# winddori2002/DEX-TTS

Hardware: AMD Instinct MI355X
Metric: mel-frames/s at n_timesteps=50, 80-ch mel (sampler only); RTF (higher is better)
Workload: dtype bf16; 1 GPU; gedex_b1: gedex_lj B=1/GPU T=512 n_timesteps=50 (BASELINE.json configs[1]); global_batch=1, frames=512, hipgraph=False, parallelism=1 GPU

## Files before the change

dex_tts_amd/csrc/conv3x3_bf16.hip:

```cpp
#include "kernels.h"
#include <cstdlib>
#include <cstdio>
#include "lp_util.h"
#include "kernels_lp.h"
#include "conv_gn.h"

namespace dex {
namespace DEX_LP_NS {

typedef float f32x16 __attribute__((ext_vector_type(16)));
typedef unsigned short u16;
typedef unsigned u32x4 __attribute__((ext_vector_type(4)));

__device__ __forceinline__ float cv_mish(float x) {
    const float e = __expf(fminf(x, 20.f));
    const float n = e * (e + 2.f);
    return x * (n * __builtin_amdgcn_rcpf(n + 2.f));
}

template <int NT, int COUT>
__device__ __forceinline__ void cv_epilogue(const Conv3P& p, f32x16 (&acc)[NT], int b, int ho, int w0, int nbase, int lane, int tid,
                                            long long* gnred) {
    const int i = lane & 31, hh = lane >> 5;
    constexpr int cpg = COUT / 8;
    if (p.gn_stats) { if (tid < 16) gnred[tid] = 0; __syncthreads(); }
    const bool full = ho < p.H && w0 + 32 <= p.W;
    const long ybase = (long)b * p.H * p.W * COUT + ((long)ho * p.W + w0 + 4 * hh) * COUT + nbase + i;
    float* yl = p.Y + ybase;
    u16* yh = reinterpret_cast<u16*>(p.Y) + ybase;
    const bool yb = p.y_bf16 != 0;
#pragma unroll
    for (int t = 0; t < NT; ++t) {
        const int n = nbase + t * 32 + i;
        const float bias = p.bias[n];
        float gs = 0.f, gss = 0.f;
        if (full && yb) {
            const bool odd = (lane & 1) != 0;
            u16* yp = yh + (odd ? 16 * COUT - 1 : 0) + t * 32;
#pragma unroll
            for (int r = 0; r < 16; ++r) { const float v = acc[t][r] + bias; gs += v; gss = fmaf(v, v, gss); }
#pragma unroll
            for (int j = 0; j < 8; ++j) {
                const float lo_r = acc[t][j] + bias, hi_r = acc[t][8 + j] + bias;
                const float recv = lane_xor1(odd ? lo_r : hi_r);
                const float mine = odd ? hi_r : lo_r;
                const unsigned pk = odd ? pack2_lp(recv, mine) : pack2_lp(mine, recv);
                *reinterpret_cast<unsigned*>(yp + ((j & 3) + 8 * (j >> 2)) * COUT) = pk;
            }
        } else if (full) {
            const bool odd = (lane & 1) != 0;
            float* yp = yl + (odd ? 16 * COUT - 1 : 0) + t * 32;
#pragma unroll
            for (int r = 0; r < 16; ++r) { const float v = acc[t][r] + bias; gs += v; gss = fmaf(v, v, gss); }
#pragma unroll
            for (int j = 0; j < 8; ++j) {
                const float lo_r = acc[t][j] + bias, hi_r = acc[t][8 + j] + bias;
                const float recv = lane_xor1(odd ? lo_r : hi_r);
                const float mine = odd ? hi_r : lo_r;
                *reinterpret_cast<float2*>(yp + ((j & 3) + 8 * (j >> 2)) * COUT) = odd ? make_float2(recv, mine) : make_float2(mine, recv);
            }
        } else {
#pragma unroll
            for (int r = 0; r < 16; ++r) {
                const int wo = w0 + (r & 3) + 8 * (r >> 2) + 4 * hh;
                const bool ok = ho < p.H && wo < p.W;
                const float v = acc[t][r] + bias;
                const float vs = ok ? v : 0.f;
                gs += vs; gss = fmaf(vs, vs, gss);
                if (ok) {
                    if (yb) yh[((r & 3) + 8 * (r >> 2)) * COUT + t * 32] = lp_bits(v);
                    else yl[((r & 3) + 8 * (r >> 2)) * COUT + t * 32] = v;
                }
            }
        }
        if (p.gn_stats) {
            for (int o = 1; o < cpg; o <<= 1) { gs += __shfl_xor(gs, o); gss += __shfl_xor(gss, o); }
            gs += __shfl_xor(gs, 32); gss += __shfl_xor(gss, 32);
            if (hh == 0 && (i & (cpg - 1)) == 0) {
                const double inv_n = 1.0 / ((double)p.H * p.W * cpg);
                gn_add(&gnred[(n / cpg) * 2], gn_fix(gs, inv_n)); gn_add(&gnred[(n / cpg) * 2 + 1], gn_fix(gss, inv_n));
            }
        }
    }
    if (p.gn_stats) {
        __syncthreads();
        if (tid < 16) {
            const long long v = gnred[tid];
            if (v != 0) {
                const int slot = (blockIdx.x + blockIdx.y * gridDim.x) % GN_SLOTS;
                gn_add(p.gn_stats + (((long)b * 8 + (tid >> 1)) * GN_SLOTS + slot) * 2 + (tid & 1), v);
            }
        }
    }
}

template <int NT, int COUT>
__device__ __forceinline__ void cv_res_store(const Conv3P& p, const f32x16 (&accr)[NT], int b, int ho, int w0, int nb, int lane) {
    const int i = lane & 31, hh = lane >> 5;
    float* yl = p.res_y + ((long)b * p.H * p.W + (long)ho * p.W + w0 + 4 * hh) * COUT + nb + i;
    const bool rfull = ho < p.H && w0 + 32 <= p.W;
    const bool odd = (lane & 1) != 0;
#pragma unroll
    for (int t = 0; t < NT; ++t) {
        const float bias = p.res_b[nb + t * 32 + i];
        if (rfull) {
            float* yp = yl + (odd ? 16 * COUT - 1 : 0) + t * 32;
#pragma unroll
            for (int j = 0; j < 8; ++j) {
                const float lo_r = accr[t][j] + bias, hi_r = accr[t][8 + j] + bias;
                const float recv = lane_xor1(odd ? lo_r : hi_r);
                const float mine = odd ? hi_r : lo_r;
                *reinterpret_cast<float2*>(yp + ((j & 3) + 8 * (j >> 2)) * COUT) = odd ? make_float2(recv, mine) : make_float2(mine, recv);
            }
        } else {
#pragma unroll
            for (int r = 0; r < 16; ++r) {
                const int wo = w0 + (r & 3) + 8 * (r >> 2) + 4 * hh;
                if (ho < p.H && wo < p.W) yl[((r & 3) + 8 * (r >> 2)) * COUT + t * 32] = accr[t][r] + bias;
            }
        }
    }
}

template <int CC, int COUT, int NSL, int TH, bool PRO2 = false, bool RES = false, bool XB = false, int NW = 4, bool RW = false>
__global__ __launch_bounds__(64 * NW) void conv3x3_lp_kernel(const Conv3P p) {
    constexpr int PW = 34, PH = TH + 2;
    constexpr int LDP = CC + 8;
    constexpr int WN = NW / TH;
    constexpr int NTHR = 64 * NW;
    constexpr int NT = NSL / 32 / WN;
    constexpr int NSLICE = COUT / NSL;
    constexpr int ITEMS = PH * PW * (CC / 8);
    constexpr int NI = (ITEMS + NTHR - 1) / NTHR;
    constexpr int WITEMS = NSL * CC / 8;
    constexpr int WPT = (WITEMS + NTHR - 1) / NTHR;
    constexpr bool WFULL = WITEMS % NTHR == 0;
    constexpr int RING = CC == 128 ? (PRO2 ? 1 : 2) : 3;
    constexpr int NPASS = RW ? 1
                        : TH == 5 ? (CC == 128 ? (PRO2 ? 6 : 3) : (PRO2 ? 3 : XB ? 1 : 2))
                                  : CC == 128 ? (TH == 8 ? (PRO2 ? 8 : 4) : (PRO2 ? 5 : 2)) : (PRO2 ? 3 : 1);
    constexpr int NIP = (NI + NPASS - 1) / NPASS;
    constexpr int RWI = 9 * WITEMS;
    constexpr int RWPT = (RWI + NTHR - 1) / NTHR;
    constexpr int RWB = (RWPT + NPASS - 1) / NPASS;
#ifdef DEX_LP_WSPLIT
    constexpr int NTAP = 18;
#else
    constexpr int NTAP = 9;
#endif
    static_assert(NT >= 1 && WPT >= 1 && NW % TH == 0 && NTHR % (CC / 8) == 0, "tile");
    static_assert(!RW || NTAP == 9, "the resident schedule holds nine taps");
    extern __shared__ __attribute__((aligned(16))) u16 smem[];
    u16* patch = smem;
    u16* wbuf = smem + PH * PW * LDP;
    u16* rbuf = wbuf + (RW ? 9 : 2) * NSL * LDP;
    __shared__ long long gnred[16];
    constexpr int COEF_N = (TH == 8) ? 128 : 256;
    __shared__ __attribute__((aligned(16))) float coef[3][COEF_N];

    const int tid = threadIdx.x, lane = tid & 63, wave = tid >> 6;
    const int i = lane & 31, hh = lane >> 5;
    const int wrow = wave % TH, wcol = wave / TH;
#ifdef DEX_TIMING
    long long tk[8] = {0, 0, 0, 0, 0, 0, 0, 0};
    const long long tk0 = __builtin_readcyclecounter();
    long long tlast = tk0;
#define CSTAMP(k) do { const long long now_ = __builtin_readcyclecounter(); tk[k] += now_ - tlast; tlast = now_; } while (0)
#else
#define CSTAMP(k) do {} while (0)
#endif
    const int xs = p.skip_dead ? (int)((blockIdx.x + blockIdx.y + blockIdx.z) % gridDim.x) : (int)blockIdx.x;
    const int w0 = xs * 32, h0 = blockIdx.y * TH;
    const int b = blockIdx.z / NSLICE, slice = blockIdx.z % NSLICE;
    const int step = p.step + b * p.row_bstride;
    const float* X = p.X + (long)b * p.H * p.W * p.ldx + p.x_coff;
    const u16* Xh = reinterpret_cast<const u16*>(p.X) + (long)b * p.H * p.W * p.ldx + p.x_coff;
    const float* mrow = p.mask + (long)b * p.mask_bstride;
    const int K = 9 * p.Cin;
    const u16* Wg = reinterpret_cast<const u16*>(p.Wbf) + (long)slice * NSL * K;
    const bool pro = p.pro_stats != nullptr;
    if constexpr (!PRO2) {
        if (p.skip_dead) {
            const int wi = w0 - 1 + (lane < 34 ? lane : 33);
            const float mv = (unsigned)wi < (unsigned)p.W ? mrow[wi * p.mask_ws] : 0.f;
            if (__builtin_amdgcn_ballot_w64(mv != 0.f) == 0) {
                f32x16 zacc[NT];
#pragma unroll
                for (int t = 0; t < NT; ++t)
#pragma unroll
                    for (int r = 0; r < 16; ++r) zacc[t][r] = 0.f;
                if constexpr (RES) cv_res_store<NT, COUT>(p, zacc, b, h0 + wrow, w0, slice * NSL + wcol * NT * 32, lane);
                cv_epilogue<NT, COUT>(p, zacc, b, h0 + wrow, w0, slice * NSL + wcol * NT * 32, lane, tid, gnred);
                return;
            }
        }
    }

    f32x16 acc[NT];
#pragma unroll
    for (int t = 0; t < NT; ++t)
#pragma unroll
        for (int r = 0; r < 16; ++r) acc[t][r] = 0.f;

    f32x16 accr[RES ? NT : 1];
    if constexpr (RES) {
#pragma unroll
        for (int t = 0; t < NT; ++t)
#pragma unroll
            for (int r = 0; r < 16; ++r) accr[t][r] = 0.f;
    }
    int wofs[WPT], wlds[WPT];
    bool wok[WPT];
#pragma unroll
    for (int j = 0; j < WPT; ++j) {
        const int it = tid + NTHR * j;
        const int n = it / (CC / 8), c8 = (it % (CC / 8)) * 8;
        wofs[j] = n * K + c8;
        wlds[j] = n * LDP + c8;
        wok[j] = WFULL || it < WITEMS;
    }
    const int pc8 = (tid % (CC / 8)) * 8;

    CvGnLoads gnl{};
    if (pro) gnl = cv_gn_issue(p, b, tid, step);
    const int nchunk = RW ? 1 : p.Cin / CC;
    for (int ch = 0; ch < nchunk; ++ch) {
        const int cbase = ch * CC;
        u32x4 w0r[WPT], wr[RING][WPT], rwr[RES ? WPT : 1];
#ifdef DEX_LP_WSPLIT
        u32x4 rwl[RES ? WPT : 1];
#define WS_TAPOFS(t) ((long)((t) % 9) * p.Cin + ((t) >= 9 ? p.w_lo_off : 0L))
#else
#define WS_TAPOFS(t) ((long)(t) * p.Cin)
#endif
        float4 sc0, sc1, sh0, sh1, t0, t1;
#pragma unroll
        for (int ps = 0; ps < NPASS; ++ps) {
            float4 pf0[NIP], pf1[XB ? 1 : NIP], rf0[PRO2 ? NIP : 1], rf1[PRO2 ? NIP : 1];
            float pmk[NIP];
            bool pin[NIP];
#pragma unroll
            for (int q = 0; q < NIP; ++q) {
                const int it = min(tid + NTHR * (ps * NIP + q), ITEMS - 1);
                const int px = it / (CC / 8);
                const int pw = px % PW, ph = px / PW;
                const int hi = h0 + ph - 1, wi = w0 + pw - 1;
                const bool inb = (unsigned)hi < (unsigned)p.H && (unsigned)wi < (unsigned)p.W;
                const int hc = inb ? hi : 0, wc = inb ? wi : 0;
                if constexpr (XB) {
                    pf0[q] = *reinterpret_cast<const float4*>(Xh + ((long)hc * p.W + wc) * p.ldx + cbase + pc8);
                } else {
                    const float* src = X + ((long)hc * p.W + wc) * p.ldx + cbase + pc8;
                    pf0[q] = *reinterpret_cast<const float4*>(src);
                    pf1[q] = *reinterpret_cast<const float4*>(src + 4);
                }
                if constexpr (PRO2) {
                    const float* rs = p.pro_res + ((long)b * p.H * p.W + (long)hc * p.W + wc) * p.Cin + cbase + pc8;
                    rf0[q] = *reinterpret_cast<const float4*>(rs);
                    rf1[q] = *reinterpret_cast<const float4*>(rs + 4);
                }
                const float mk = mrow[wc * p.mask_ws];
                pmk[q] = inb ? mk : 0.f;
                pin[q] = inb;
            }
            u32x4 rwv[RW ? RWB : 1];
            if constexpr (RW) {
#pragma unroll
                for (int j = 0; j < RWB; ++j) {
                    const int it = tid + NTHR * (ps * RWB + j);
                    if (ps * RWB + j < RWPT && (RWI % NTHR == 0 || it < RWI)) {
                        const int r = it % WITEMS;
                        rwv[j] = *reinterpret_cast<const u32x4*>(Wg + (r / (CC / 8)) * K + (it / WITEMS) * p.Cin + (r % (CC / 8)) * 8);
                    }
                }
            }
            if (ps == 0) {
                if constexpr (RES) {
                    const u16* Rg = reinterpret_cast<const u16*>(p.res_w) + (long)slice * NSL * p.Cin;
#pragma unroll
                    for (int j = 0; j < WPT; ++j) {
                        const int it = tid + NTHR * j;
                        if (!wok[j]) continue;
                        rwr[j] = *reinterpret_cast<const u32x4*>(Rg + (long)(it / (CC / 8)) * p.Cin + cbase + (it % (CC / 8)) * 8);
#ifdef DEX_LP_WSPLIT
                        rwl[j] = *reinterpret_cast<const u32x4*>(Rg + p.res_lo_off + (long)(it / (CC / 8)) * p.Cin + cbase + (it % (CC / 8)) * 8);
#endif
                    }
                }
                if constexpr (!RW) {
#pragma unroll
                    for (int j = 0; j < WPT; ++j) if (wok[j]) w0r[j] = *reinterpret_cast<const u32x4*>(Wg + wofs[j] + cbase);
#pragma unroll
                    for (int s = 0; s < RING; ++s)
// ... 67 lines not shown
        }
        if constexpr (!RW) {
#pragma unroll
            for (int j = 0; j < WPT; ++j) if (wok[j]) *reinterpret_cast<u32x4*>(wbuf + wlds[j]) = w0r[j];
        }
        if constexpr (RES) {
#pragma unroll
            for (int j = 0; j < WPT; ++j) if (wok[j]) *reinterpret_cast<u32x4*>(rbuf + wlds[j]) = rwr[j];
        }
        CSTAMP(2);
        if constexpr (RW) {
            lds_barrier();
            constexpr int KS = CC / 16;
            const u16* ap = patch + (wrow * PW + i) * LDP + hh * 8;
            const u16* bp = wbuf + (wcol * NT * 32 + i) * LDP + hh * 8;
            const u16* rp = rbuf + (wcol * NT * 32 + i) * LDP + hh * 8;
            lp8 af[2], bf[2][NT], rf[2][RES ? NT : 1];
            af[0] = *reinterpret_cast<const lp8*>(ap);
#pragma unroll
            for (int t = 0; t < NT; ++t) bf[0][t] = *reinterpret_cast<const lp8*>(bp + t * 32 * LDP);
#pragma unroll
            for (int s = 0; s < 9 * KS; ++s) {
                if (s + 1 < 9 * KS) {
                    const int tap = (s + 1) / KS, ks = (s + 1) % KS, kh = tap / 3, kw = tap - kh * 3;
                    af[(s + 1) & 1] = *reinterpret_cast<const lp8*>(ap + (kh * PW + kw) * LDP + ks * 16);
#pragma unroll
                    for (int t = 0; t < NT; ++t) bf[(s + 1) & 1][t] = *reinterpret_cast<const lp8*>(bp + (tap * NSL + t * 32) * LDP + ks * 16);
                    if constexpr (RES) {
                        if (tap == 4) {
#pragma unroll
                            for (int t = 0; t < NT; ++t) rf[(s + 1) & 1][t] = *reinterpret_cast<const lp8*>(rp + t * 32 * LDP + ks * 16);
                        }
                    }
                }
                __builtin_amdgcn_sched_barrier(0);
#pragma unroll
                for (int t = 0; t < NT; ++t) acc[t] = DEX_MFMA_LP(af[s & 1], bf[s & 1][t], acc[t], 0, 0, 0);
                if constexpr (RES) {
                    if (s / KS == 4) {
#pragma unroll
                        for (int t = 0; t < NT; ++t) accr[t] = DEX_MFMA_LP(af[s & 1], rf[s & 1][t], accr[t], 0, 0, 0);
                    }
                }
                __builtin_amdgcn_sched_barrier(0);
            }
        } else {
#pragma unroll
        for (int tt = 0; tt < NTAP; ++tt) {
            const int tap = tt % 9;
            lds_barrier();
            if (tt + 1 < NTAP) {
                u16* wn = wbuf + ((tt + 1) & 1) * NSL * LDP;
#pragma unroll
                for (int j = 0; j < WPT; ++j) if (wok[j]) *reinterpret_cast<u32x4*>(wn + wlds[j]) = wr[tt % RING][j];
                if (tt + 1 + RING < NTAP) {
#pragma unroll
                    for (int j = 0; j < WPT; ++j)
                        if (wok[j]) wr[tt % RING][j] = *reinterpret_cast<const u32x4*>(Wg + wofs[j] + WS_TAPOFS(tt + 1 + RING) + cbase);
                }
                __builtin_amdgcn_sched_barrier(0);
            }
#ifdef DEX_LP_WSPLIT
            if constexpr (RES) {
                if (tt == 5) {
#pragma unroll
                    for (int j = 0; j < WPT; ++j) if (wok[j]) *reinterpret_cast<u32x4*>(rbuf + wlds[j]) = rwl[j];
                }
            }
#endif
            const u16* wb = wbuf + (tt & 1) * NSL * LDP;
            const int kh = tap / 3, kw = tap - kh * 3;
            const u16* ap = patch + ((wrow + kh) * PW + i + kw) * LDP + hh * 8;
            const u16* bp = wb + (wcol * NT * 32 + i) * LDP + hh * 8;
#pragma unroll
            for (int ks = 0; ks < CC / 16; ++ks) {
                const lp8 af = *reinterpret_cast<const lp8*>(ap + ks * 16);
#pragma unroll
                for (int t = 0; t < NT; ++t) {
                    const lp8 bf = *reinterpret_cast<const lp8*>(bp + t * 32 * LDP + ks * 16);
                    acc[t] = DEX_MFMA_LP(af, bf, acc[t], 0, 0, 0);
                }
                if constexpr (RES) {
                    if (tap == 4) {
#pragma unroll
                        for (int t = 0; t < NT; ++t) {
                            const lp8 rf = *reinterpret_cast<const lp8*>(rbuf + (wcol * NT * 32 + t * 32 + i) * LDP + hh * 8 + ks * 16);
                            accr[t] = DEX_MFMA_LP(af, rf, accr[t], 0, 0, 0);
                        }
                    }
                }
            }
        }
        }
    }
    if constexpr (RES) cv_res_store<NT, COUT>(p, accr, b, h0 + wrow, w0, slice * NSL + wcol * NT * 32, lane);
    CSTAMP(3);
    cv_epilogue<NT, COUT>(p, acc, b, h0 + wrow, w0, slice * NSL + wcol * NT * 32, lane, tid, gnred);
#ifdef DEX_TIMING
    CSTAMP(4);
    if (p.dbg && tid == 0) {
        long long* d = p.dbg + ((long)(blockIdx.z * gridDim.y + blockIdx.y) * gridDim.x + blockIdx.x) * 8;
        for (int k = 0; k < 5; ++k) d[k] = tk[k];
        unsigned hw, xcc;
        asm volatile("s_getreg_b32 %0, hwreg(HW_REG_HW_ID)" : "=s"(hw));
        asm volatile("s_getreg_b32 %0, hwreg(HW_REG_XCC_ID)" : "=s"(xcc));
        d[5] = hw; d[6] = xcc & 15u;
        d[7] = __builtin_readcyclecounter() - tk0;
    }
#endif
}

template <int CC, int COUT, int NSL, int TH, bool PRO2 = false, bool RES = false, bool XB = false, int NW = 4, bool RW = false>
static void launch_c3(const Conv3P& p, hipStream_t st) {
    constexpr int LDP = CC + 8;
    const size_t lds = ((size_t)(TH + 2) * 34 * LDP + ((RW ? 9 : 2) + (RES ? 1 : 0)) * NSL * LDP) * sizeof(u16);
    static bool attr = false;
    if (!attr) {
        hipFuncSetAttribute(reinterpret_cast<const void*>(&conv3x3_lp_kernel<CC, COUT, NSL, TH, PRO2, RES, XB, NW, RW>), hipFuncAttributeMaxDynamicSharedMemorySize, (int)lds);
        attr = true;
    }
    dim3 grid((p.W + 31) / 32, (p.H + TH - 1) / TH, p.B * (COUT / NSL));
    if (RW && p.Cin != CC) { fprintf(stderr, "libdexamd: resident conv3x3 form needs Cin == %d in one chunk (got %d)\n", CC, p.Cin); abort(); }
    Conv3P q = p;
    q.skip_dead = (p.B >= 4 && (long)grid.x * grid.y * grid.z >= 1024 && knob_or("DEX_CONV_SKIP_DEAD", 1) != 0) ? 1 : 0;
    static char sym[96];
    if (!sym[0]) snprintf(sym, sizeof sym, "conv3x3_lp_kernel<%d,%d,%d,%d,%d,%d,%d,%d%s>", CC, COUT, NSL, TH, (int)PRO2, (int)RES, (int)XB, NW, RW ? ",resident" : "");
    g_last_symbol = sym;
    hipLaunchKernelGGL((conv3x3_lp_kernel<CC, COUT, NSL, TH, PRO2, RES, XB, NW, RW>), grid, dim3(64 * NW), lds, st, q);
}

bool conv3x3_bf16_tail_supported(int C) {
#if defined(DEX_LP_WSPLIT) && !defined(DEX_WS_HAVE_CONV3)
    return false;
#endif
    return C == 64 || C == 128; }
bool conv3x3_bf16_xb_supported(int Cin, int Cout) {
#if defined(DEX_LP_WSPLIT) && !defined(DEX_WS_HAVE_CONV3)
    return false;
#endif
    return Cin == Cout && (Cin == 64 || Cin == 128); }
bool conv3x3_bf16_res_supported(int Cin, int Cout) {
#if defined(DEX_LP_WSPLIT) && !defined(DEX_WS_HAVE_CONV3_RES)
    return false;
#endif
    return (Cout == 128 && Cin == 64) || (Cout == 64 && (Cin == 128 || Cin == 256)); }
bool conv3x3_bf16_supported(int Cin, int Cout) {
#if defined(DEX_LP_WSPLIT) && !defined(DEX_WS_HAVE_CONV3)
    return false;
#endif
   
    return (Cin == 64 || Cin == 128 || Cin == 256) && (Cout == 64 || Cout == 128);
}

bool conv3x3_plain_lp_in_supported(int H, int W, int B, int Cin, int Cout) {
#if defined(DEX_LP_WSPLIT) && !defined(DEX_WS_HAVE_CONV3)
    return false;
#endif
   
    const int w8 = knob_or("DEX_CONV_W8", 1);
    const long tiles4 = (long)((W + 31) / 32) * ((H + 3) / 4) * B;
    return w8 && tiles4 >= 256 && Cin == 64 && Cout == 128;
}

bool conv3x3_cat_lp_in_supported(int H, int W, int B, int Cin, int Cout) {
#if defined(DEX_LP_WSPLIT) && !defined(DEX_WS_HAVE_CONV3_RES)
    return false;
#endif
   
    if (Cout != 64 || Cin < 128 || Cin % 128 != 0) return false;
    const int w8 = knob_or("DEX_CONV_W8", 1);
    const long small_max = knob_or("DEX_CONV_SMALL_MAX", 256);
    const long tiles4 = (long)((W + 31) / 32) * ((H + 3) / 4) * B;
    return w8 && tiles4 >= small_max;
}

static bool conv3x3_resident_on() { return knob_or("DEX_CONV_RESIDENT", 1) != 0; }

static bool launch_c3_round1(const Conv3P& p, bool small, hipStream_t st) {
    if (!knob_or("DEX_CONV_ROUND1", 1)) return false;
    const bool tail_ = p.pro_res != nullptr;
#ifdef DEX_LP_WSPLIT
    const bool c64 = p.Cin == 64 && p.Cout == 64 && !p.res_w && !tail_;
#else
    const bool c64 = p.Cin == 64 && p.Cout == 64 && !p.res_w;
#endif
    const bool r128 = p.Cin == 64 && p.Cout == 128 && p.res_w && !tail_ && !p.x_bf16;
    if (!c64 && !r128) return false;
    const long strips = (long)((p.W + 31) / 32) * p.B;
    const long cur = c64 ? strips * (small ? (p.H + 1) / 2 : (p.H + 3) / 4) : strips * (small ? (p.H + 1) / 2 * 2 : (p.H + 3) / 4);
    const long one = strips * ((p.H + 4) / 5) * (c64 ? 1 : 4);
    const long ncu = device_cus();
    if (cur <= ncu || one > ncu || one * 4 < ncu * 3) return false;
#ifndef DEX_LP_WSPLIT
    if (conv3x3_resident_on()) {
        if (c64 && !tail_) {
            p.x_bf16 ? launch_c3<64, 64, 64, 5, false, false, true, 10, true>(p, st) : launch_c3<64, 64, 64, 5, false, false, false, 10, true>(p, st);
            return true;
        }
        if (!c64) { launch_c3<64, 128, 32, 5, false, true, false, 5, true>(p, st); return true; }
    }
#endif
    if (c64) {
#ifndef DEX_LP_WSPLIT
        if (tail_) { p.x_bf16 ? launch_c3<64, 64, 64, 5, true, false, true, 10>(p, st) : launch_c3<64, 64, 64, 5, true, false, false, 10>(p, st); return true; }
#endif
        p.x_bf16 ? launch_c3<64, 64, 64, 5, false, false, true, 10>(p, st) : launch_c3<64, 64, 64, 5, false, false, false, 10>(p, st);
    } else {
        launch_c3<64, 128, 32, 5, false, true, false, 5>(p, st);
    }
    return true;
}

static bool launch_c3_small_resident(const Conv3P& p, bool small, hipStream_t st) {
#ifdef DEX_LP_WSPLIT
    return false;
#else
    if (!small || !conv3x3_resident_on() || p.Cin != 64 || p.Cout != 64 || p.res_w) return false;
    if ((long)((p.W + 31) / 32) * ((p.H + 1) / 2) * p.B > device_cus()) return false;
    const bool tail_ = p.pro_res != nullptr;
    if (tail_) { p.x_bf16 ? launch_c3<64, 64, 64, 2, true, false, true, 4, true>(p, st) : launch_c3<64, 64, 64, 2, true, false, false, 4, true>(p, st); }
    else { p.x_bf16 ? launch_c3<64, 64, 64, 2, false, false, true, 4, true>(p, st) : launch_c3<64, 64, 64, 2, false, false, false, 4, true>(p, st); }
    return true;
#endif
}

void launch_conv3x3_lp(const Conv3P& p, hipStream_t st) {
    if (const int tpw = conv3x3_stream_tiles(p)) { launch_conv3x3_stream(p, tpw, st); return; }
    if (conv3x3_regw_form(p)) { launch_conv3x3_regw(p, st); return; }
    const bool tail_ = p.pro_res != nullptr;
    const long tiles4 = (long)((p.W + 31) / 32) * ((p.H + 3) / 4) * p.B;
    const long small_max = knob_or("DEX_CONV_SMALL_MAX", 256);
    const bool small = tiles4 < small_max;
    const int w8 = knob_or("DEX_CONV_W8", 1);
    const int th8 = knob_or("DEX_CONV_TH8", 1);
    if (th8 && w8 && !small && !tail_ && p.Cin == 128 && p.Cout == 128 && !p.res_w && p.H % 8 == 0 && (long)((p.W + 31) / 32) * (p.H / 8) * p.B >= 512) {
        p.x_bf16 ? launch_c3<128, 128, 128, 8, false, false, true, 8>(p, st) : launch_c3<128, 128, 128, 8, false, false, false, 8>(p, st);
        return;
    }
    if (w8 && !small && p.Cin == 128 && p.Cout == 128 && !p.res_w) {
        if (p.x_bf16) { tail_ ? launch_c3<128, 128, 128, 4, true, false, true, 8>(p, st) : launch_c3<128, 128, 128, 4, false, false, true, 8>(p, st); }
        else { tail_ ? launch_c3<128, 128, 128, 4, true, false, false, 8>(p, st) : launch_c3<128, 128, 128, 4, false, false, false, 8>(p, st); }
        return;
    }
    if (w8 && !small && p.res_w && p.Cout == 128 && p.Cin == 64) {
        p.x_bf16 ? launch_c3<64, 128, 128, 4, false, true, true, 8>(p, st) : launch_c3<64, 128, 128, 4, false, true, false, 8>(p, st);
        return;
    }
    if (th8 && w8 && !small && p.res_w && p.Cout == 64 && p.Cin >= 128 && !p.pro_stats && p.H % 8 == 0 && (long)((p.W + 31) / 32) * (p.H / 8) * p.B >= 512) {
        p.x_bf16 ? launch_c3<128, 64, 64, 8, false, true, true, 8>(p, st) : launch_c3<128, 64, 64, 8, false, true, false, 8>(p, st);
        return;
    }
    if (w8 && !small && p.res_w && p.Cout == 64 && p.Cin >= 128) {
        p.x_bf16 ? launch_c3<128, 64, 64, 4, false, true, true, 8>(p, st) : launch_c3<128, 64, 64, 4, false, true, false, 8>(p, st);
        return;
    }
    if (launch_c3_round1(p, small, st)) return;
    if (launch_c3_small_resident(p, small, st)) return;
    if (p.x_bf16) {
        if (tail_) {
            if (p.Cin == 64) { small ? launch_c3<64, 64, 64, 2, true, false, true>(p, st) : launch_c3<64, 64, 64, 4, true, false, true>(p, st); }
            else { small ? launch_c3<128, 128, 64, 2, true, false, true>(p, st) : launch_c3<128, 128, 128, 4, true, false, true>(p, st); }
        } else {
            if (p.Cin == 64) { small ? launch_c3<64, 64, 64, 2, false, false, true>(p, st) : launch_c3<64, 64, 64, 4, false, false, true>(p, st); }
            else { small ? launch_c3<128, 128, 64, 2, false, false, true>(p, st) : launch_c3<128, 128, 128, 4, false, false, true>(p, st); }
        }
        return;
    }
    if (tail_) {
        if (p.Cin == 64 && p.Cout == 64) { small ? launch_c3<64, 64, 64, 2, true>(p, st) : launch_c3<64, 64, 64, 4, true>(p, st); }
        else { small ? launch_c3<128, 128, 64, 2, true>(p, st) : launch_c3<128, 128, 128, 4, true>(p, st); }
        return;
    }
    if (p.res_w) {
        if (p.Cout == 128 && p.Cin == 64) { small ? launch_c3<64, 128, 64, 2, false, true>(p, st) : launch_c3<64, 128, 128, 4, false, true>(p, st); return; }
        if (p.Cout == 64 && p.Cin >= 128) { small ? launch_c3<128, 64, 64, 2, false, true>(p, st) : launch_c3<128, 64, 64, 4, false, true>(p, st); return; }
    }
    if (p.Cout == 64) {
        if (p.Cin == 64) { small ? launch_c3<64, 64, 64, 2>(p, st) : launch_c3<64, 64, 64, 4>(p, st); }
        else { small ? launch_c3<128, 64, 64, 2>(p, st) : launch_c3<128, 64, 64, 4>(p, st); }
    } else {
        if (p.Cin == 64) { small ? launch_c3<64, 128, 64, 2>(p, st) : launch_c3<64, 128, 128, 4>(p, st); }
        else { small ? launch_c3<128, 128, 64, 2>(p, st) : launch_c3<128, 128, 128, 4>(p, st); }
    }
}

}
}
```

dex_tts_amd/csrc/dex_api.hip:

```cpp
#include <hip/hip_runtime.h>
#include <cstdlib>

#include <cmath>
#include <cstdarg>
#include <atomic>
#include <cstdio>
#include <mutex>
#include <cstring>
#include <map>
#include <unordered_map>
#include <string_view>
#include <string>
#include <vector>

#include "../../include/dex_amd.h"
#include "kernels.h"
#include "weight_store.h"

using namespace dex;

namespace dex {
namespace {
const char* const KNOB_NAMES[] = {
    "DEX_CONV_STREAM", "DEX_CONV_PP", "DEX_CONV_SKIP_DEAD", "DEX_H_BF16", "DEX_ATTN_SEPARATE", "DEX_ATTN_Q64", "DEX_ATTN_Q64_TAIL", "DEX_ATTN_Q64_HALF", "DEX_DIT_XCDS", "DEX_ATTN_GENERIC", "DEX_RES2", "DEX_LP_INTER", "DEX_DIT_CHAIN",
    "DEX_DIT_CLUSTER", "DEX_DIT_CLUSTER_LOCAL", "DEX_ATTN_X_LP", "DEX_RES_X_LP", "DEX_CAT_LP", "DEX_XCD_MAP", "DEX_DEBUG_DROP_HANDOFF", "DEX_PATCH_FUSED",
    "DEX_CONV_DOWN", "DEX_CONVT_UP", "DEX_DEBUG_PLAN",
    "DEX_ATTN_SHARED_W8", "DEX_CONVT_MT", "DEX_CONVT_WGS", "DEX_CONV_DOWN_WGS", "DEX_CONV_REGW", "DEX_CONV_REGW_RES", "DEX_CONV_SMALL_MAX", "DEX_CONV_TH8",
    "DEX_CONV_W8", "DEX_DWCONV_CAP", "DEX_FINAL_CAP", "DEX_FIRST_CAP", "DEX_FIRST_MFMA", "DEX_GEMM_NWALK", "DEX_NWALK_SPLIT", "DEX_NWALK_BM", "DEX_POS_COL", "DEX_POS_COL_MIN",
    "DEX_POS_CT", "DEX_REGW_MIN_TILES", "DEX_REGW_WGS", "DEX_ROWCHAIN64", "DEX_ROWCHAIN64A", "DEX_TIV_CAP", "DEX_TV_CHAIN", "DEX_TIV_FOLD", "DEX_LINATTN_NSUB", "DEX_TV_FOLD", "DEX_OUT2_MIN", "DEX_NWALK_DMA",
    "DEX_LINATTN_HEADWAVES", "DEX_LINATTN_OUT2_HW", "DEX_CONV_ROUND1", "DEX_CONV_RESIDENT", "DEX_KVCTX_ROWS", "DEX_OUT2_ROWS", "DEX_PE_TOK", "DEX_NWALK_SMALL"};
constexpr int N_KNOBS = (int)(sizeof(KNOB_NAMES) / sizeof(KNOB_NAMES[0]));
int knob_parse(const char* e) {
    if (!e) return KNOB_UNSET;
    char* end = nullptr;
    const long v = strtol(e, &end, 10);
    if (end == e) {
        static bool warned = false;
        if (!warned) { warned = true; fprintf(stderr, "libdexamd: ignoring a DEX_* knob whose value '%s' is not an integer\n", e); }
        return KNOB_UNSET;
    }
    return (int)v;
}
struct KnobSnapshot {
    int v[N_KNOBS];
    KnobSnapshot() { for (int i = 0; i < N_KNOBS; ++i) v[i] = knob_parse(getenv(KNOB_NAMES[i])); }
};
thread_local const KnobSnapshot* t_knobs = nullptr;
struct WsplitScope {
    bool prev;
    explicit WsplitScope(bool on) : prev(g_lp_wsplit) { g_lp_wsplit = on; }
    ~WsplitScope() { g_lp_wsplit = prev; }
};
struct KnobScope {
    const KnobSnapshot* prev;
    explicit KnobScope(const KnobSnapshot* k) : prev(t_knobs) { t_knobs = k; }
    ~KnobScope() { t_knobs = prev; }
};
}
static int knob_index(const char* name) {
    static const std::unordered_map<std::string_view, int> idx = [] {
        std::unordered_map<std::string_view, int> m;
        for (int i = 0; i < N_KNOBS; ++i) m.emplace(KNOB_NAMES[i], i);
        return m;
    }();
    const auto it = idx.find(std::string_view(name));
    return it == idx.end() ? -1 : it->second;
}
int knob(const char* name) {
    if (t_knobs) {
        const int i = knob_index(name);
        if (i >= 0) return t_knobs->v[i];
    }
    return knob_parse(getenv(name));
}
}
static_assert(PREC_FP32 == DEX_PREC_FP32 && PREC_BF16 == DEX_PREC_BF16 && PREC_FP16 == DEX_PREC_FP16 && PREC_FP16X2 == DEX_PREC_FP16X2, "kernels.h mirrors DexPrecision");

namespace {
void xcd_map_probe();

struct TD { float* p; int ld; int coff; int C; int lp = 0; };

struct ResW { PackedW w1, w2, wr; const float *b1, *g1, *be1, *b2, *g2, *be2, *br, *mlp_w, *mlp_b; int cin, cout; };
constexpr int ATT_KSPLIT_MAX = 4;
static int att_split_cap(long tokens) { return tokens <= 20480 ? 8 : ATT_KSPLIT_MAX; }
static bool attention_q64_regime(int N, int B) {
    if (N < 1024) return dit_sep64_small_n(N, B) && dit_rowchain64_form(N, B, 0);
    const int ks = attention_q64_ksplit(N, B, att_split_cap((long)B * N));
    const int nt32 = (N + 31) / 32, ng = (nt32 + 7) / 8;
    return 2L * B * ng * ks >= 128;
}
struct LinW { PackedW wqkv; const float *wqkv_raw, *wout_raw, *bias_eff, *g; LpView wkv[3], wq_frag[3]; int C; };
struct DitBlockW { PackedW wqkv, wproj, wfc1, wfc2; const float *bqkv, *bproj, *bfc1, *bfc2, *ada_w, *ada_b; };

struct Prof { std::string name; hipEvent_t a, b; double flops, bytes; };
struct ProfAgg { std::string name; int calls; double ms, flops, bytes; };

struct Arena {
    char* base = nullptr; size_t off = 0, cap = 0; bool dry = true;
    void* take(size_t bytes) {
        off = (off + 255) & ~size_t(255);
        void* p = dry ? nullptr : (void*)(base + off);
        if (!dry && trace) fprintf(stderr, "plan[%d] off %zu bytes %zu\n", trace++, off, bytes);
        off += bytes;
        return p;
    }
    int trace = 0;
    float* f(size_t n) { return (float*)take(n * sizeof(float)); }
};

}

struct DexCtx : WeightStore {
    DexCtx() : WeightStore("") {}
    DexConfig cfg{};
    int lpi() const { return precision == DEX_PREC_FP16X2 ? 2 : precision == DEX_PREC_FP16 ? 1 : 0; }
    int lp_kind() const { return precision == DEX_PREC_BF16 ? 1 : 2; }
    bool lp() const { return precision != DEX_PREC_FP32; }
    bool tuned = true;
    int precision = DEX_PREC_FP32;
    std::vector<std::vector<ResW>> down_res, up_res;
    std::vector<LinW> down_lin, up_lin;
    std::vector<PackedW> down_ds_w;
    std::vector<std::vector<PackedW>> up_us_w;
    std::vector<const float*> down_ds_b, up_us_b;
    const float *fc_w3 = nullptr, *fc_w1 = nullptr;
    PackedW fin_w, pe_pw, fl_w, tv_wk, tv_wv, tv_wl;
    PackedW pos_w;
    const float *fin_b = nullptr, *fin_g = nullptr, *fin_be = nullptr, *fconv_w = nullptr, *fconv_b = nullptr;
    const float *pe_dw = nullptr, *pe_db = nullptr, *pe_pb = nullptr, *pos_b = nullptr, *freq_pos = nullptr;
    std::vector<DitBlockW> blocks;
    const float *fl_b = nullptr, *fl_ada_w = nullptr, *fl_ada_b = nullptr;
    const float *tv_wq_raw = nullptr;
    float *mel_basis = nullptr, *mel_filt = nullptr; void* mel_ws = nullptr; size_t mel_ws_bytes = 0;
    const int* last_xerr = nullptr;
    int* st_host = nullptr; hipEvent_t st_ev = nullptr; bool st_pending = false;
    struct Tap { std::string name; const float* p; std::vector<int64_t> shape; };
    std::vector<Tap> taps;
    bool prof_on = false;
    std::vector<Prof> prof;
    std::vector<ProfAgg> prof_agg;
    struct GraphEntry { std::vector<uint64_t> key; hipGraphExec_t exec; uint64_t stamp; const int* xerr; };
    std::vector<GraphEntry> graphs;
    uint64_t graph_clock = 0;
    void drop_graphs() { for (auto& g : graphs) hipGraphExecDestroy(g.exec); graphs.clear(); }
    template <typename F> int replay(const std::vector<uint64_t>& key, hipStream_t st, F&& enqueue);
    void reset_records() {
        taps.clear();
        if (prof_on) { for (auto& pr : prof) { hipEventDestroy(pr.a); hipEventDestroy(pr.b); } prof.clear(); prof_agg.clear(); }
    }
};

template <typename F> int DexCtx::replay(const std::vector<uint64_t>& key, hipStream_t st, F&& enqueue) {
    GraphEntry* hit = nullptr;
    for (auto& g : graphs) if (g.key == key) { hit = &g; break; }
    if (!hit) {
        constexpr size_t MAX_GRAPHS = 8;
        if (graphs.size() >= MAX_GRAPHS) {
            size_t lru = 0;
            for (size_t i = 1; i < graphs.size(); ++i) if (graphs[i].stamp < graphs[lru].stamp) lru = i;
            hipGraphExecDestroy(graphs[lru].exec);
            graphs.erase(graphs.begin() + lru);
        }
        hipGraph_t graph = nullptr;
        DEX_HIPCHK(this, hipStreamBeginCapture(st, hipStreamCaptureModeThreadLocal));
        const int rc = enqueue();
        hipError_t ec = hipStreamEndCapture(st, &graph);
        if (rc) { if (graph) hipGraphDestroy(graph); return rc; }
        if (ec != hipSuccess || !graph) return fail(DEX_ERR_HIP, "stream capture failed: %s", hipGetErrorString(ec));
        hipGraphExec_t exec = nullptr;
        ec = hipGraphInstantiate(&exec, graph, nullptr, nullptr, 0);
        hipGraphDestroy(graph);
        if (ec != hipSuccess) return fail(DEX_ERR_HIP, "hipGraphInstantiate failed: %s", hipGetErrorString(ec));
        graphs.push_back({key, exec, 0, last_xerr});
        hit = &graphs.back();
    }
    last_xerr = hit->xerr;
    hit->stamp = ++graph_clock;
    DEX_HIPCHK(this, hipGraphLaunch(hit->exec, st));
    DEX_HIPCHK(this, hipGetLastError());
    return DEX_OK;
}

// ... 663 lines not shown
        g.inmask = nullptr; g.inmask_ws = 1; g.outmask = nullptr; g.outmask_ws = 1; g.mask_bstride = P.d.T;
        g.act = 0; g.gate = nullptr; g.gate_nstride = 1; g.gate_step_stride = 0;
        g.res = nullptr; g.ldres = 0; g.res_bstride = 0; g.res_coff = 0;
        g.step = sp; g.row_bstride = rbs; g.unpatch_s = 0; g.unpatch_C = 0; g.B = P.d.B;
        return g;
    }
    void gemm(const char* name, const IGemmP& g) {
        const double M = (double)g.Ho * g.Wo * g.B;
        const double fl = 2.0 * M * g.N * g.groups * g.K;
        const double by = 4.0 * (M * g.Cin * g.groups + M * g.N * g.groups * g.ksplit + (double)g.K * g.N * g.groups);
        run(name, fl, by, [&] { launch_igemm(g, x->precision, st); });
    }
    struct Pro { const gnfix_t* stats; const float *gamma, *beta, *tadd; const float* res = nullptr; float* xout = nullptr; bool x_bf16 = false;
                 bool res2 = false; FirstConvP res2f{};
                 mutable bool xout_lp_ok = false;
                 mutable bool xout_lp = false; };
    static bool ln_fusable(int K) { return K == 64 || K == 128 || K == 256 || K == 512; }
    bool h_bf16() const { return x->lp() && !knob_off("DEX_H_BF16"); }
    bool fast_conv(int cin, int cout) const { return x->lp() && conv3x3_bf16_supported(cin, cout); }
    void conv3x3(const char* name, const TD& X, int H, int W, int mask_ws, bool inmask, const PackedW& Wt, const float* bias, int Cout, float* out,
                 gnfix_t* gn = nullptr, const Pro* pro = nullptr, const ResW* shortcut = nullptr, float* shortcut_out = nullptr,
                 bool xb = false, bool yb = false) {
        const int t = x->lpi();
        if (fast_conv(X.C, Cout) && Wt.nk[t].p) {
            Conv3P c{};
            c.x_bf16 = (xb || X.lp) ? 1 : 0; c.y_bf16 = yb ? 1 : 0;
            c.X = X.p; c.ldx = X.ld; c.x_coff = X.coff; c.H = H; c.W = W; c.Cin = X.C; c.Cout = Cout;
            c.Wbf = Wt.nk[t].p; c.w_lo_off = Wt.nk[t].lo_off; c.bias = bias; c.Y = out; c.mask = mask; c.mask_ws = mask_ws; c.mask_bstride = P.d.T;
            if (pro) { c.pro_stats = pro->stats; c.pro_gamma = pro->gamma; c.pro_beta = pro->beta; c.pro_tadd = pro->tadd; c.pro_res = pro->res; c.pro_xout = pro->xout;
                if (pro->res2) {
                    const FirstConvP& f = pro->res2f;
                    c.pro_res = nullptr; c.res2_w = f.W1; c.res2_b = f.b1; c.res2_mu = f.mu; c.res2_x = f.x; c.res2_spk = f.spk;
                    c.res2_scal = f.scal; c.res2_scal_stride = f.scal_stride; c.res2_planes = f.planes;
                } }
            c.step = sp; c.row_bstride = rbs; c.gn_stats = gn; c.B = P.d.B;
            c.Wfrag = Wt.frag[t].p;
            const bool want_xout_lp = pro && pro->xout && pro->xout_lp_ok;
            if (shortcut) {
                c.res_w = shortcut->wr.nk[t].p; c.res_lo_off = shortcut->wr.nk[t].lo_off; c.res_b = shortcut->br; c.res_y = shortcut_out;
                c.res_wfrag = shortcut->wr.frag[t].p;
            }
            if (want_xout_lp && (c.pro_res || c.res2_w) && conv3x3_strip_form(c)) { c.xout_lp = 1; pro->xout_lp = true; }
            const double M = (double)H * W * P.d.B;
            const double bytes = M * (((xb || X.lp) ? 2.0 : 4.0) * X.C + (yb ? 2.0 : 4.0) * Cout + (pro && (pro->res || pro->res2) ? (pro->res2 ? 4.0 * X.C : 8.0 * X.C) - (c.xout_lp ? 2.0 * X.C : 0.0) : 0.0) + (shortcut ? 4.0 * Cout : 0.0))
                                 + 2.0 * 9 * X.C * Cout;
            run(name, 2.0 * M * Cout * (9 * X.C + (shortcut ? X.C : 0)), bytes, [&] { launch_conv3x3_lp(c, x->precision, st); });
            return;
        }
        IGemmP g = base_gemm(X.p, X.ld, X.coff, H, W, X.C, Wt, Cout, bias, out, Cout, 0);
        g.KH = 3; g.KW = 3; g.off_h = -1; g.off_w = -1; g.K = 9 * X.C;
        if (inmask) { g.inmask = mask; g.inmask_ws = mask_ws; }
        g.gn_stats = gn; g.gn_groups = 8; g.gn_cpg = Cout / 8;
        gemm(name, g);
    }
    void gn_stats(const float* h, int C, long npix, gnfix_t* stats) {
        GnStatsP s{h, C, npix * C, (int)npix, C, 8, stats, P.d.B};
        run("gn_stats", 3.0 * npix * C * P.d.B, 4.0 * npix * C * P.d.B, [&] { launch_gn_stats(s, st); });
    }
    void gn_apply(const float* h, int C, long npix, int W, int mask_ws, const gnfix_t* stats, const float* gamma, const float* beta,
                  const float* tadd, const float* res, int ldres, long resb, bool res_under_mask, float* out) {
        GnApplyP a{};
        a.X = h; a.ldx = C; a.xb = npix * C; a.Y = out; a.ldy = C; a.yb = npix * C; a.y_coff = 0;
        a.npix = (int)npix; a.W = W; a.C = C; a.groups = 8; a.stats = stats; a.gamma = gamma; a.beta = beta;
        a.mask = mask; a.mask_ws = mask_ws; a.mask_bstride = P.d.T;
        a.tadd = tadd; a.tadd_step_stride = C; a.step = sp; a.row_bstride = rbs;
        a.res = res; a.ldres = ldres; a.resb = resb; a.res_under_mask = res_under_mask ? 1 : 0; a.B = P.d.B;
        run("gn_apply_mish", 12.0 * npix * C * P.d.B, (res ? 12.0 : 8.0) * npix * C * P.d.B, [&] { launch_gn_apply(a, st); });
    }

    void resblock(const ResW& w, const StageBuf& s, const TD& X, const float* tadd, float* out, bool first_layer, LinKvCtxP* tail = nullptr,
                  const Pro* head = nullptr, Pro* ctail = nullptr) {
        const long npix = s.npix;
        const float* resptr; int ldres; long resb; bool under = false;
        gnfix_t* st1 = nullptr;
        const bool conv2_fast = fast_conv(w.cout, w.cout) && conv3x3_bf16_xb_supported(w.cout, w.cout);
        const bool conv1_fast = first_layer || (head ? true : fast_conv(X.C, w.cout));
        const bool h1b = h_bf16() && conv2_fast && conv1_fast;
        const bool h2b = h_bf16() && conv2_fast && (ctail || tail);
        if (first_layer) {
            FirstConvP f{};
            f.h1_bf16 = h1b ? x->lp_kind() : 0;
            f.mu = mu; f.x = xcur; f.spk = P.spk_plane; f.mask = mask; f.B = P.d.B; f.H = s.H; f.T = s.W; f.planes = w.cin; f.C = w.cout;
            f.W3 = w.w1.f32; f.b3 = w.b1; f.W1 = w.wr.f32; f.b1 = w.br; f.scal = P.scal; f.scal_stride = SCAL_STRIDE; f.step = sp; f.row_bstride = rbs;
            f.h1 = s.h1; f.res = s.rbuf;
            { if (ctail && h2b && w.cout == 64 && conv3x3_res2_form(s.H, s.W, P.d.B) && !knob_off("DEX_RES2")) { f.res = nullptr; ctail->res2 = true; ctail->res2f = f; } }
            st1 = next_stats(); f.gn_stats = st1;
            run("first_conv", 2.0 * npix * P.d.B * w.cout * (w.cin * 10), npix * P.d.B * ((h1b ? 2.0 : 4.0) * w.cout + (f.res ? 4.0 * w.cout : 0.0) + 4.0 * w.cin), [&] { launch_first_conv(f, st); });
            resptr = s.rbuf; ldres = w.cout; resb = npix * w.cout;
        } else {
            st1 = next_stats();
            bool fused_res = false;
            if (head) {
                TD H2{s.h2, X.C, 0, X.C};
                head->xout_lp_ok = tail != nullptr && !w.wr && lp_inter_cur && head->xout == X.p && X.coff == 0 && X.ld == X.C && !knob_off("DEX_RES_X_LP");
                conv3x3("conv3x3", H2, s.H, s.W, s.mask_ws, true, w.w1, w.b1, w.cout, s.h1, st1, head, nullptr, nullptr, head->x_bf16, h1b);
            } else {
                fused_res = w.wr && fast_conv(X.C, w.cout) && conv3x3_bf16_res_supported(X.C, w.cout);
                conv3x3("conv3x3", X, s.H, s.W, s.mask_ws, true, w.w1, w.b1, w.cout, s.h1, st1, nullptr, fused_res ? &w : nullptr, s.rbuf, false, h1b);
            }
            if (fused_res) {
                resptr = s.rbuf; ldres = w.cout; resb = npix * w.cout;
            } else if (w.wr) {
                IGemmP g = base_gemm(X.p, X.ld, X.coff, s.H, s.W, X.C, w.wr, w.cout, w.br, s.rbuf, w.cout, 0);
                g.inmask = mask; g.inmask_ws = s.mask_ws;
                gemm("conv1x1_res", g);
                resptr = s.rbuf; ldres = w.cout; resb = npix * w.cout;
            } else {
                resptr = X.p + X.coff; ldres = X.ld; resb = npix * X.ld; under = true;
            }
        }
        if (!st1) { st1 = next_stats(); gn_stats(s.h1, w.cout, npix, st1); }
        gnfix_t* st2 = next_stats();
        if (fast_conv(w.cout, w.cout)) {
            Pro pro{st1, w.g1, w.be1, tadd};
            TD H1{s.h1, w.cout, 0, w.cout};
            conv3x3("conv3x3", H1, s.H, s.W, s.mask_ws, true, w.w2, w.b2, w.cout, s.h2, st2, &pro, nullptr, nullptr, h1b, h2b);
        } else {
            gn_apply(s.h1, w.cout, npix, s.W, s.mask_ws, st1, w.g1, w.be1, tadd, nullptr, 0, 0, false, s.a1);
            TD A1{s.a1, w.cout, 0, w.cout};
            conv3x3("conv3x3", A1, s.H, s.W, s.mask_ws, false, w.w2, w.b2, w.cout, s.h2, st2);
        }
        if (ctail) {
            ctail->stats = st2; ctail->gamma = w.g2; ctail->beta = w.be2; ctail->tadd = nullptr; ctail->res = resptr; ctail->xout = out;
            ctail->x_bf16 = h2b;
            return;
        }
        if (tail) {
            tail->H2 = s.h2; tail->gn_stats = st2; tail->gamma = w.g2; tail->beta = w.be2;
            tail->res = resptr; tail->ldres = ldres; tail->resb = resb; tail->res_under_mask = under ? 1 : 0;
            tail->res_lp = (head && head->xout_lp && resptr == X.p) ? 1 : 0;
            tail->mask = mask; tail->mask_ws = s.mask_ws; tail->mask_bstride = P.d.T; tail->W = s.W; tail->Xout = out;
            tail->h2_bf16 = h2b ? 1 : 0;
            return;
        }
        gn_apply(s.h2, w.cout, npix, s.W, s.mask_ws, st2, w.g2, w.be2, nullptr, resptr, ldres, resb, under, out);
    }

    bool lp_inter_cur = false;
    bool cat_lp = false;
    IGemmP final_gemm(int mask_ws, float* out, int ldo, int ocoff) {
        const DexConfig& c = x->cfg;
        const int hid = c.dit_hidden, mid = mid_dim(c);
        const bool fuse_lnf = x->lp() && ln_fusable(hid);
        const int s2c = c.dit_stride * c.dit_stride * mid;
        IGemmP fl = base_gemm(fuse_lnf ? P.tok : P.xn, hid, 0, P.Hf, P.Wt, hid, x->fl_w, s2c, x->fl_b, out, ldo, ocoff);
        if (fuse_lnf) { fl.ln_shift = P.fin_mod; fl.ln_scale = P.fin_mod + hid; fl.ln_step_stride = 2L * hid; }
        fl.Wfrag = x->fl_w.frag[x->lpi()].p;
        fl.unpatch_s = c.dit_stride; fl.unpatch_C = mid; fl.OHf = P.Hm; fl.OWf = P.Wm;
        fl.c_bstride = (long)P.Hm * P.Wm * ldo;
        fl.outmask = mask; fl.outmask_ws = mask_ws;
        return fl;
    }
    bool linattn_fused(int C) const { return x->lp() && (C == 64 || C == 128) && linattn_fused_supported(C); }
    void linattn(const LinW& w, const StageBuf& s, const TD& X, float* out, int ldo, int ocoff, const LinKvCtxP* tail = nullptr, bool out_lp = false,
                 void* out2_lp = nullptr, int ldo2 = 0, int ocoff2 = 0) {
        const long npix = s.npix; const int B = P.d.B;
        if (linattn_fused(X.C)) {
            int nsub = 1;
            while (nsub < 4 && (npix + 128 * nsub - 1) / (128 * nsub) * B > 192) nsub *= 2;
            {
                const int ncu = device_cus();
                const long slots = (long)(X.C == 64 ? 2 : 1) * ncu;
                if ((npix + 127) / 128 * B >= 2 * slots) {
                    long best = -1;
                    for (int n = 1; n <= 8; ++n) {
                        const long wgs = (npix + 128L * n - 1) / (128L * n) * B;
                        const long cost = (wgs + slots - 1) / slots * n;
                        if (best < 0 || cost <= best) { best = cost; nsub = n; }
                    }
                }
                const int forced = knob_or("DEX_LINATTN_NSUB", 0);
                if (forced > 0) nsub = forced;
            }
            const int nblk = (int)((npix + 128L * nsub - 1) / (128L * nsub));
            LinKvCtxP k{};
            if (tail) k = *tail;
            k.X = X.p; k.ldx = X.ld; k.x_coff = X.coff; k.xb = npix * X.ld; k.npix = (int)npix; k.C = X.C; k.Wkv = w.wkv[x->lpi()].p;
            k.wkv_lo_off = w.wkv[x->lpi()].lo_off;
            k.nsub = nsub; k.nblk = nblk; k.part_m = s.pm; k.part_s = s.ps; k.part_c = s.pc; k.B = B;
            k.headwaves = knob_or("DEX_LINATTN_HEADWAVES", (long)nblk * B <= device_cus() ? 1 : 0) != 0 ? 1 : 0;
            k.rows = knob_or("DEX_KVCTX_ROWS", 1) != 0 ? 1 : 0;
            const bool xlp = k.H2 && k.Xout && lp_inter_cur && linattn_out2_lp_out_supported((int)npix, B) && !knob_off("DEX_ATTN_X_LP");
            k.xout_lp = xlp ? 1 : 0;
            run("linattn_kvctx", 2.0 * npix * B * (256.0 * X.C + 128 * 32), (tail ? (tail->h2_bf16 ? 10.0 : 12.0) - (xlp ? 2.0 : 0.0) : 4.0) * npix * X.C * B, [&] { launch_linattn_kvctx(k, x->precision, st); });
            LinMergeP mg{s.pm, s.ps, s.pc, nblk, w.wout_raw, w.g, X.C, s.mbf, B};
            run("linattn_merge", 2.0 * 128 * 32 * X.C * B, 4.0 * nblk * 4 * 1088 * B, [&] { launch_linattn_merge(mg, x->precision, st); });
            LinOut2P o{X.p, X.ld, X.coff, npix * X.ld, (int)npix, X.C, w.wq_frag[x->lpi()].p, s.mbf, w.bias_eff, out, ldo, ocoff, npix * ldo, B, out_lp ? 1 : 0,
                       out2_lp, ldo2, ocoff2, npix * ldo2, xlp ? 1 : 0};
            o.wq_lo_off = w.wq_frag[x->lpi()].lo_off;
            o.hw = knob_or("DEX_LINATTN_OUT2_HW", linattn_out2_lp_out_supported((int)npix, B) ? 0 : 1) != 0 ? 1 : 0;
            o.rows = knob_or("DEX_OUT2_ROWS", 1) != 0 ? 1 : 0;
            run("linattn_out", 4.0 * npix * B * 128.0 * X.C, ((out_lp ? 6.0 : 8.0) - (xlp ? 2.0 : 0.0) + (out2_lp ? 2.0 : 0.0)) * npix * X.C * B, [&] { launch_linattn_out2(o, x->precision, st); });
            return;
        }
        IGemmP g = base_gemm(X.p, X.ld, X.coff, s.H, s.W, X.C, w.wqkv, 384, nullptr, s.qkv, 384, 0);
        gemm("linattn_qkv", g);
        LinAttnCtxP cp{s.qkv, 384, npix * 384, (int)npix, 4, LA_CHUNK, s.nchunks, s.pm, s.ps, s.pc, B};
        run("linattn_ctx", 2.0 * npix * 128 * 32 * B, 4.0 * npix * 384 * B, [&] { launch_linattn_ctx(cp, st); });
        LinAttnCombineP cb{s.pm, s.ps, s.pc, s.nchunks, 4, w.wout_raw, w.g, w.C, s.weff, B};
        run("linattn_combine", 2.0 * 128 * 32 * w.C * B, 4.0 * s.nchunks * 4 * 1100 * B, [&] { launch_linattn_combine(cb, st); });
        IGemmP o = base_gemm(s.qkv, 384, 0, s.H, s.W, 128, s.weff, w.C, w.bias_eff, out, ldo, ocoff);
        o.w_bstride = 128L * w.C;
        o.res = X.p; o.ldres = X.ld; o.res_coff = X.coff; o.res_bstride = npix * X.ld;
        gemm("linattn_out", o);
    }

    void dit(const TD& X, bool mask_input, int mask_ws, float* out, int ldo, int ocoff, const float* in_aff = nullptr) {
        const DexConfig& c = x->cfg;
        const int B = P.d.B, hid = c.dit_hidden, mid = mid_dim(c), N = P.N, mh = mlp_hidden(c);
        DwConvP dw{};
        dw.X = X.p + X.coff; dw.ldx = X.ld; dw.xb = (long)P.Hm * P.Wm * X.ld; dw.Hi = P.Hm; dw.Wi = P.Wm; dw.C = mid;
        dw.k = c.dit_patch; dw.s = c.dit_stride; dw.pad = c.dit_patch / 2; dw.Wd = x->pe_dw; dw.bd = x->pe_db;
        dw.mask = mask_input ? mask : nullptr; dw.mask_ws = mask_ws; dw.mask_bstride = P.d.T;
        dw.Y = P.pe0; dw.Hf = P.Hf; dw.Wt = P.Wt; dw.B = B; dw.aff = in_aff;
        if (patch_fused()) {
            run("patch_embed", 2.0 * B * N * mid * (c.dit_patch * c.dit_patch + hid), 4.0 * B * (P.Hm * P.Wm * mid + N * hid),
                [&] { launch_patch_embed_fused(dw, x->pe_pw.nk[x->lpi()].p, x->pe_pb, P.emb, hid, x->precision, st); });
        } else {
            run("patch_dwconv_silu", 2.0 * B * N * mid * c.dit_patch * c.dit_patch, 4.0 * B * (P.Hm * P.Wm + N) * mid, [&] { launch_dwconv_silu(dw, st); });
            IGemmP pe = base_gemm(P.pe0, mid, 0, P.Hf, P.Wt, mid, x->pe_pw, hid, x->pe_pb, P.emb, hid, 0);
            gemm("patch_pointwise", pe);
        }
        const int G = c.dit_conv_pos_groups, kp = c.dit_conv_pos, cg = hid / G;
        int nsplit = POS_SPLIT, pcg = 0, pcgp = 0;
        if (x->lp() && x->pos_w.frag[x->lpi()].p) {
            PosConvP pcd{P.emb, x->pos_w.frag[x->lpi()].p, P.pos_part, P.Hf, P.Wt, hid, G, B};
            run("pos_conv", 2.0 * B * N * (double)kp * kp * cg * hid, 8.0 * B * N * hid + 2.0 * kp * kp * cg * hid, [&] { launch_pos_conv_direct(pcd, x->precision, st); });
            nsplit = 1;
        } else {
            const int cgp = (cg % 32) ? 64 : cg;
            const float* src = P.emb;
            if (cgp != cg) {
                run("pos_group_pad", 0, 8.0 * B * N * hid, [&] { launch_group_pad(P.emb, P.emb_pad, (long)B * N, G, cg, cgp, st); });
                src = P.emb_pad;
            }
            IGemmP pc = base_gemm(src, G * cgp, 0, P.Hf, P.Wt, cgp, x->pos_w, cgp, nullptr, P.pos_part, G * cgp, 0);
            pc.KH = kp; pc.KW = kp; pc.off_h = -(kp / 2); pc.off_w = -(kp / 2); pc.K = kp * kp * cgp;
            pc.groups = G; pc.w_gstride = (long)kp * kp * cgp * cgp; pc.ksplit = POS_SPLIT; pc.c_sstride = (long)B * N * G * cgp;
            gemm("pos_conv", pc);
            pcg = cgp != cg ? cg : 0; pcgp = cgp;
        }
        PosFinishP pf{P.pos_part, nsplit, (long)B * N * (pcg ? G * pcgp : hid), x->pos_b, P.emb, x->freq_pos, P.tok, P.Hf, P.Wt, hid, B, pcg, pcgp};
        run("pos_finish", 20.0 * B * N * hid, 4.0 * B * N * hid * (nsplit + 2), [&] { launch_pos_finish(pf, st); });
        if (debug) hipMemcpyAsync(P.dbg_tok, P.tok, (size_t)B * N * hid * 4, hipMemcpyDeviceToDevice, st);
        tap("tok_in", P.dbg_tok, (long)B * N, hid, hid);
        const float scale = 1.0f / sqrtf((float)(hid / c.dit_heads));
        const bool chain = x->lp() && dit_rowchain_supported(hid, mh) && c.dit_heads == 2 &&
                           !knob_off("DEX_DIT_CHAIN");
        for (int k = 0; k < c.dit_depth; ++k) {
            const DitBlockW& w = x->blocks[k];
            const float* ada = P.ada[k];
            const bool fuse_ln = x->lp() && ln_fusable(hid);
            DitChainP ch{};
            if (chain) {
                ch.ksplit = 0; ch.heads = c.dit_heads; ch.rows_per_batch = N; ch.X = P.tok; ch.ada = ada; ch.step = sp; ch.row_bstride = rbs; ch.M = B * N; ch.B = B;
                ch.Qh = (k & 1) ? P.qh : P.qh2; ch.Kh = (k & 1) ? P.kh : P.kh2; ch.Vt = (k & 1) ? P.vt : P.vt2;
                ch.Qin = (k & 1) ? P.qh2 : P.qh; ch.Kin = (k & 1) ? P.kh2 : P.kh; ch.Vin = (k & 1) ? P.vt2 : P.vt;
                ch.Npad = P.Npad;
                ch.qscale = scale * 1.4426950408889634f;
                if (P.xflag) {
                    ch.xslab = P.xslab; ch.xflag = P.xflag; ch.epoch = (unsigned)(sp * (c.dit_depth + 1) + k + 1);
                    ch.xerr = reinterpret_cast<int*>(P.xflag + (P.xflag_bytes - sizeof(int)) / sizeof(unsigned));
                    x->last_xerr = ch.xerr;
                    ch.xdrop = knob_or("DEX_DEBUG_DROP_HANDOFF", 0);
                    ch.xlocal = (P.xlocal && ch.epoch < (1u << 24)) ? 1 : 0;
                    ch.xcds = dit_rowchain_cluster_xcds(N, B);
                }
            }
            if (chain && k == 0) {
                ch.qkv_only = 1; ch.Wq = w.wqkv.frag[x->lpi()].p; ch.bq = w.bqkv;
                ch.Qh = P.qh; ch.Kh = P.kh; ch.Vt = P.vt;
                ch.next_shift = ada; ch.next_scale = ada + hid; ch.next_step_stride = 6L * hid;
                run("dit_qkv", 2.0 * B * N * 3.0 * hid * hid, 4.0 * B * N * hid + 2.0 * B * N * 3 * hid, [&] { launch_dit_rowchain(ch, x->precision, st); });
                ch.qkv_only = 0; ch.Wq = nullptr; ch.bq = nullptr; ch.next_shift = ch.next_scale = nullptr;
                ch.Qh = P.qh2; ch.Kh = P.kh2; ch.Vt = P.vt2;
            }
            if (!chain) {
                IGemmP q = base_gemm(fuse_ln ? P.tok : P.xn, hid, 0, 1, N, hid, w.wqkv, 3 * hid, w.bqkv, P.qkv, 3 * hid, 0);
                if (fuse_ln) { q.ln_shift = ada + 0 * hid; q.ln_scale = ada + 1 * hid; q.ln_step_stride = 6L * hid; }
                else {
                    LnModP l1{P.tok, P.xn, N, hid, ada + 0 * hid, ada + 1 * hid, 6L * hid, sp, B, rbs};
                    run("ln_modulate", 8.0 * B * N * hid, 8.0 * B * N * hid, [&] { launch_ln_mod(l1, st); });
                }
                gemm("dit_qkv", q);
            }
            if (chain) {
                const int sep_env = knob("DEX_ATTN_SEPARATE");
                const bool batch_regime = attention_direct_batch_regime(N, B);
                const int q64_env = knob("DEX_ATTN_Q64");
                const bool q64_ok = q64_env != KNOB_UNSET ? q64_env != 0 : attention_q64_regime(N, B);
                const bool separate = sep_env != KNOB_UNSET ? sep_env != 0 : ((batch_regime && N >= 1024) || q64_ok);
                const bool q64 = separate && q64_ok;
                int ks = 1, tail_row0 = 0, tail_ks = 0;
                bool o_lp = false;
                if (separate) {
                    const long blocks = (long)((N + 31) / 32) * 2 * B;
                    const int ntiles = (N + 31) / 32;
                    ks = q64 ? attention_q64_ksplit(N, B, att_split_cap((long)B * N))
                       : batch_regime ? attention_direct_ksplit(N, B)
                                      : (int)std::max<long>(1, std::min<long>(std::min<long>(768 / blocks, (ntiles + 7) / 8), ATT_KSPLIT_MAX));
                    AttnDirectP ad{ch.Qin, ch.Kin, ch.Vin, N, P.Npad, B, P.ao, (long)B * N * hid, ks > 1 ? P.att_ml : nullptr, ks, nullptr};
                    o_lp = (batch_regime || q64) && ks == 1 && lp_inter_cur && dit_rowchain64_form(N, B, 0);
                    ad.o_lp = o_lp ? 1 : 0;
                    if (q64 && ks == 1 && dit_rowchain64_form(N, B, 0) && knob_or("DEX_ATTN_Q64_TAIL", 0) != 0) {
                        int pks = 1, tg = 0, tk = 1;
                        attention_q64_plan(N, B, att_split_cap((long)B * N), &pks, &tg, &tk);
                        if (pks == 1 && tk > 1) { ad.tail_g = tg; ad.tail_ks = tk; ad.ml = P.att_ml; tail_row0 = tg * 256; tail_ks = tk; }
                    }
                    run("dit_attention", 4.0 * B * (double)N * N * hid, 2.0 * 3 * B * N * hid + (o_lp ? 2.0 : 4.0) * B * N * hid * ks,
                        [&] { if (q64) launch_attention_q64(ad, x->precision, st); else launch_attention_direct(ad, x->precision, st); });
                }
                ch.attn_inline = separate ? 0 : 1; ch.o_lp = o_lp ? 1 : 0; ch.tail_row0 = tail_row0; ch.tail_ks = tail_ks;
                const bool last = k + 1 == c.dit_depth;
                ch.O = P.ao; ch.ksplit = ks; ch.o_sstride = (long)B * N * hid; ch.ml = P.att_ml;
                ch.Wp = w.wproj.frag[x->lpi()].p; ch.W1 = w.wfc1.frag[x->lpi()].p; ch.W2 = w.wfc2.frag[x->lpi()].p;
                ch.bp = w.bproj; ch.b1 = w.bfc1; ch.b2 = w.bfc2;
                if (!last) {
                    const DitBlockW& wn = x->blocks[k + 1];
                    ch.Wq = wn.wqkv.frag[x->lpi()].p; ch.bq = wn.bqkv;
                    ch.next_shift = P.ada[k + 1]; ch.next_scale = P.ada[k + 1] + hid; ch.next_step_stride = 6L * hid;
                }
                const double M = (double)B * N;
                const double wel = (double)hid * hid + 2.0 * hid * mh + (last ? 0.0 : 3.0 * hid * hid);
                run(separate ? "dit_rowchain" : "dit_block", 2.0 * M * wel + (separate ? 0.0 : 4.0 * B * (double)N * N * hid),
                    4.0 * M * hid * (last ? 3 : 6) + 2.0 * wel, [&] { launch_dit_rowchain(ch, x->precision, st); });
                if (debug) {
                    float* dst = P.dbg_tok + (size_t)(k + 1) * B * N * hid;
                    hipMemcpyAsync(dst, P.tok, (size_t)B * N * hid * 4, hipMemcpyDeviceToDevice, st);
                    char nm[32]; snprintf(nm, sizeof nm, "tok_blk%d", k);
                    tap(nm, dst, (long)B * N, hid, hid);
                }
                continue;
            }
            AttnP a{};
            a.Q = P.qkv; a.ldq = 3 * hid; a.qb = (long)N * 3 * hid;
            a.K = P.qkv + hid; a.ldk = 3 * hid; a.kb = a.qb; a.V = P.qkv + 2 * hid; a.ldv = 3 * hid; a.vb = a.qb;
            a.O = P.ao; a.ldo = hid; a.ob = (long)N * hid; a.Nq = N; a.Nk = N; a.kv_len = nullptr; a.kv_len_add = 0;
            a.heads = c.dit_heads; a.scale = scale; a.B = B; a.head_dim = hid / c.dit_heads;
            a.force_generic = (knob_or("DEX_ATTN_GENERIC", 0) && x->precision == DEX_PREC_FP32) ? 1 : 0;
            run("dit_attention", 4.0 * B * (double)N * N * hid, 4.0 * 4 * B * N * hid, [&] { launch_attention(a, x->precision, st); });
            IGemmP pr = base_gemm(P.ao, hid, 0, 1, N, hid, w.wproj, hid, w.bproj, P.tok, hid, 0);
            pr.gate = ada + 2 * hid; pr.gate_nstride = 1; pr.gate_step_stride = 6L * hid;
            pr.res = P.tok; pr.ldres = hid; pr.res_bstride = (long)N * hid;
            gemm("dit_proj", pr);
            IGemmP f1 = base_gemm(fuse_ln ? P.tok : P.xn, hid, 0, 1, N, hid, w.wfc1, mh, w.bfc1, P.hmlp, mh, 0);
            if (fuse_ln) { f1.ln_shift = ada + 3 * hid; f1.ln_scale = ada + 4 * hid; f1.ln_step_stride = 6L * hid; }
            else {
                LnModP l2{P.tok, P.xn, N, hid, ada + 3 * hid, ada + 4 * hid, 6L * hid, sp, B, rbs};
                run("ln_modulate", 8.0 * B * N * hid, 8.0 * B * N * hid, [&] { launch_ln_mod(l2, st); });
            }
            f1.act = 1;
            gemm("dit_fc1_gelu", f1);
            IGemmP f2 = base_gemm(P.hmlp, mh, 0, 1, N, mh, w.wfc2, hid, w.bfc2, P.tok, hid, 0);
            f2.gate = ada + 5 * hid; f2.gate_nstride = 1; f2.gate_step_stride = 6L * hid;
            f2.res = P.tok; f2.ldres = hid; f2.res_bstride = (long)N * hid;
            gemm("dit_fc2", f2);
            if (debug) {
                float* dst = P.dbg_tok + (size_t)(k + 1) * B * N * hid;
                hipMemcpyAsync(dst, P.tok, (size_t)B * N * hid * 4, hipMemcpyDeviceToDevice, st);
                char nm[32]; snprintf(nm, sizeof nm, "tok_blk%d", k);
                tap(nm, dst, (long)B * N, hid, hid);
            }
        }
        const bool fuse_lnf = x->lp() && ln_fusable(hid);
        if (!fuse_lnf) {
            LnModP lf{P.tok, P.xn, N, hid, P.fin_mod, P.fin_mod + hid, 2L * hid, sp, B, rbs};
            run("ln_modulate", 8.0 * B * N * hid, 8.0 * B * N * hid, [&] { launch_ln_mod(lf, st); });
        }
        IGemmP fl = final_gemm(mask_ws, out, ldo, ocoff);
        if (cat_lp) { fl.C = reinterpret_cast<float*>(P.cat16); fl.c_lp = x->lp_kind(); }
        gemm("dit_final_unpatchify", fl);
    }

    bool patch_fused() const {
        const DexConfig& c = x->cfg;
        return x->lp() && !debug && !knob_off("DEX_PATCH_FUSED") &&
               patch_embed_fused_supported(c.dit_patch, mid_dim(c), c.dit_hidden, (long)P.d.B * P.N);
    }
    bool tiv_fold() const { return !debug && P.tiv_aff && knob_or("DEX_TIV_FOLD", 1) != 0; }
    bool tv_chain_on() const {
        return x->lp() && x->tv_wl.nk[x->lpi()].p && P.tv_kp && tv_chain_form(P.Hm * P.Wm, mid_dim(x->cfg), P.d.B);
    }
    bool tv_fold_on() const { return tv_chain_on() && x->lpi() != 2 && P.tv_G && knob_or("DEX_TV_FOLD", 1) != 0; }
    void dex_adaptors(const TD& X, int mask_ws) {
        const DexConfig& c = x->cfg;
        const int B = P.d.B, mid = mid_dim(c);
        const long npix = (long)P.Hm * P.Wm;
        InStatsP is{X.p + X.coff, X.ld, npix * X.ld, (int)npix, mid, P.tv_stats, B, mask, mask_ws, (long)P.d.T, P.Wm};
        run("in2d_stats", 3.0 * npix * mid * B, 4.0 * npix * mid * B, [&] { launch_in_stats(is, st); });
        const long stats_floats = (long)B * mid * IN_SLOTS * 2 * (long)(sizeof(gnfix_t) / sizeof(float));
        if (tv_fold_on()) {
            TvFold2P f2{P.tv_stats, (int)npix, 1e-5f, P.tv_G, (long)(P.d.Ts + 1) * mid, P.tv_g0, P.tv_v0p, sp, P.d.Ts + 1, P.tv_nkpad, mid,
                        1.0f / sqrtf((float)mid), P.tv_kp, P.tv_vtp, P.tv_xmean, reinterpret_cast<float*>(P.tiv_stats), stats_floats, x->lp_kind(), B, rbs};
            run("tv_fold_keys", 2.0 * B * (P.d.Ts + 1) * mid, 6.0 * B * (P.d.Ts + 1) * mid, [&] { launch_tv_fold2(f2, st); });
            TvChainP tc{X.p, X.ld, X.coff, npix * X.ld, (int)npix, P.Wm, mask, mask_ws, (long)P.d.T,
                        nullptr, 0L, nullptr, nullptr, 0L,
                        P.tv_kp, P.tv_vtp, P.tv_nkpad, P.d.Ts + 1, args->sty_lengths_dev, 1, 1.0f,
                        P.tv_out, P.tiv_stats, B, P.tv_xmean, reinterpret_cast<float*>(P.tv_stats), stats_floats};
            run("tv_chain", 4.0 * B * (double)npix * (P.d.Ts + 1) * mid, 8.0 * B * npix * mid, [&] { launch_tv_chain(tc, x->precision, st); });
            tap("tv", P.tv_out, B * npix, mid, mid);
            tiv(npix);
            return;
        }
        const bool qbf = x->lp();
        InFoldP fo{P.tv_stats, (int)npix, 1e-5f, x->tv_wq_raw, mid, P.tv_weff, P.tv_beff, B, qbf ? P.tv_wbf : nullptr, x->lp_kind()};
        fo.split = x->lpi() == 2 ? 1 : 0;
        run("tv_fold_in2d", 2.0 * mid * mid * B, 8.0 * mid * mid * B, [&] { launch_in_fold(fo, st); });
        IGemmP q = base_gemm(X.p, X.ld, X.coff, P.Hm, P.Wm, mid, P.tv_weff, mid, P.tv_beff, P.tv_q, mid, 0);
        q.w_bstride = (long)mid * mid; q.bias_bstride = mid; q.inmask = mask; q.inmask_ws = mask_ws;
        if (qbf) { q.Wbf = P.tv_wbf; q.w_lo_off = fo.split ? (long)B * mid * mid : 0; }
        const bool chain = tv_chain_on();
        if (!chain) gemm("tv_q", q);
        TvRow0P r0{P.tv_k0, P.tv_v0, sp, P.tv_K, P.tv_V, (long)(P.d.Ts + 1) * mid, mid, B, reinterpret_cast<float*>(P.tv_stats),
                   (long)B * mid * IN_SLOTS * 2 * 2 * (long)(sizeof(gnfix_t) / sizeof(float))};
        r0.row_bstride = rbs;
        if (chain) { r0.Kp = P.tv_kp; r0.VTp = P.tv_vtp; r0.NkPad = P.tv_nkpad; r0.lp_kind = x->lp_kind(); }
        run("tv_time_token", 0, 8.0 * mid * B, [&] { launch_tv_row0(r0, st); });
        if (chain) {
            const LpView& wl = x->tv_wl.nk[x->lpi()];
            TvChainP tc{X.p, X.ld, X.coff, npix * X.ld, (int)npix, P.Wm, mask, mask_ws, (long)P.d.T,
                        P.tv_wbf, fo.split ? (long)B * mid * mid : 0L, P.tv_beff, wl.p, wl.lo_off,
                        P.tv_kp, P.tv_vtp, P.tv_nkpad, P.d.Ts + 1, args->sty_lengths_dev, 1, 1.0f / sqrtf((float)mid),
                        P.tv_out, P.tiv_stats, B};
            run("tv_chain", 4.0 * B * (double)npix * mid * mid + 4.0 * B * (double)npix * (P.d.Ts + 1) * mid, 8.0 * B * npix * mid,
                [&] { launch_tv_chain(tc, x->precision, st); });
            tap("tv", P.tv_out, B * npix, mid, mid);
            tiv(npix);
            return;
        }
        AttnP a{};
        a.Q = P.tv_q; a.ldq = mid; a.qb = npix * mid; a.K = P.tv_K; a.ldk = mid; a.kb = (long)(P.d.Ts + 1) * mid;
        a.V = P.tv_V; a.ldv = mid; a.vb = a.kb; a.O = P.tv_ao; a.ldo = mid; a.ob = npix * mid;
        a.Nq = (int)npix; a.Nk = P.d.Ts + 1; a.kv_len = args->sty_lengths_dev; a.kv_len_add = 1; a.heads = 1;
        a.scale = 1.0f / sqrtf((float)mid); a.B = B; a.head_dim = mid;
        const bool ao_lp = lp_inter_cur && mid == 128 && x->tv_wl.nk[x->lpi()].p && attention_lp_shared_form((int)npix, 1, B, 1);
        a.o_lp = ao_lp ? 1 : 0;
        run("tv_attention", 4.0 * B * (double)npix * (P.d.Ts + 1) * mid, (ao_lp ? 2.0 : 4.0) * B * npix * mid + 4.0 * B * (npix + 2 * (P.d.Ts + 1)) * mid, [&] { launch_attention(a, x->precision, st); });
        IGemmP o = base_gemm(P.tv_ao, mid, 0, P.Hm, P.Wm, mid, x->tv_wl, mid, nullptr, P.tv_out, mid, 0);
        if (ao_lp) o.a_lp = x->lp_kind();
        o.res = X.p; o.ldres = X.ld; o.res_coff = X.coff; o.res_bstride = npix * X.ld;
        o.outmask = mask; o.outmask_ws = mask_ws;
        o.gn_stats = P.tiv_stats; o.gn_groups = mid; o.gn_cpg = 1; o.stats_final = 1;
        gemm("tv_out", o);
        tap("tv", P.tv_out, B * npix, mid, mid);
        tiv(npix);
    }
    void tiv(long npix) {
        const int B = P.d.B, mid = mid_dim(x->cfg);
        TivApplyP ta{P.tv_out, mid, npix * mid, P.tiv_out, mid, npix * mid, (int)npix, mid, P.tiv_stats, 1e-5f, P.sap_s, P.sap_m, sp, B, rbs};
        if (tiv_fold()) { run("tiv_coefficients", 0, 16.0 * mid * B, [&] { launch_tiv_coef(ta, P.tiv_aff, st); }); return; }
        run("tiv_adain", 2.0 * npix * mid * B, 8.0 * npix * mid * B, [&] { launch_tiv_apply(ta, st); });
        tap("tiv", P.tiv_out, B * npix, mid, mid);
    }

    void step(float* denoised, float* xnext) {
        const DexConfig& c = x->cfg;
        const int B = P.d.B, ns = c.n_stages;
        gn_idx = 0;
        if (debug) {
            tap("mlp", P.temb + (long)sp * c.dim, rbs ? B : 1, c.dim, c.dim);
            tap("vit.t_embedder", P.c_emb + (long)sp * c.dit_hidden, rbs ? B : 1, c.dit_hidden, c.dit_hidden);
        }
        if (!stats_other) zero_fill(stats_base, P.stats_bytes, st);
        TD cur{nullptr, 0, 0, 0};
        const bool lp_inter = x->lp() && !debug && ns >= 2 && !knob_off("DEX_LP_INTER") && fast_conv(c.dim, c.dim);
        lp_inter_cur = lp_inter;
        cat_lp = false;
        if (lp_inter && ns == 2 && P.cat16) {
            const StageBuf& sm_ = P.down[ns - 1];
            const ResW& uw = x->up_res[0][0];
            const bool tail_ok = linattn_fused(sm_.C) && linattn_out2_lp_out_supported((int)sm_.npix, B);
            const bool conv_ok = uw.wr && fast_conv(2 * sm_.C, uw.cout) && conv3x3_bf16_res_supported(2 * sm_.C, uw.cout) &&
                                 conv3x3_cat_lp_in_supported(P.up[0].H, P.up[0].W, B, 2 * sm_.C, uw.cout);
            IGemmP fl = final_gemm(sm_.mask_ws, P.cat[0], 2 * sm_.C, 0);
            fl.c_lp = x->lp_kind();
            cat_lp = !knob_off("DEX_CAT_LP") && tail_ok && conv_ok && fl.Wbf && igemm_nwalk_form(fl);
        }
        const int lpk = x->lp_kind();
        for (int i = 0; i < ns; ++i) {
            const StageBuf& s = P.down[i];
            Pro t0{};
            const bool defer0 = x->lp() && conv3x3_bf16_tail_supported(s.C) && fast_conv(s.C, s.C) &&
                                (i == 0 || x->down_res[i][0].wr);
            resblock(x->down_res[i][0], s, cur, P.tadd_down[2 * i], s.r0out, i == 0, nullptr, nullptr, defer0 ? &t0 : nullptr);
            TD r0{s.r0out, s.C, 0, s.C};
            LinKvCtxP tail{};
            const bool defer = linattn_fused(s.C);
            resblock(x->down_res[i][1], s, r0, P.tadd_down[2 * i + 1], s.r1out, false, defer ? &tail : nullptr, defer0 ? &t0 : nullptr);
            TD r1{s.r1out, s.C, 0, s.C};
            if (debug && !x->lp()) {
                char n0[24], n1[24]; snprintf(n0, sizeof n0, "downs.%d.0", i); snprintf(n1, sizeof n1, "downs.%d.1", i);
                tap(n0, s.r0out, B * s.npix, s.C, s.C); tap(n1, s.r1out, B * s.npix, s.C, s.C);
            }
            const bool t1_lp = lp_inter && i == 0 && i < ns - 1 && linattn_fused(s.C) && linattn_out2_lp_out_supported((int)s.npix, B);
            const bool skip16 = cat_lp && i == ns - 1;
            linattn(x->down_lin[i], s, r1, s.attn_out, s.attn_ld, s.attn_coff, defer ? &tail : nullptr, t1_lp,
                    skip16 ? P.cat16 : nullptr, s.attn_ld, s.attn_coff);
            char nm[16]; snprintf(nm, sizeof nm, "down%d", i);
            tap(nm, s.attn_out + s.attn_coff, B * s.npix, s.C, s.attn_ld);
            if (i < ns - 1) {
                TD a{s.attn_out, s.attn_ld, s.attn_coff, s.C};
                IGemmP g = base_gemm(a.p, a.ld, a.coff, s.H, s.W, s.C, x->down_ds_w[i], s.C, x->down_ds_b[i], s.ds_out, s.C, 0);
                g.KH = 3; g.KW = 3; g.sh = 2; g.sw = 2; g.off_h = -1; g.off_w = -1; g.K = 9 * s.C;
                g.Ho = s.H / 2; g.Wo = s.W / 2; g.OHf = g.Ho; g.OWf = g.Wo; g.c_bstride = (long)g.Ho * g.Wo * s.C;
                g.inmask = mask; g.inmask_ws = s.mask_ws;
                const ResW& nw = x->down_res[i + 1][0];
                const bool t2_lp = lp_inter && nw.wr && fast_conv(s.C, nw.cout) && conv3x3_bf16_res_supported(s.C, nw.cout) &&
                                   conv3x3_plain_lp_in_supported(g.Ho, g.Wo, B, s.C, nw.cout);
                g.a_lp = t1_lp ? lpk : 0; g.c_lp = t2_lp ? lpk : 0;
                const bool strip_off = knob_off("DEX_CONV_DOWN");
                if (x->lp() && !strip_off && x->down_ds_w[i].frag[x->lpi()].p && conv_down_supported(s.C, s.H, s.W, a.ld, s.C, a.coff)) {
                    ConvDownP d{};
                    d.X = a.p; d.a_lp = g.a_lp; d.ldx = a.ld; d.xb = (long)s.H * s.W * a.ld; d.x_coff = a.coff; d.H = s.H; d.W = s.W;
                    d.Wfrag = x->down_ds_w[i].frag[x->lpi()].p; d.bias = x->down_ds_b[i];
                    d.Y = s.ds_out; d.c_lp = g.c_lp; d.ldy = s.C; d.y_coff = 0;
                    d.inmask = mask; d.inmask_ws = s.mask_ws; d.mask_bstride = P.d.T; d.B = B;
                    const double M = 0.25 * s.H * s.W * B;
                    run("downsample", 2.0 * M * s.C * 9 * s.C, 4.0 * M * s.C * (g.a_lp ? 2.0 : 4.0) + M * s.C * (g.c_lp ? 2.0 : 4.0), [&] { launch_conv_down(d, x->precision, st); });
                } else
                gemm("downsample", g);
                cur = TD{s.ds_out, s.C, 0, s.C, t2_lp ? lpk : 0};
                if (debug && !x->lp()) { char nd[24]; snprintf(nd, sizeof nd, "downs.%d.3", i); tap(nd, s.ds_out, (long)B * g.Ho * g.Wo, s.C, s.C); }
            }
        }
        const StageBuf& sm = P.down[ns - 1];
        TD mid_in{sm.attn_out, sm.attn_ld, sm.attn_coff, sm.C};
        float* dit_dst = P.cat[0];
        const int dit_ld = 2 * sm.C;
        if (c.variant == DEX_VARIANT_DEX) {
            dex_adaptors(mid_in, sm.mask_ws);
            TD t{tiv_fold() ? P.tv_out : P.tiv_out, sm.C, 0, sm.C};
            dit(t, false, sm.mask_ws, dit_dst, dit_ld, 0, tiv_fold() ? P.tiv_aff : nullptr);
        } else {
            dit(mid_in, true, sm.mask_ws, dit_dst, dit_ld, 0);
        }
        tap("dit_out", dit_dst, B * sm.npix, sm.C, dit_ld);
        bool up_out_lp = false;
        for (int j = 0; j < ns - 1; ++j) {
            const StageBuf& s = P.up[j];
            const int i = ns - 1 - j;
            TD X{P.cat[j], 2 * stage_dim(c, i), 0, 2 * stage_dim(c, i)};
            if (cat_lp && j == 0) X = TD{reinterpret_cast<float*>(P.cat16), 2 * stage_dim(c, i), 0, 2 * stage_dim(c, i), lpk};
            Pro t0{};
            const bool defer0 = x->lp() && conv3x3_bf16_tail_supported(s.C) && fast_conv(s.C, s.C) &&
                                x->up_res[j][0].wr;
            resblock(x->up_res[j][0], s, X, P.tadd_up[2 * j], s.r0out, false, nullptr, nullptr, defer0 ? &t0 : nullptr);
            TD r0{s.r0out, s.C, 0, s.C};
            LinKvCtxP tail{};
            const bool defer = linattn_fused(s.C);
            resblock(x->up_res[j][1], s, r0, P.tadd_up[2 * j + 1], s.r1out, false, defer ? &tail : nullptr, defer0 ? &t0 : nullptr);
            TD r1{s.r1out, s.C, 0, s.C};
            if (debug && !x->lp()) {
                char n0[24], n1[24]; snprintf(n0, sizeof n0, "ups.%d.0", j); snprintf(n1, sizeof n1, "ups.%d.1", j);
                tap(n0, s.r0out, B * s.npix, s.C, s.C); tap(n1, s.r1out, B * s.npix, s.C, s.C);
            }
            const bool t5_lp = lp_inter && linattn_fused(s.C) && linattn_out2_lp_out_supported((int)s.npix, B);
            linattn(x->up_lin[j], s, r1, s.attn_out, s.C, 0, defer ? &tail : nullptr, t5_lp);
            char nm[16]; snprintf(nm, sizeof nm, "up%d", j);
            tap(nm, s.attn_out, B * s.npix, s.C, s.C);
            float* dst; int ldd;
            if (j < ns - 2) { dst = P.cat[j + 1]; ldd = 2 * stage_dim(c, i - 1); } else { dst = P.up_out; ldd = s.C; }
            {
                IGemmP g = base_gemm(s.attn_out, s.C, 0, s.H, s.W, s.C, x->up_us_w[j][0], s.C, x->up_us_b[j], dst, ldd, 0);
                g.KH = 2; g.KW = 2; g.step_h = -1; g.step_w = -1; g.K = 4 * s.C; g.parity = 1;
                g.OHf = 2 * s.H; g.OWf = 2 * s.W; g.osh = 2; g.osw = 2;
                g.c_bstride = 4L * s.H * s.W * ldd;
                g.inmask = mask; g.inmask_ws = s.mask_ws;
                g.a_lp = t5_lp ? lpk : 0;
                up_out_lp = lp_inter && j == ns - 2 && conv3x3_res2_form(80, P.d.T, B);
                g.c_lp = up_out_lp ? lpk : 0;
                const bool strip_off = knob_off("DEX_CONVT_UP");
                if (x->lp() && x->up_us_w[j][0].frag[x->lpi()].p && !strip_off && convt_up_supported(s.C, s.H, s.W, s.C, ldd)) {
                    ConvTUpP u{};
                    u.X = s.attn_out; u.a_lp = g.a_lp; u.ldx = s.C; u.xb = (long)s.H * s.W * s.C; u.x_coff = 0; u.H = s.H; u.W = s.W;
                    for (int par = 0; par < 4; ++par) u.Wfrag[par] = x->up_us_w[j][par].frag[x->lpi()].p;
                    u.bias = x->up_us_b[j];
                    u.Y = dst; u.c_lp = g.c_lp; u.ldy = ldd; u.y_coff = 0;
                    u.inmask = mask; u.inmask_ws = s.mask_ws; u.mask_bstride = P.d.T; u.B = B;
                    const double M = 4.0 * s.H * s.W * B;
                    run("upsample_convT", 2.0 * M * s.C * 4 * s.C, M * s.C * (g.c_lp ? 2.0 : 4.0) + 0.25 * M * s.C * (g.a_lp ? 2.0 : 4.0),
                        [&] { launch_convt_up(u, x->precision, st); });
                } else gemm("upsample_convT", g);
            }
        }
        tap("up_out", P.up_out, (long)B * 80 * P.d.T, c.dim, c.dim);
        TD U{P.up_out, c.dim, 0, c.dim, up_out_lp ? lpk : 0};
        gnfix_t* stf = next_stats();
        const bool hfb = h_bf16() && fast_conv(c.dim, c.dim);
        conv3x3("conv3x3", U, 80, P.d.T, 1, true, x->fin_w, x->fin_b, c.dim, P.hF, stf, nullptr, nullptr, nullptr, false, hfb);
        FinalGP f{};
        f.x_bf16 = hfb ? x->lp_kind() : 0;
        f.X = P.hF; f.xb = 80L * P.d.T * c.dim; f.npix = 80 * P.d.T; f.W = P.d.T; f.C = c.dim; f.groups = 8; f.stats = stf;
        f.gamma = x->fin_g; f.beta = x->fin_be; f.mask = mask; f.mask_bstride = P.d.T; f.wfc = x->fconv_w; f.bfc = x->fconv_b;
        f.xcur = xcur; f.denoised = denoised; f.xnext = xnext; f.scal = P.scal; f.scal_stride = SCAL_STRIDE; f.step = sp; f.row_bstride = rbs; f.B = B;
        f.zero_ptr = reinterpret_cast<float*>(stats_other); f.zero_n = P.stats_bytes / (long)sizeof(float);
        f.poison = P.xflag ? reinterpret_cast<const int*>(P.xflag + (P.xflag_bytes - sizeof(int)) / sizeof(unsigned)) : nullptr;
        f.mode = up.mode; f.htab = up.htab; f.dbuf = P.dbuf; f.xhat = P.xbuf;
        f.gtab = up.gtab; f.xstate = up.xstate; f.xin_next = up.xin_next;
        FinalMP fm{};
        static_cast<FinalP&>(fm) = f;
        fm.mtab = up.mtab; fm.dprev_in = up.dprev_in; fm.dprev_out = up.dprev_out;
        run("final_conv_euler", 14.0 * 80 * P.d.T * c.dim * B, 80.0 * P.d.T * ((hfb ? 2.0 : 4.0) * c.dim + 12.0) * B,
            [&] { if (up.mtab) launch_final_multistep(fm, st); else if (up.gtab) launch_final_general(f, st); else launch_final(f, st); });
    }

    void prepare(const float* sigmas_dev, int n, bool levels = false) {
        const DexConfig& c = x->cfg;
        const int dim = c.dim, hid = c.dit_hidden, B = P.d.B, mid = mid_dim(c);
        auto R = [&](const std::string& k) { return x->raw.at(k).p; };
        auto lin = [&](const float* X, int ldx, int rows, int K, const std::string& w, bool bias, int N, float* Y, int ai, int ao) {
            SmallLinP s{X, ldx, rows, K, R(w + ".weight"), bias ? R(w + ".bias") : nullptr, N, Y, N, ai, ao};
            run("cond_mlp", 2.0 * rows * K * N, 4.0 * K * N, [&] { launch_small_linear(s, st); });
        };
        if (P.tv_stats) zero_fill(P.tv_stats, (size_t)B * mid_dim(c) * IN_SLOTS * 2 * 2 * sizeof(gnfix_t), st);
        if (P.xflag) zero_fill(P.xflag, P.xflag_bytes, st);
        zero_fill(P.vt, P.vt_bytes, st);
        zero_fill(P.vt2, P.vt_bytes, st);
        CondPrepP cp{sigmas_dev, n, c.pe_scale, dim, P.scal, SCAL_STRIDE, P.t_unet, P.t_dit, levels ? 1 : 0};
        run("cond_prep", 0, 0, [&] { launch_cond_prep(cp, st); });
        lin(P.t_unet, dim, n, dim, "mlp.0", true, 4 * dim, P.tmp_u, 0, 1);
        lin(P.tmp_u, 4 * dim, n, 4 * dim, "mlp.2", true, dim, P.temb, 0, 0);
        for (int i = 0; i < c.n_stages; ++i)
            for (int r = 0; r < 2; ++r)
                lin(P.temb, dim, n, dim, "downs." + std::to_string(i) + "." + std::to_string(r) + ".mlp.1", true, stage_dim(c, i), P.tadd_down[2 * i + r], 1, 0);
        for (int j = 0; j < c.n_stages - 1; ++j)
            for (int r = 0; r < 2; ++r)
                lin(P.temb, dim, n, dim, "ups." + std::to_string(j) + "." + std::to_string(r) + ".mlp.1", true, stage_dim(c, c.n_stages - 2 - j), P.tadd_up[2 * j + r], 1, 0);
        lin(P.t_dit, 256, n, 256, "vit.t_embedder.mlp.0", true, hid, P.c_tmp, 0, 2);
        lin(P.c_tmp, hid, n, hid, "vit.t_embedder.mlp.2", true, hid, P.c_emb, 0, 0);
        for (int k = 0; k < c.dit_depth; ++k)
            lin(P.c_emb, hid, n, hid, "vit.blocks." + std::to_string(k) + ".adaLN_modulation.1", true, 6 * hid, P.ada[k], 2, 0);
        lin(P.c_emb, hid, n, hid, "vit.final_layer.adaLN_modulation.1", true, 2 * hid, P.fin_mod, 2, 0);
        if (c.n_spks > 1) {
            lin(args->spk_dev, c.spk_emb_dim, B, c.spk_emb_dim, "spk_mlp.0", true, 4 * c.spk_emb_dim, P.spk_tmp, 0, 1);
            lin(P.spk_tmp, 4 * c.spk_emb_dim, B, 4 * c.spk_emb_dim, "spk_mlp.2", true, c.n_feats, P.spk_plane, 0, 0);
        }
        if (c.variant == DEX_VARIANT_DEX) {
            lin(P.t_unet, dim, n, dim, "mlp_adap.0", true, dim, P.adap_tmp, 0, 1);
            lin(P.adap_tmp, dim, n, dim, "mlp_adap.2", true, 2 * dim, P.t_adap, 0, 0);
            lin(P.t_unet, dim, n, dim, "mlp_adap_sty.0", true, dim, P.adap_tmp, 0, 1);
            lin(P.adap_tmp, dim, n, dim, "mlp_adap_sty.2", true, 2 * dim, P.t_sty, 0, 0);
            lin(P.t_sty, mid, n, mid, "tv_adaptor.w_k", false, mid, P.tv_k0, 0, 0);
            lin(P.t_sty, mid, n, mid, "tv_adaptor.w_v", false, mid, P.tv_v0, 0, 0);
            const int L = args->n_ref;
            for (int j = 0; j < L; ++j)
                run("ref_stats", 0, 4.0 * B * mid * args->Tr, [&] {
                    launch_row_stats(args->ref_skips_dev[j], B, mid, args->Tr, 1e-5f, P.ref_mean + (long)j * mid, P.ref_std + (long)j * mid, (long)L * mid, st);
                });
            SapP sm{P.t_adap, 2 * dim, 0, n, P.ref_mean, L, mid, R("tiv_adaptor.mean_sap.W.weight"), R("tiv_adaptor.mean_sap.W.bias"), P.sap_m, B};
            SapP ss{P.t_adap, 2 * dim, 0, n, P.ref_std, L, mid, R("tiv_adaptor.std_sap.W.weight"), R("tiv_adaptor.std_sap.W.bias"), P.sap_s, B};
            run("sap_pool", 0, 0, [&] { launch_sap(sm, st); launch_sap(ss, st); });
            run("sty_transpose", 0, 8.0 * B * mid * args->Ts, [&] { launch_transpose_cl(args->sty_dev, P.tv_keys, B, mid, args->Ts, 0, (long)args->Ts * mid, st); });
            for (int which = 0; which < 2; ++which) {
                float* dst = which ? P.tv_V : P.tv_K;
                IGemmP g = base_gemm(P.tv_keys, mid, 0, 1, args->Ts, mid, which ? x->tv_wv : x->tv_wk, mid, nullptr, dst + mid, mid, 0);
                g.c_bstride = (long)(args->Ts + 1) * mid;
                gemm("tv_kv", g);
            }
            if (tv_chain_on()) {
                TvKvPrepP kp{P.tv_K, P.tv_V, (long)(args->Ts + 1) * mid, args->Ts + 1, P.tv_nkpad, P.tv_kp, P.tv_vtp, B};
                run("tv_kv_operands", 0, 12.0 * B * (args->Ts + 1) * mid, [&] { launch_tv_kv_prep(kp, x->precision, st); });
            }
            if (tv_fold_on()) {
                const long kvb = (long)(args->Ts + 1) * mid;
                for (int which = 0; which < 2; ++which) {
                    IGemmP g = base_gemm((which ? P.tv_V : P.tv_K) + mid, mid, 0, 1, args->Ts, mid, which ? x->tv_wl.f32 : x->tv_wq_raw, mid, nullptr,
                                         (which ? P.tv_Vp : P.tv_G) + mid, mid, 0);
                    g.a_bstride = kvb; g.c_bstride = kvb;
                    gemm("tv_fold_kv", g);
                    IGemmP t = base_gemm(which ? P.tv_v0 : P.tv_k0, mid, 0, 1, n, mid, which ? x->tv_wl.f32 : x->tv_wq_raw, mid, nullptr, which ? P.tv_v0p : P.tv_g0, mid, 0);
                    t.B = 1;
                    gemm("tv_fold_time_rows", t);
                }
                TvKvPrepP kp{P.tv_G, P.tv_Vp, kvb, args->Ts + 1, P.tv_nkpad, P.tv_kp, P.tv_vtp, B};
                run("tv_fold_operands", 0, 6.0 * B * (args->Ts + 1) * mid, [&] { launch_tv_vfrag_prep(kp, x->precision, st); });
            }
        }
    }
};

int validate(DexCtx* x, const DexSampleArgs* a, bool need_z) {
    if (!x || !a) return DEX_ERR_ARG;
    if (!x->finalized) return x->fail(DEX_ERR_STATE, "dex_ctx_finalize has not been called");
    if (a->B < 1 || a->T < 4 || (a->T % 4) != 0) return x->fail(DEX_ERR_ARG, "T (%d) must be a positive multiple of 4 (fix_len_compatibility), B >= 1", a->T);
    if ((a->T >> (x->cfg.n_stages - 1)) * (1 << (x->cfg.n_stages - 1)) != a->T) return x->fail(DEX_ERR_ARG, "T must be divisible by 2^(n_stages-1)");
    if (need_z && a->n_steps < 2) return x->fail(DEX_ERR_ARG, "n_steps must be >= 2 (edm.py:157 divides by num_steps - 1)");
    const bool tables = need_z && a->tables;
    if (!a->mu_dev || !a->mask_dev || (!a->sigmas_dev && !tables) || !a->out_dev || !a->workspace_dev) return x->fail(DEX_ERR_ARG, "null device pointer");
    if (need_z && !a->z_dev) return x->fail(DEX_ERR_ARG, "z_dev is null");
    if (need_z && !tables && a->S_churn < 0.f) return x->fail(DEX_ERR_ARG, "S_churn must be >= 0");
    if (need_z && !tables && a->S_churn > 0.f && !a->noise_dev) return x->fail(DEX_ERR_ARG, "S_churn > 0 needs noise_dev ([n_steps][B,80,T] draws of randn_like, edm.py:196)");
    if (tables) {
        const DexSamplerTables* tb = a->tables;
        if (!tb->sigma_dev || !tb->coef_dev || !tb->step_dev) return x->fail(DEX_ERR_ARG, "DexSamplerTables: null table pointer");
        if (tb->n_rows != dex_num_evals(a->n_steps, a->solver))
            return x->fail(DEX_ERR_ARG, "DexSamplerTables: n_rows (%d) must be dex_num_evals(n_steps, solver) = %d", tb->n_rows, dex_num_evals(a->n_steps, a->solver));
        if (tb->flags & ~(uint32_t)(DEX_TABLES_SCALED | DEX_TABLES_CHURN)) return x->fail(DEX_ERR_ARG, "DexSamplerTables: unknown flags 0x%x", tb->flags);
    }
    if (x->cfg.n_spks > 1 && !a->spk_dev) return x->fail(DEX_ERR_ARG, "spk_dev required when n_spks > 1");
    if (x->cfg.variant == DEX_VARIANT_DEX) {
        if (!a->ref_skips_dev || !a->sty_dev || !a->sty_lengths_dev || a->Tr < 2 || a->Ts < 1 || a->n_ref < 1 || a->n_ref > 7)
            return x->fail(DEX_ERR_ARG, "DEX needs ref_skips_dev (1..7 tensors, Tr >= 2), sty_dev, sty_lengths_dev, Ts >= 1");
        for (int j = 0; j < a->n_ref; ++j) if (!a->ref_skips_dev[j]) return x->fail(DEX_ERR_ARG, "ref_skips_dev[%d] is null", j);
    }
    if (((uintptr_t)a->workspace_dev & 255) != 0) return x->fail(DEX_ERR_ARG, "workspace must be 256-byte aligned");
    return DEX_OK;
}

__global__ void set_sigma_pair(const float* src, float* dst) { dst[0] = src[0]; dst[1] = 0.f; }

struct Eval {
    const float* xin;
    float* xout;
    Update up;
    int noise_step = -1;
};

struct SamplerKind {
    const DexSamplerTables* tb;
    bool heun, multistep, churn, scaled;
    int n, E;
    explicit SamplerKind(const DexSampleArgs* a)
// ... 373 lines not shown
```

dex_tts_amd/csrc/kernels.h:

```cpp
#pragma once
#include <hip/hip_runtime.h>
#include <stdint.h>

namespace dex {

constexpr int KNOB_UNSET = -2147483647 - 1;
int knob(const char* name);
inline int knob_or(const char* name, int dflt) { const int v = knob(name); return v == KNOB_UNSET ? dflt : v; }
inline bool knob_off(const char* name) { return knob(name) == 0; }
inline bool knob_set(const char* name) { return knob(name) != KNOB_UNSET; }
inline int device_cus() {
    static const int n = [] { int dev = 0, v = 0; (void)hipGetDevice(&dev); (void)hipDeviceGetAttribute(&v, hipDeviceAttributeMultiprocessorCount, dev); return v > 0 ? v : 256; }();
    return n;
}

constexpr int GN_SLOTS = 32;
typedef long long gnfix_t;

extern thread_local const char* g_last_symbol;

constexpr int PREC_FP32 = 0, PREC_BF16 = 1, PREC_FP16 = 2, PREC_FP16X2 = 3;
inline bool prec_wsplit(int precision) { return precision == PREC_FP16X2; }
extern thread_local bool g_lp_wsplit;
inline bool prec_is_lp(int precision) { return precision != PREC_FP32; }

struct IGemmP {
    const float* A; int lda; long a_bstride; int a_coff;
    int Hi, Wi, Cin;
    int KH, KW, sh, sw, off_h, off_w, step_h, step_w;
    int Ho, Wo;
    const float* W; long w_bstride; long w_gstride;
    const void* Wbf;
    const void* Wfrag = nullptr;
    long w_lo_off = 0;
    int N, K, ksplit, groups;
    const float* bias; long bias_bstride;
    float* C; int ldc; long c_bstride; long c_sstride; int c_coff;
    int OHf, OWf, osh, osw, oh0, ow0;
    const float* inmask; int inmask_ws;
    const float* outmask; int outmask_ws;
    long mask_bstride;
    int act;
    float act_in_slope;
    const float* gate; int gate_nstride; long gate_step_stride;
    const float* res; int ldres; long res_bstride; int res_coff;
    int step;
    int row_bstride = 0;
    int unpatch_s, unpatch_C;
    int parity;
    gnfix_t* gn_stats; int gn_groups, gn_cpg;
    int stats_final;
    const float* ln_shift; const float* ln_scale; long ln_step_stride;
    int B;
    int a_lp, c_lp;
};
void launch_igemm(const IGemmP& p, int precision, hipStream_t st);

struct ConvTUpP { const void* X; int a_lp; int ldx; long xb; int x_coff; int H, W;
                  const void* Wfrag[4]; const float* bias;
                  void* Y; int c_lp; int ldy; int y_coff;
                  const float* inmask; int inmask_ws; long mask_bstride; int B;
                  int nseg, rows_per_wg; };
bool convt_up_supported(int C, int H, int W, int ldx, int ldy);
struct ConvDownP { const void* X; int a_lp; int ldx; long xb; int x_coff; int H, W;
                   const void* Wfrag; const float* bias;
                   void* Y; int c_lp; int ldy; int y_coff;
                   const float* inmask; int inmask_ws; long mask_bstride; int B;
                   int nseg, rows_per_wg; };
bool conv_down_supported(int C, int H, int W, int ldx, int ldy, int x_coff);
void launch_conv_down(const ConvDownP& p, int precision, hipStream_t st);
void launch_convt_up(const ConvTUpP& p, int precision, hipStream_t st);

struct Conv3P {
    const float* X; int ldx; int x_coff; int H, W, Cin, Cout;
    const void* Wbf; const float* bias; float* Y;
    const void* Wfrag;
    const float* mask; int mask_ws; long mask_bstride;
    const gnfix_t* pro_stats; const float* pro_gamma; const float* pro_beta; const float* pro_tadd;
    const float* pro_res; float* pro_xout;
    int xout_lp;
    const float *res2_w, *res2_b, *res2_mu, *res2_x, *res2_spk, *res2_scal; int res2_scal_stride, res2_planes;
    const void* res_w; const float* res_b; float* res_y;
    const void* res_wfrag;
    int step; gnfix_t* gn_stats; int B;
    long long* dbg;
    int x_bf16, y_bf16;
    long w_lo_off = 0, res_lo_off = 0;
    int row_bstride = 0;
    int skip_dead = 0;
};
bool conv3x3_bf16_supported(int Cin, int Cout);
bool conv3x3_bf16_tail_supported(int C);
bool conv3x3_bf16_res_supported(int Cin, int Cout);
bool conv3x3_bf16_xb_supported(int Cin, int Cout);
bool conv3x3_plain_lp_in_supported(int H, int W, int B, int Cin, int Cout);
bool igemm_nwalk_form(const IGemmP& p);
bool conv3x3_cat_lp_in_supported(int H, int W, int B, int Cin, int Cout);
bool conv3x3_strip_form(const Conv3P& p);
bool conv3x3_res2_form(int H, int W, int B);
void launch_conv3x3_lp(const Conv3P& p, int precision, hipStream_t st);

struct FirstConvP {
    const float* mu; const float* x; const float* spk;
    const float* mask; int B, H, T, planes, C;
    const float* W3; const float* b3;
    const float* W1; const float* b1;
    const float* scal; int scal_stride; int step;
    float* h1; float* res;
    int h1_bf16;
    gnfix_t* gn_stats;
    int row_bstride = 0;
};
void launch_first_conv(const FirstConvP& p, hipStream_t st);

struct GnStatsP { const float* X; int ld; long bstride; int npix; int C; int groups; gnfix_t* stats; int B; };
void launch_gn_stats(const GnStatsP& p, hipStream_t st);

struct GnApplyP {
    const float* X; int ldx; long xb;
    float* Y; int ldy; long yb; int y_coff;
    int npix, W, C, groups; const gnfix_t* stats; const float* gamma; const float* beta;
    const float* mask; int mask_ws; long mask_bstride;
    const float* tadd; long tadd_step_stride; int step;
    const float* res; int ldres; long resb; int res_under_mask;
    int B;
    int row_bstride = 0;
};
void launch_gn_apply(const GnApplyP& p, hipStream_t st);

struct FinalP {
    const float* X; long xb; int npix, W, C, groups; const gnfix_t* stats; const float* gamma; const float* beta;
    const float* mask; long mask_bstride;
    const float* wfc; const float* bfc;
    const float* xcur;
    float* denoised;
    float* xnext;
    const float* scal; int scal_stride; int step;
    float* zero_ptr; long zero_n;
    int B;
    int mode; const float* htab; float* dbuf; const float* xhat;
    int x_bf16;
    const int* poison;
    int row_bstride = 0;
};
void launch_final(const FinalP& p, hipStream_t st);
struct FinalGP : FinalP {
    const float* gtab; const float* xstate; float* xin_next;
};
void launch_final_general(const FinalGP& p, hipStream_t st);
struct FinalMP : FinalP {
    const float* mtab; const float* dprev_in; float* dprev_out;
};
void launch_final_multistep(const FinalMP& p, hipStream_t st);
void launch_ablation_churn(float* x, const float* noise, const float* rk, float* xin, const float* s, long n, hipStream_t st);
void launch_ablation_init(const float* z, float* x, const float* c0, float* xin, const float* s, long n, hipStream_t st);
void launch_churn_tables(const float* sigmas, int n, float S_churn, float S_min, float S_max, float S_noise,
                         float* t_hat, float* h, float* ncoef, hipStream_t st);
void launch_add_noise(float* x, const float* noise, const float* ncoef_i, long n, hipStream_t st);
void launch_heun_expand(const float* t_hat, const float* h, int n, float* sig, float* hout, hipStream_t st);

struct LinAttnCtxP { const float* qkv; int ld; long bstride; int n; int heads; int chunk; int nchunks;
                     float* part_m; float* part_s; float* part_c; int B; };
void launch_linattn_ctx(const LinAttnCtxP& p, hipStream_t st);
struct LinAttnCombineP { const float* part_m; const float* part_s; const float* part_c; int nchunks; int heads;
                         const float* Wout;
                         const float* g;
                         int C; float* Weff;
                         int B; };
void launch_linattn_combine(const LinAttnCombineP& p, hipStream_t st);

struct LinKvCtxP { const float* X; int ldx; int x_coff; long xb; int npix; int C; const void* Wkv; int nsub; int nblk;
                   float* part_m; float* part_s; float* part_c; int B;
                   const float* H2; const gnfix_t* gn_stats; const float* gamma; const float* beta;
                   const float* res; int ldres; long resb; int res_under_mask;
                   const float* mask; int mask_ws; long mask_bstride; int W; float* Xout;
                   int h2_bf16;
                   int res_lp;
                   int xout_lp;     long wkv_lo_off = 0;
                   int headwaves = 0;
                   int rows = 0;
                   long long* dbg = nullptr;
};
void launch_linattn_kvctx(const LinKvCtxP& p, int precision, hipStream_t st);
struct LinMergeP { const float* part_m; const float* part_s; const float* part_c; int nblk;
                   const float* Wout; const float* g; int C; void* W2; int B; };
void launch_linattn_merge(const LinMergeP& p, int precision, hipStream_t st);
struct LinOut2P { const float* X; int ldx; int x_coff; long xb; int npix; int C; const void* Wq; const void* W2;
                  const float* bias; float* Y; int ldy; int y_coff; long yb; int B;
                  int y_lp;
                  void* Y2; int ldy2; int y2_coff; long y2b;
                  int x_lp;     long wq_lo_off = 0;
                  int hw = 0;
                  int rows = 0;
                  long long* dbg = nullptr;
                  };
void launch_linattn_out2(const LinOut2P& p, int precision, hipStream_t st);
bool linattn_out2_lp_out_supported(int npix, int B);
bool linattn_fused_supported(int C);

struct DwConvP { const float* X; int ldx; long xb; int Hi, Wi, C; int k, s, pad; const float* Wd; const float* bd;
                 const float* mask; int mask_ws; long mask_bstride;
                 float* Y; int Hf, Wt; int B;
                 const float* aff = nullptr; };
void launch_dwconv_silu(const DwConvP& p, hipStream_t st);
bool patch_embed_fused_supported(int k, int C, int hid, long ntok);
void launch_patch_embed_fused(const DwConvP& p, const void* Wb, const float* bias, float* emb, int hid, int precision, hipStream_t st);

struct PosConvP { const float* X; const void* Wf; float* Y; int Hf, Wt, hid, G, B;
                  int ncol; };
bool pos_conv_direct_supported(int hid, int groups, int kernel, int Hf);
void launch_pos_conv_direct(const PosConvP& p, int precision, hipStream_t st);
struct PosFinishP { const float* part; int nsplit; long split_stride; const float* bias; const float* emb;
                    const float* freq_pos; float* tok; int Hf, Wt, D; int B;
                    int cg, cg_pad; };
void launch_pos_finish(const PosFinishP& p, hipStream_t st);
void launch_group_pad(const float* src, float* dst, long rows, int G, int cg, int cg_pad, hipStream_t st);

struct LnModP { const float* X; float* Y; int rows_per_batch; int D; const float* shift; const float* scale;
                long step_stride; int step; int B; int row_bstride = 0; };
void launch_ln_mod(const LnModP& p, hipStream_t st);

struct DitChainP { const float* O; int ksplit; long o_sstride; const float* ml; int heads; int rows_per_batch;
                   float* X; const void *Wp, *W1, *W2, *Wq; const float *bp, *b1, *b2, *bq;
                   const float* ada;
                   const float *next_shift, *next_scale; long next_step_stride;
                   void *Qh, *Kh, *Vt; int Npad; float qscale;
                   const void *Qin, *Kin, *Vin;
                   int qkv_only;
                   int attn_inline;
                   int step; int M; int B; long long* dbg;
                   float* xslab; unsigned* xflag; unsigned epoch; int* xerr;
                   int o_lp;
                   int xcd_map;
                   int xlocal;
                   int xdrop;
                   int tail_row0 = 0, tail_ks = 0;
                   int row_bstride = 0;
                   int xcds = 8; };
constexpr int DIT_CLUSTER = 4;
constexpr size_t DIT_CLUSTER_SLAB_FLOATS = 2 * DIT_CLUSTER * (32 * 256 + 256);
constexpr size_t DIT_CLUSTER_FLAG_WORDS = 2 * DIT_CLUSTER;
bool dit_rowchain64_form(int rows_per_batch, int B, int attn_inline);
bool dit_rowchain_cluster_form(int rows_per_batch, int B);
bool dit_rowchain_cluster_local_fits(int rows_per_batch, int B);
int dit_rowchain_cluster_xcds(int rows_per_batch, int B);
bool dit_rowchain_supported(int hidden, int mlp_hidden);
struct AttnDirectP { const void *Qh, *Kh, *Vt; int N, Npad, B; float* O; long o_sstride; float* ml; int ksplit; long long* dbg;
                     int o_lp;
                     int xcd_map;
                     int tail_g = 0, tail_ks = 0;
                     int half_g = 0, half_n = 0; };
void launch_attention_direct(const AttnDirectP& p, int precision, hipStream_t st);
bool attention_direct_batch_regime(int N, int B);
int attention_direct_ksplit(int N, int B);
void launch_attention_q64(const AttnDirectP& p, int precision, hipStream_t st);
int attention_q64_ksplit(int N, int B, int max_split);
void attention_q64_plan(int N, int B, int max_split, int* ks, int* tail_g, int* tail_ks);
bool attention_q64_half_plan(int N, int B, int* half_g, int* half_n);
void launch_dit_rowchain(const DitChainP& p, int precision, hipStream_t st);
void launch_pack_lp_frag(const float* src, void* dst, int K, int N, int precision, hipStream_t st);
void launch_pack_lp_frag_nk(const float* src, void* dst, int K, int N, int precision, hipStream_t st);

struct AttnP { const float* Q; int ldq; long qb; const float* K; int ldk; long kb; const float* V; int ldv; long vb;
               float* O; int ldo; long ob; int Nq, Nk; const int* kv_len; int kv_len_add; int heads; float scale; int B;
               int ksplit; long o_sstride; float* ml;
               long long* dbg;
               int head_dim;
               int force_generic;
               int o_lp; };
inline bool dit_sep64_small_n(int N, int B) {
    if (N < 512 || N >= 1024) return false;
    const long t = (long)B * ((N + 63) / 64), r = (t + 255) / 256;
    return t >= 256 && t * 100 >= r * 256 * 65;
}
bool attention_lp_shared_form(int Nq, int heads, int B, int ksplit);
bool attention_head_dim_supported(int hd);
void launch_attention(const AttnP& p, int precision, hipStream_t st);

struct SmallLinP { const float* X; int ldx; int rows; int K; const float* W; const float* bias; int N;
                   float* Y; int ldy; int act_in; int act_out; };
void launch_small_linear(const SmallLinP& p, hipStream_t st);

struct CondPrepP { const float* sigmas; int n; float pe_scale; int dim; float* scal; int scal_stride;
                   float* t_unet; float* t_dit;
                   int no_next = 0; };
void launch_cond_prep(const CondPrepP& p, hipStream_t st);

void launch_scale_copy(const float* src, float* dst, long n, const float* scal_ptr, hipStream_t st);
void launch_step_reset(int* step, hipStream_t st);
void launch_step_inc(int* step, hipStream_t st);
void launch_iota(int* dst, int n, hipStream_t st);
void launch_permute4(const float* src, float* dst, int d0, int d1, int d2, int d3, int p0, int p1, int p2, int p3,
                     hipStream_t st);
void launch_f32_residual_lp(const float* src, float* dst, long n, int precision, hipStream_t st);
void launch_f32_to_lp(const float* src, void* dst, long n, int precision, hipStream_t st);
void launch_pack_lp_nk(const float* src, void* dst, int K, int N, int precision, hipStream_t st);
void launch_spk_plane(const float* spk_out, float* plane, int B, int F, hipStream_t st);

void launch_row_stats(const float* X, int B, int C, int len, float eps, float* mean, float* std, long out_bstride, hipStream_t st);
constexpr int IN_SLOTS = GN_SLOTS;
struct InStatsP { const float* X; int ld; long bstride; int npix; int C; gnfix_t* stats; int B;
                  const float* mask; int mask_ws; long mask_bstride; int W; };
void launch_in_stats(const InStatsP& p, hipStream_t st);
struct SapP { const float* t_tok; int t_ld; int t_coff; int nsteps; const float* stats; int L; int C;
              const float* w; const float* bias; float* out; int B; };
void launch_sap(const SapP& p, hipStream_t st);
struct InFoldP { const gnfix_t* stats; int npix; float eps; const float* Wq; int C; float* Weff; float* beff; int B;
                 void* Wbf; int lp; int split = 0; };
void launch_in_fold(const InFoldP& p, hipStream_t st);
struct TivApplyP { const float* X; int ld; long xb; float* Y; int ldy; long yb; int npix; int C; const gnfix_t* stats;
                   float eps; const float* s_tab; const float* m_tab; int step; int B;
                   int row_bstride = 0; };
void launch_tiv_apply(const TivApplyP& p, hipStream_t st);
void launch_tiv_coef(const TivApplyP& p, float* aff, hipStream_t st);
struct TvRow0P { const float* k0; const float* v0; int step; float* K; float* V; long kvb; int C; int B;
                 float* zero_ptr; long zero_n;
                 void* Kp = nullptr; void* VTp = nullptr; int NkPad = 0; int lp_kind = 0;
                 int row_bstride = 0; };
void launch_tv_row0(const TvRow0P& p, hipStream_t st);
struct TvKvPrepP { const float* K; const float* V; long kvb; int Nk; int NkPad; void* Kp; void* VTp; int B; };
struct TvChainP { const float* X; int ldx; int x_coff; long x_bstride; int npix; int Wm;
                  const float* mask; int mask_ws; long mask_bstride;
                  const void* Weff; long weff_lo_off; const float* beff;
                  const void* Wl; long wl_lo_off;
                  const void* Kp; const void* VTp; int NkPad; int Nk; const int* kv_len; int kv_len_add; float scale;
                  float* out; gnfix_t* stats; int B;
                  const float* xmean = nullptr; float* zero_ptr = nullptr; long zero_n = 0; };
struct TvFold2P { const gnfix_t* stats; int npix; float eps; const float* G; long gb; const float* g0; const float* v0p; int step;
                  int Nk; int NkPad; int C; float scale; void* Kp; void* VTp; float* xmean; float* zero_ptr; long zero_n; int lp_kind; int B;
                  int row_bstride = 0; };
void launch_tv_fold2(const TvFold2P& p, hipStream_t st);
bool tv_chain_form(int npix, int C, int B);
void launch_tv_kv_prep(const TvKvPrepP& p, int precision, hipStream_t st);
void launch_tv_vfrag_prep(const TvKvPrepP& p, int precision, hipStream_t st);
void launch_tv_chain(const TvChainP& p, int precision, hipStream_t st);
void launch_transpose_cl(const float* src, float* dst, int B, int C, int L, int row_off, long dst_bstride, hipStream_t st);

void launch_mel_to_cl(const float* mel, float* out, int B, int C, int T, int ldc, hipStream_t st, const int* len = nullptr);
void launch_voc_len_mask(const int* len, float* mask, int B, int T, int R, hipStream_t st);
void launch_voc_window_len(const int* len, int* wlen, int B, int T, int lo, int W, hipStream_t st);
void launch_mel_window_to_cl(const float* mel, float* out, int B, int C, int T, int lo, int W, int ldc, const int* wlen, hipStream_t st);
void launch_voc_window_crop(const float* src, long src_bstride, long off, float* dst, long dst_bstride, long n, int B, hipStream_t st);
struct ConvTFoldP { const float* Y; const float* bias; float* out; int L, Cout, k, u, pad, B; const int* len; int R; };
void launch_convt_fold(const ConvTFoldP& p, hipStream_t st);
void launch_avg3(const float* a, const float* b, const float* c, float* out, long n, hipStream_t st);
struct ConvPostP { const float* X; const float* W; const float* bias; float* wav; int L, C, B; float slope; const int* len; int R; };
struct AaSnakeP { const float* X; float* Y; int L, C, B; const float* a; const float* inv_b; const float* filt; const int* len; int R; };
void launch_aa_snake(const AaSnakeP& p, hipStream_t st);
void launch_snake_coeffs(const float* alpha, const float* beta, float* a, float* inv_b, int C, int logscale, hipStream_t st);
void launch_conv_post_tanh(const ConvPostP& p, hipStream_t st);
// ... 50 lines not shown
```

dex_tts_amd/csrc/kernels_lp.h:

```cpp
#include "kernels.h"
#include "lp_config.h"

namespace dex {
namespace DEX_LP_NS {

bool conv3x3_bf16_supported(int Cin, int Cout);
bool conv3x3_bf16_tail_supported(int C);
bool conv3x3_bf16_res_supported(int Cin, int Cout);
bool conv3x3_bf16_xb_supported(int Cin, int Cout);
void launch_conv3x3_lp(const Conv3P& p, hipStream_t st);
int conv3x3_stream_tiles(const Conv3P& p);
void launch_conv3x3_stream(const Conv3P& p, int tiles_per_wg, hipStream_t st);
bool conv3x3_regw_form(const Conv3P& p);
void launch_conv3x3_regw(const Conv3P& p, hipStream_t st);
bool linattn_out2_lp_out_supported(int npix, int B);
bool linattn_fused_supported(int C);
bool conv3x3_plain_lp_in_supported(int H, int W, int B, int Cin, int Cout);
bool conv3x3_res2_form(int H, int W, int B);
void launch_igemm_lp(const IGemmP& p, hipStream_t st);
bool attention_lp_shared_form(int Nq, int heads, int B, int ksplit);
bool igemm_nwalk_form(const IGemmP& p);
bool conv3x3_cat_lp_in_supported(int H, int W, int B, int Cin, int Cout);
bool convt_up_supported(int C, int H, int W, int ldx, int ldy);
void launch_convt_up(const ConvTUpP& p, hipStream_t st);
bool conv_down_supported(int C, int H, int W, int ldx, int ldy, int x_coff);
void launch_conv_down(const ConvDownP& p, hipStream_t st);
void launch_attention_lp(const AttnP& p, hipStream_t st);
void launch_attention_direct(const AttnDirectP& p, hipStream_t st);
bool tv_chain_form(int npix, int C, int B);
void launch_tv_kv_prep(const TvKvPrepP& p, hipStream_t st);
void launch_tv_vfrag_prep(const TvKvPrepP& p, hipStream_t st);
void launch_tv_chain(const TvChainP& p, hipStream_t st);
bool attention_direct_batch_regime(int N, int B);
int attention_direct_ksplit(int N, int B);
void launch_attention_q64(const AttnDirectP& p, hipStream_t st);
int attention_q64_ksplit(int N, int B, int max_split);
void attention_q64_plan(int N, int B, int max_split, int* ks, int* tail_g, int* tail_ks);
bool attention_q64_half_plan(int N, int B, int* half_g, int* half_n);
bool dit_rowchain_supported(int hidden, int mlp_hidden);
bool dit_rowchain64_form(int rows_per_batch, int B, int attn_inline);
bool dit_rowchain_cluster_form(int rows_per_batch, int B);
bool dit_rowchain_cluster_local_fits(int rows_per_batch, int B);
int dit_rowchain_cluster_xcds(int rows_per_batch, int B);
void launch_dit_rowchain(const DitChainP& p, hipStream_t st);
void launch_pack_lp_frag(const float* src, void* dst, int K, int N, hipStream_t st);
void launch_pack_lp_frag_nk(const float* src, void* dst, int K, int N, hipStream_t st);
void launch_linattn_kvctx(const LinKvCtxP& p, hipStream_t st);
void launch_linattn_merge(const LinMergeP& p, hipStream_t st);
void launch_linattn_out2(const LinOut2P& p, hipStream_t st);
bool patch_embed_fused_supported(int k, int C, int hid, long ntok);
void launch_patch_embed_fused(const DwConvP& p, const void* Wb, const float* bias, float* emb, int hid, hipStream_t st);
bool pos_conv_direct_supported(int hid, int groups, int kernel, int Hf);
void launch_pos_conv_direct(const PosConvP& p, hipStream_t st);

}
}
```

dex_tts_amd/csrc/linattn_fused.hip:

```cpp
#include "kernels.h"
#include "lp_util.h"
#include "kernels_lp.h"

namespace dex {
namespace DEX_LP_NS {

typedef float f32x16 __attribute__((ext_vector_type(16)));
typedef unsigned short u16;
union LFrag { uint4 u; lp8 v; };
constexpr float LOG2E_F = 1.4426950408889634f;


#ifdef DEX_TIMING
#define KSTAMP_DECL long long tk[8] = {0, 0, 0, 0, 0, 0, 0, 0}; const long long tk0 = __builtin_readcyclecounter(); long long tlast = tk0;
#define KSTAMP(k) do { const long long now_ = __builtin_readcyclecounter(); tk[k] += now_ - tlast; tlast = now_; } while (0)
#define KSTAMP_STORE(n)                                                                                               \
    if (p.dbg && threadIdx.x == 0) {                                                                                  \
        long long* d_ = p.dbg + ((long)blockIdx.y * gridDim.x + blockIdx.x) * 8;                                      \
        for (int k_ = 0; k_ < (n); ++k_) d_[k_] = tk[k_];                                                             \
        d_[7] = __builtin_readcyclecounter() - tk0;                                                                   \
    }
#else
#define KSTAMP_DECL
#define KSTAMP(k) do {} while (0)
// ... 815 lines not shown
        }
        KSTAMP(5);
    }
    KSTAMP_STORE(7)
}

template <int C, bool ROWS = false>
__global__ __launch_bounds__(256) void linattn_out2_hw_kernel(const LinOut2P p) {
    constexpr int KS1 = C / 16, CT = C / 32, KQ = KS1 / 4;
    constexpr int O8 = C / 8, XH = ROWS ? 33 : 32, LDY = C + 4;
    __shared__ uint4 xs[KS1][2 * XH], qs[8][64];
    __shared__ __attribute__((aligned(16))) float ys[ROWS ? 32 * LDY : 4];
    KSTAMP_DECL
    const int tid = threadIdx.x, lane = tid & 63;
    const int t = __builtin_amdgcn_readfirstlane(tid >> 6);
    const int i = lane & 31, hh = lane >> 5;
    const int fi = hh * XH + i;
    const int b = blockIdx.y;
    const int px0 = blockIdx.x * 32;
    if (px0 >= p.npix) return;
    const float* X = p.X + (long)b * p.xb + p.x_coff;
    const int px = min(px0 + i, p.npix - 1);
    const int rp0 = 8 * t + lane / O8, rch = 8 * (lane % O8);
    float4 xa[KQ], xc[KQ];
    if constexpr (ROWS) {
#pragma unroll
        for (int k = 0; k < KQ; ++k) {
            const float* xr = X + (long)min(px0 + rp0 + k * (64 / O8), p.npix - 1) * p.ldx + rch;
            xa[k] = *reinterpret_cast<const float4*>(xr);
            xc[k] = *reinterpret_cast<const float4*>(xr + 4);
        }
    } else {
        const float* xr = X + (long)px * p.ldx + hh * 8;
#pragma unroll
        for (int k = 0; k < KQ; ++k) {
            const int ks = t * KQ + k;
            xa[k] = *reinterpret_cast<const float4*>(xr + ks * 16);
            xc[k] = *reinterpret_cast<const float4*>(xr + ks * 16 + 4);
        }
    }
    const uint4* wq = reinterpret_cast<const uint4*>(p.Wq) + lane;
    uint4 wqf[KS1];
#ifdef DEX_LP_WSPLIT
    uint4 wql[KS1];
#endif
#pragma unroll
    for (int ks = 0; ks < KS1; ++ks) {
        wqf[ks] = wq[(t * KS1 + ks) * 64];
#ifdef DEX_LP_WSPLIT
        wql[ks] = wq[(t * KS1 + ks) * 64 + p.wq_lo_off / 8];
#endif
    }
    const bool g2 = t < CT;
    const int ct = g2 ? t : 0;
    const uint4* w2 = reinterpret_cast<const uint4*>(p.W2) + (long)b * CT * 8 * 64 + lane;
    uint4 w2f[8];
    float4 res[4], bia[4];
    if (g2) {
#pragma unroll
        for (int ks = 0; ks < 8; ++ks) w2f[ks] = w2[(ct * 8 + ks) * 64];
    }
    if constexpr (ROWS) {
        bia[0] = *reinterpret_cast<const float4*>(p.bias + rch);
        bia[1] = *reinterpret_cast<const float4*>(p.bias + rch + 4);
    } else if (g2) {
        if constexpr (C != 128) {
#pragma unroll
            for (int g4 = 0; g4 < 4; ++g4) res[g4] = *reinterpret_cast<const float4*>(X + (long)px * p.ldx + ct * 32 + 8 * g4 + 4 * hh);
        }
        const float4* bt = reinterpret_cast<const float4*>(p.bias + ct * 32);
        const unsigned hm = 0u - (unsigned)hh;
#pragma unroll
        for (int g4 = 0; g4 < 4; ++g4) {
            const float4 b0 = bt[2 * g4], b1 = bt[2 * g4 + 1];
            bia[g4] = make_float4(__uint_as_float((__float_as_uint(b1.x) & hm) | (__float_as_uint(b0.x) & ~hm)),
                                  __uint_as_float((__float_as_uint(b1.y) & hm) | (__float_as_uint(b0.y) & ~hm)),
                                  __uint_as_float((__float_as_uint(b1.z) & hm) | (__float_as_uint(b0.z) & ~hm)),
                                  __uint_as_float((__float_as_uint(b1.w) & hm) | (__float_as_uint(b0.w) & ~hm)));
        }
    }
    KSTAMP(0);
#pragma unroll
    for (int k = 0; k < KQ; ++k) {
        LFrag f;
        f.u.x = pack2_lp(xa[k].x, xa[k].y); f.u.y = pack2_lp(xa[k].z, xa[k].w);
        f.u.z = pack2_lp(xc[k].x, xc[k].y); f.u.w = pack2_lp(xc[k].z, xc[k].w);
        if constexpr (ROWS) xs[rch >> 4][((rch >> 3) & 1) * XH + rp0 + k * (64 / O8)] = f.u;
        else xs[t * KQ + k][fi] = f.u;
    }
    if constexpr (C == 128 && !ROWS) {
#pragma unroll
        for (int k = 0; k < 2; ++k) {
            const float4 snd = hh ? xa[k] : xc[k];
            float4 rcv;
            rcv.x = __shfl_xor(snd.x, 32); rcv.y = __shfl_xor(snd.y, 32); rcv.z = __shfl_xor(snd.z, 32); rcv.w = __shfl_xor(snd.w, 32);
            res[2 * k] = hh ? rcv : xa[k];
            res[2 * k + 1] = hh ? xc[k] : rcv;
        }
    }
    lds_barrier();
    KSTAMP(1);
    {
        f32x16 q;
#pragma unroll
        for (int r = 0; r < 16; ++r) q[r] = 0.f;
#pragma unroll
        for (int ks = 0; ks < KS1; ++ks) {
            LFrag af, xf; af.u = wqf[ks]; xf.u = xs[ks][fi];
            q = DEX_MFMA_LP(af.v, xf.v, q, 0, 0, 0);
#ifdef DEX_LP_WSPLIT
            LFrag al; al.u = wql[ks];
            q = DEX_MFMA_LP(al.v, xf.v, q, 0, 0, 0);
#endif
        }
#pragma unroll
        for (int k2 = 0; k2 < 2; ++k2) {
            LFrag f;
            f.u.x = pack2_lp(q[8 * k2 + 0], q[8 * k2 + 1]); f.u.y = pack2_lp(q[8 * k2 + 2], q[8 * k2 + 3]);
            f.u.z = pack2_lp(q[8 * k2 + 4], q[8 * k2 + 5]); f.u.w = pack2_lp(q[8 * k2 + 6], q[8 * k2 + 7]);
            qs[t * 2 + k2][lane] = f.u;
        }
    }
    KSTAMP(2);
    lds_barrier();
    KSTAMP(3);
    if constexpr (!ROWS) { if (!g2) return; }
    f32x16 y;
    if (g2) {
#pragma unroll
        for (int r = 0; r < 16; ++r) y[r] = 0.f;
#pragma unroll
        for (int ks = 0; ks < 8; ++ks) {
            LFrag af, qf; af.u = w2f[ks]; qf.u = qs[ks][lane];
            y = DEX_MFMA_LP(af.v, qf.v, y, 0, 0, 0);
        }
    }
    KSTAMP(4);
    float* Y = p.Y + (long)b * p.yb + p.y_coff;
    if constexpr (ROWS) {
        if (g2) {
#pragma unroll
            for (int g4 = 0; g4 < 4; ++g4)
                *reinterpret_cast<float4*>(ys + i * LDY + ct * 32 + 8 * g4 + 4 * hh) = make_float4(y[g4 * 4 + 0], y[g4 * 4 + 1], y[g4 * 4 + 2], y[g4 * 4 + 3]);
        }
        lds_barrier();
#pragma unroll
        for (int k = 0; k < KQ; ++k) {
            const int rp = rp0 + k * (64 / O8);
            const float4 ya = *reinterpret_cast<const float4*>(ys + rp * LDY + rch), yc = *reinterpret_cast<const float4*>(ys + rp * LDY + rch + 4);
            if (px0 + rp < p.npix) {
                float4 oa, oc;
                oa.x = ya.x + xa[k].x + bia[0].x; oa.y = ya.y + xa[k].y + bia[0].y; oa.z = ya.z + xa[k].z + bia[0].z; oa.w = ya.w + xa[k].w + bia[0].w;
                oc.x = yc.x + xc[k].x + bia[1].x; oc.y = yc.y + xc[k].y + bia[1].y; oc.z = yc.z + xc[k].z + bia[1].z; oc.w = yc.w + xc[k].w + bia[1].w;
                float* yr = Y + (long)(px0 + rp) * p.ldy + rch;
                *reinterpret_cast<float4*>(yr) = oa;
                *reinterpret_cast<float4*>(yr + 4) = oc;
            }
        }
    } else if (px0 + i < p.npix) {
#pragma unroll
        for (int g4 = 0; g4 < 4; ++g4) {
            const int co = ct * 32 + 8 * g4 + 4 * hh;
            float4 o;
            o.x = y[g4 * 4 + 0] + res[g4].x + bia[g4].x; o.y = y[g4 * 4 + 1] + res[g4].y + bia[g4].y;
            o.z = y[g4 * 4 + 2] + res[g4].z + bia[g4].z; o.w = y[g4 * 4 + 3] + res[g4].w + bia[g4].w;
            *reinterpret_cast<float4*>(Y + (long)(px0 + i) * p.ldy + co) = o;
        }
    }
    KSTAMP(5);
    KSTAMP_STORE(7)
}
template <int C>
__global__ __launch_bounds__(256) __attribute__((amdgpu_waves_per_eu(2, C == 64 ? 4 : 2))) void linattn_out2_kernel(const LinOut2P p) {
    constexpr int KS1 = C / 16, CT = C / 32;
    constexpr int LDX = C + 4;
    constexpr int NCH = 32 * C / 4 / 64;
    extern __shared__ __attribute__((aligned(16))) float smem_o2[];
    const int tid = threadIdx.x, lane = tid & 63, wave = tid >> 6;
    const int i = lane & 31, hh = lane >> 5;
    const int b = blockIdx.y;
    const int px0 = (blockIdx.x * 4 + wave) * 32;
    if (px0 >= p.npix) return;
    float* xs = smem_o2 + wave * 32 * LDX;
    const float* X = p.X + (long)b * p.xb + p.x_coff;
    float4 xin[NCH];
    const bool xlp = p.x_lp != 0;
    if (xlp) {
        const u16* Xh = reinterpret_cast<const u16*>(p.X) + (long)b * p.xb + p.x_coff;
#pragma unroll
        for (int k = 0; k < NCH / 2; ++k) {
            const int c = lane + 64 * k, px = c / (C / 8), ch = (c % (C / 8)) * 8;
            xin[k] = *reinterpret_cast<const float4*>(Xh + (long)min(px0 + px, p.npix - 1) * p.ldx + ch);
        }
    } else {
#pragma unroll
        for (int k = 0; k < NCH; ++k) {
            const int c = lane + 64 * k, px = c / (C / 4), ch = (c % (C / 4)) * 4;
            xin[k] = *reinterpret_cast<const float4*>(X + (long)min(px0 + px, p.npix - 1) * p.ldx + ch);
        }
    }
    const uint4* w2 = reinterpret_cast<const uint4*>(p.W2) + (long)b * CT * 8 * 64 + lane;
    uint4 w2f[CT][8];
#pragma unroll
    for (int ct = 0; ct < CT; ++ct)
#pragma unroll
        for (int ks = 0; ks < 8; ++ks) w2f[ct][ks] = w2[(ct * 8 + ks) * 64];
    if (xlp) {
#pragma unroll
        for (int k = 0; k < NCH / 2; ++k) {
            const int c = lane + 64 * k, px = c / (C / 8), ch = (c % (C / 8)) * 8;
            const unsigned u0 = __float_as_uint(xin[k].x), u1 = __float_as_uint(xin[k].y), u2 = __float_as_uint(xin[k].z), u3 = __float_as_uint(xin[k].w);
            *reinterpret_cast<float4*>(xs + px * LDX + ch) = make_float4(lp_lo(u0), lp_hi(u0), lp_lo(u1), lp_hi(u1));
            *reinterpret_cast<float4*>(xs + px * LDX + ch + 4) = make_float4(lp_lo(u2), lp_hi(u2), lp_lo(u3), lp_hi(u3));
        }
    } else {
#pragma unroll
        for (int k = 0; k < NCH; ++k) {
            const int c = lane + 64 * k, px = c / (C / 4), ch = (c % (C / 4)) * 4;
            *reinterpret_cast<float4*>(xs + px * LDX + ch) = xin[k];
        }
    }
    __builtin_amdgcn_wave_barrier();
    LFrag xf[KS1];
#pragma unroll
    for (int ks = 0; ks < KS1; ++ks) {
        const float4 xa = *reinterpret_cast<const float4*>(xs + i * LDX + ks * 16 + hh * 8);
        const float4 xc = *reinterpret_cast<const float4*>(xs + i * LDX + ks * 16 + hh * 8 + 4);
        xf[ks].u.x = pack2_lp(xa.x, xa.y); xf[ks].u.y = pack2_lp(xa.z, xa.w);
        xf[ks].u.z = pack2_lp(xc.x, xc.y); xf[ks].u.w = pack2_lp(xc.z, xc.w);
    }
    const uint4* wq = reinterpret_cast<const uint4*>(p.Wq) + lane;
    LFrag qf[8];
#pragma unroll
    for (int t = 0; t < 4; ++t) {
        f32x16 q;
#pragma unroll
        for (int r = 0; r < 16; ++r) q[r] = 0.f;
#pragma unroll
        for (int ks = 0; ks < KS1; ++ks) {
            LFrag af; af.u = wq[(t * KS1 + ks) * 64];
            q = DEX_MFMA_LP(af.v, xf[ks].v, q, 0, 0, 0);
#ifdef DEX_LP_WSPLIT
            LFrag al; al.u = wq[(t * KS1 + ks) * 64 + p.wq_lo_off / 8];
            q = DEX_MFMA_LP(al.v, xf[ks].v, q, 0, 0, 0);
#endif
        }
#pragma unroll
        for (int k2 = 0; k2 < 2; ++k2) {
            qf[t * 2 + k2].u.x = pack2_lp(q[8 * k2 + 0], q[8 * k2 + 1]); qf[t * 2 + k2].u.y = pack2_lp(q[8 * k2 + 2], q[8 * k2 + 3]);
            qf[t * 2 + k2].u.z = pack2_lp(q[8 * k2 + 4], q[8 * k2 + 5]); qf[t * 2 + k2].u.w = pack2_lp(q[8 * k2 + 6], q[8 * k2 + 7]);
        }
    }
#pragma unroll
    for (int ct = 0; ct < CT; ++ct) {
        f32x16 y;
#pragma unroll
        for (int r = 0; r < 16; ++r) y[r] = 0.f;
#pragma unroll
        for (int ks = 0; ks < 8; ++ks) {
            LFrag af; af.u = w2f[ct][ks];
            y = DEX_MFMA_LP(af.v, qf[ks].v, y, 0, 0, 0);
        }
#pragma unroll
        for (int g4 = 0; g4 < 4; ++g4) {
            const int co = ct * 32 + 8 * g4 + 4 * hh;
            float* slot = xs + i * LDX + co;
            const float4 res = *reinterpret_cast<const float4*>(slot);
            const float4 bia = *reinterpret_cast<const float4*>(p.bias + co);
            float4 o;
            o.x = y[g4 * 4 + 0] + res.x + bia.x; o.y = y[g4 * 4 + 1] + res.y + bia.y;
            o.z = y[g4 * 4 + 2] + res.z + bia.z; o.w = y[g4 * 4 + 3] + res.w + bia.w;
            *reinterpret_cast<float4*>(slot) = o;
        }
    }
    __builtin_amdgcn_wave_barrier();
    float* Y = p.Y + (long)b * p.yb + p.y_coff;
#pragma unroll
    for (int k = 0; k < NCH; ++k) {
        const int c = lane + 64 * k, px = c / (C / 4), ch = (c % (C / 4)) * 4;
        const float4 o = *reinterpret_cast<const float4*>(xs + px * LDX + ch);
        if (px0 + px < p.npix) {
            if (p.y_lp) {
                u16* yh = reinterpret_cast<u16*>(p.Y) + (long)b * p.yb + p.y_coff + (long)(px0 + px) * p.ldy + ch;
                *reinterpret_cast<uint2*>(yh) = make_uint2(pack2_lp(o.x, o.y), pack2_lp(o.z, o.w));
            } else *reinterpret_cast<float4*>(Y + (long)(px0 + px) * p.ldy + ch) = o;
            if (p.Y2) {
                u16* y2 = reinterpret_cast<u16*>(p.Y2) + (long)b * p.y2b + p.y2_coff + (long)(px0 + px) * p.ldy2 + ch;
                *reinterpret_cast<uint2*>(y2) = make_uint2(pack2_lp(o.x, o.y), pack2_lp(o.z, o.w));
            }
        }
    }
}
bool linattn_fused_supported(int C) {
#if defined(DEX_LP_WSPLIT) && !defined(DEX_WS_HAVE_LINATTN)
    return false;
#endif
    return C == 64 || C == 128;
}
static long out2_min_wgs() { return knob_or("DEX_OUT2_MIN", 256); }
bool linattn_out2_lp_out_supported(int npix, int B) { return (long)((npix + 127) / 128) * B >= out2_min_wgs(); }
void launch_linattn_out2(const LinOut2P& p, hipStream_t st) {
    dim3 grid((p.npix + 127) / 128, p.B);
    const size_t lds = (size_t)4 * 32 * (p.C + 4) * sizeof(float);
    static bool attr = false;
    if (!attr) {
        hipFuncSetAttribute(reinterpret_cast<const void*>(&linattn_out2_kernel<128>), hipFuncAttributeMaxDynamicSharedMemorySize, (int)((size_t)4 * 32 * 132 * sizeof(float)));
        attr = true;
    }
    const bool lp_io = p.x_lp || p.y_lp || p.Y2;
    if (p.hw && !lp_io) {
        g_last_symbol = "linattn_out2_hw_kernel";
        const dim3 g1((p.npix + 31) / 32, p.B);
        if (p.rows) {
            if (p.C == 64) hipLaunchKernelGGL((linattn_out2_hw_kernel<64, true>), g1, dim3(256), 0, st, p);
            else hipLaunchKernelGGL((linattn_out2_hw_kernel<128, true>), g1, dim3(256), 0, st, p);
            return;
        }
        if (p.C == 64) hipLaunchKernelGGL((linattn_out2_hw_kernel<64, false>), g1, dim3(256), 0, st, p);
        else hipLaunchKernelGGL((linattn_out2_hw_kernel<128, false>), g1, dim3(256), 0, st, p);
        return;
    }
    if ((long)grid.x * p.B < out2_min_wgs()) {
        if (p.C == 64) hipLaunchKernelGGL(linattn_out2_direct_kernel<64>, grid, dim3(256), 0, st, p);
        else hipLaunchKernelGGL(linattn_out2_direct_kernel<128>, grid, dim3(256), 0, st, p);
        return;
    }
    if (p.C == 64) hipLaunchKernelGGL(linattn_out2_kernel<64>, grid, dim3(256), lds, st, p);
    else hipLaunchKernelGGL(linattn_out2_kernel<128>, grid, dim3(256), lds, st, p);
}

}
}
```

dex_tts_amd/csrc/lp_dispatch.hip:

```cpp
#include "kernels.h"

#include "kernels_lp.h"
#undef DEX_LP_NS
#define DEX_LP_NS f16
#include "kernels_lp.h"
#undef DEX_LP_NS
#define DEX_LP_NS f16w
#include "kernels_lp.h"
#undef DEX_LP_NS

namespace dex {

thread_local const char* g_last_symbol = nullptr;
thread_local bool g_lp_wsplit = false;

bool conv3x3_bf16_supported(int Cin, int Cout) { return (g_lp_wsplit ? f16w::conv3x3_bf16_supported(Cin, Cout) : bf16::conv3x3_bf16_supported(Cin, Cout)); }
bool conv3x3_bf16_tail_supported(int C) { return (g_lp_wsplit ? f16w::conv3x3_bf16_tail_supported(C) : bf16::conv3x3_bf16_tail_supported(C)); }
bool conv3x3_bf16_res_supported(int Cin, int Cout) { return (g_lp_wsplit ? f16w::conv3x3_bf16_res_supported(Cin, Cout) : bf16::conv3x3_bf16_res_supported(Cin, Cout)); }
bool conv3x3_bf16_xb_supported(int Cin, int Cout) { return (g_lp_wsplit ? f16w::conv3x3_bf16_xb_supported(Cin, Cout) : bf16::conv3x3_bf16_xb_supported(Cin, Cout)); }
bool conv3x3_plain_lp_in_supported(int H, int W, int B, int Cin, int Cout) { return (g_lp_wsplit ? f16w::conv3x3_plain_lp_in_supported(H, W, B, Cin, Cout) : bf16::conv3x3_plain_lp_in_supported(H, W, B, Cin, Cout)); }
bool linattn_out2_lp_out_supported(int npix, int B) { return (g_lp_wsplit ? f16w::linattn_out2_lp_out_supported(npix, B) : bf16::linattn_out2_lp_out_supported(npix, B)); }
bool linattn_fused_supported(int C) { return (g_lp_wsplit ? f16w::linattn_fused_supported(C) : bf16::linattn_fused_supported(C)); }
bool conv3x3_res2_form(int H, int W, int B) { return (g_lp_wsplit ? f16w::conv3x3_res2_form(H, W, B) : bf16::conv3x3_res2_form(H, W, B)); }
bool attention_lp_shared_form(int Nq, int heads, int B, int ksplit) { return (g_lp_wsplit ? f16w::attention_lp_shared_form(Nq, heads, B, ksplit) : bf16::attention_lp_shared_form(Nq, heads, B, ksplit)); }
bool igemm_nwalk_form(const IGemmP& p) { return (g_lp_wsplit ? f16w::igemm_nwalk_form(p) : bf16::igemm_nwalk_form(p)); }
bool conv3x3_cat_lp_in_supported(int H, int W, int B, int Cin, int Cout) { return (g_lp_wsplit ? f16w::conv3x3_cat_lp_in_supported(H, W, B, Cin, Cout) : bf16::conv3x3_cat_lp_in_supported(H, W, B, Cin, Cout)); }
bool conv3x3_strip_form(const Conv3P& p) { return (g_lp_wsplit ? f16w::conv3x3_stream_tiles(p) : bf16::conv3x3_stream_tiles(p)) != 0 || (g_lp_wsplit ? f16w::conv3x3_regw_form(p) : bf16::conv3x3_regw_form(p)); }
bool pos_conv_direct_supported(int hid, int groups, int kernel, int Hf) { return (g_lp_wsplit ? f16w::pos_conv_direct_supported(hid, groups, kernel, Hf) : bf16::pos_conv_direct_supported(hid, groups, kernel, Hf)); }
bool tv_chain_form(int npix, int C, int B) { return (g_lp_wsplit ? f16w::tv_chain_form(npix, C, B) : bf16::tv_chain_form(npix, C, B)); }
bool attention_direct_batch_regime(int N, int B) { return (g_lp_wsplit ? f16w::attention_direct_batch_regime(N, B) : bf16::attention_direct_batch_regime(N, B)); }
int attention_direct_ksplit(int N, int B) { return (g_lp_wsplit ? f16w::attention_direct_ksplit(N, B) : bf16::attention_direct_ksplit(N, B)); }
int attention_q64_ksplit(int N, int B, int max_split) { return (g_lp_wsplit ? f16w::attention_q64_ksplit(N, B, max_split) : bf16::attention_q64_ksplit(N, B, max_split)); }
void attention_q64_plan(int N, int B, int max_split, int* ks, int* tail_g, int* tail_ks) { (g_lp_wsplit ? f16w::attention_q64_plan(N, B, max_split, ks, tail_g, tail_ks) : bf16::attention_q64_plan(N, B, max_split, ks, tail_g, tail_ks)); }
bool conv_down_supported(int C, int H, int W, int ldx, int ldy, int x_coff) { return (g_lp_wsplit ? f16w::conv_down_supported(C, H, W, ldx, ldy, x_coff) : bf16::conv_down_supported(C, H, W, ldx, ldy, x_coff)); }
bool convt_up_supported(int C, int H, int W, int ldx, int ldy) { return (g_lp_wsplit ? f16w::convt_up_supported(C, H, W, ldx, ldy) : bf16::convt_up_supported(C, H, W, ldx, ldy)); }
bool patch_embed_fused_supported(int k, int C, int hid, long ntok) { return (g_lp_wsplit ? f16w::patch_embed_fused_supported(k, C, hid, ntok) : bf16::patch_embed_fused_supported(k, C, hid, ntok)); }
bool dit_rowchain_supported(int hidden, int mlp_hidden) { return (g_lp_wsplit ? f16w::dit_rowchain_supported(hidden, mlp_hidden) : bf16::dit_rowchain_supported(hidden, mlp_hidden)); }
bool dit_rowchain64_form(int rows_per_batch, int B, int attn_inline) { return (g_lp_wsplit ? f16w::dit_rowchain64_form(rows_per_batch, B, attn_inline) : bf16::dit_rowchain64_form(rows_per_batch, B, attn_inline)); }
bool dit_rowchain_cluster_form(int rows_per_batch, int B) { return (g_lp_wsplit ? f16w::dit_rowchain_cluster_form(rows_per_batch, B) : bf16::dit_rowchain_cluster_form(rows_per_batch, B)); }
int dit_rowchain_cluster_xcds(int rows_per_batch, int B) { return bf16::dit_rowchain_cluster_xcds(rows_per_batch, B); }
bool dit_rowchain_cluster_local_fits(int rows_per_batch, int B) { return (g_lp_wsplit ? f16w::dit_rowchain_cluster_local_fits(rows_per_batch, B) : bf16::dit_rowchain_cluster_local_fits(rows_per_batch, B)); }

#define DEX_LP_CALL(fn, ...) do { if (precision == PREC_FP16X2) f16w::fn(__VA_ARGS__); else if (precision == PREC_FP16) f16::fn(__VA_ARGS__); else bf16::fn(__VA_ARGS__); } while (0)

void launch_conv3x3_lp(const Conv3P& p, int precision, hipStream_t st) { DEX_LP_CALL(launch_conv3x3_lp, p, st); }
void launch_igemm_lp(const IGemmP& p, int precision, hipStream_t st) { DEX_LP_CALL(launch_igemm_lp, p, st); }
void launch_convt_up(const ConvTUpP& p, int precision, hipStream_t st) { DEX_LP_CALL(launch_convt_up, p, st); }
void launch_conv_down(const ConvDownP& p, int precision, hipStream_t st) { DEX_LP_CALL(launch_conv_down, p, st); }
void launch_attention_lp(const AttnP& p, int precision, hipStream_t st) { DEX_LP_CALL(launch_attention_lp, p, st); }
void launch_tv_kv_prep(const TvKvPrepP& p, int precision, hipStream_t st) { DEX_LP_CALL(launch_tv_kv_prep, p, st); }
void launch_tv_vfrag_prep(const TvKvPrepP& p, int precision, hipStream_t st) { DEX_LP_CALL(launch_tv_vfrag_prep, p, st); }
void launch_tv_chain(const TvChainP& p, int precision, hipStream_t st) { DEX_LP_CALL(launch_tv_chain, p, st); }
void launch_attention_direct(const AttnDirectP& p, int precision, hipStream_t st) { DEX_LP_CALL(launch_attention_direct, p, st); }
bool attention_q64_half_plan(int N, int B, int* half_g, int* half_n) { return bf16::attention_q64_half_plan(N, B, half_g, half_n); }
void launch_attention_q64(const AttnDirectP& p, int precision, hipStream_t st) { DEX_LP_CALL(launch_attention_q64, p, st); }
void launch_dit_rowchain(const DitChainP& p, int precision, hipStream_t st) { DEX_LP_CALL(launch_dit_rowchain, p, st); }
void launch_pack_lp_frag(const float* src, void* dst, int K, int N, int precision, hipStream_t st) { DEX_LP_CALL(launch_pack_lp_frag, src, dst, K, N, st); }
void launch_pack_lp_frag_nk(const float* src, void* dst, int K, int N, int precision, hipStream_t st) { DEX_LP_CALL(launch_pack_lp_frag_nk, src, dst, K, N, st); }
void launch_linattn_kvctx(const LinKvCtxP& p, int precision, hipStream_t st) { DEX_LP_CALL(launch_linattn_kvctx, p, st); }
void launch_linattn_merge(const LinMergeP& p, int precision, hipStream_t st) { DEX_LP_CALL(launch_linattn_merge, p, st); }
void launch_linattn_out2(const LinOut2P& p, int precision, hipStream_t st) { DEX_LP_CALL(launch_linattn_out2, p, st); }
void launch_pos_conv_direct(const PosConvP& p, int precision, hipStream_t st) { DEX_LP_CALL(launch_pos_conv_direct, p, st); }
void launch_patch_embed_fused(const DwConvP& p, const void* Wb, const float* bias, float* emb, int hid, int precision, hipStream_t st) { DEX_LP_CALL(launch_patch_embed_fused, p, Wb, bias, emb, hid, st); }

}
```

Before: 29590 mel-frames/s.

## Extend bf16 activation handoffs to small-grid conv and linear-attention tail forms

Rewrites conv3x3 dispatch as a table of built forms that can be queried, so the planner knows when a 16-bit input form exists. It also adds bf16 output paths to the row-wise linear-attention tail kernel. With these, the B=1 small-grid stages (down, cat, up, attention tails) can hand off bf16 activations instead of fp32, cutting memory traffic and conversion passes. New small-form conv instantiations are compiled in, and launches with no built form now abort instead of falling back.

Result: no change. 29790 mel-frames/s, median of 5 (+0.7%).

```diff
diff --git a/dex_tts_amd/csrc/conv3x3_bf16.hip b/dex_tts_amd/csrc/conv3x3_bf16.hip
--- a/dex_tts_amd/csrc/conv3x3_bf16.hip
+++ b/dex_tts_amd/csrc/conv3x3_bf16.hip
@@ -4,6 +4,10 @@
 #include "lp_util.h"
 #include "kernels_lp.h"
 #include "conv_gn.h"
+
+#ifndef DEX_C3_CAT16_NPASS
+#define DEX_C3_CAT16_NPASS 2
+#endif
 
 namespace dex {
 namespace DEX_LP_NS {
@@ -138,7 +142,7 @@
     constexpr int RING = CC == 128 ? (PRO2 ? 1 : 2) : 3;
     constexpr int NPASS = RW ? 1
                         : TH == 5 ? (CC == 128 ? (PRO2 ? 6 : 3) : (PRO2 ? 3 : XB ? 1 : 2))
-                                  : CC == 128 ? (TH == 8 ? (PRO2 ? 8 : 4) : (PRO2 ? 5 : 2)) : (PRO2 ? 3 : 1);
+                                  : CC == 128 ? (TH == 8 ? (PRO2 ? 8 : 4) : (PRO2 ? 5 : (XB && RES && TH == 2) ? DEX_C3_CAT16_NPASS : 2)) : (PRO2 ? 3 : 1);
     constexpr int NIP = (NI + NPASS - 1) / NPASS;
     constexpr int RWI = 9 * WITEMS;
     constexpr int RWPT = (RWI + NTHR - 1) / NTHR;
@@ -512,31 +516,11 @@
     return (Cin == 64 || Cin == 128 || Cin == 256) && (Cout == 64 || Cout == 128);
 }
 
-bool conv3x3_plain_lp_in_supported(int H, int W, int B, int Cin, int Cout) {
-#if defined(DEX_LP_WSPLIT) && !defined(DEX_WS_HAVE_CONV3)
-    return false;
-#endif
-   
-    const int w8 = knob_or("DEX_CONV_W8", 1);
-    const long tiles4 = (long)((W + 31) / 32) * ((H + 3) / 4) * B;
-    return w8 && tiles4 >= 256 && Cin == 64 && Cout == 128;
-}
-
-bool conv3x3_cat_lp_in_supported(int H, int W, int B, int Cin, int Cout) {
-#if defined(DEX_LP_WSPLIT) && !defined(DEX_WS_HAVE_CONV3_RES)
-    return false;
-#endif
-   
-    if (Cout != 64 || Cin < 128 || Cin % 128 != 0) return false;
-    const int w8 = knob_or("DEX_CONV_W8", 1);
-    const long small_max = knob_or("DEX_CONV_SMALL_MAX", 256);
-    const long tiles4 = (long)((W + 31) / 32) * ((H + 3) / 4) * B;
-    return w8 && tiles4 >= small_max;
-}
+struct C3Form { int cc, nsl, th; bool pro2, res; int nw; bool rw; };
 
 static bool conv3x3_resident_on() { return knob_or("DEX_CONV_RESIDENT", 1) != 0; }
 
-static bool launch_c3_round1(const Conv3P& p, bool small, hipStream_t st) {
+static bool c3_round1_form(const Conv3P& p, bool small, C3Form& f) {
     if (!knob_or("DEX_CONV_ROUND1", 1)) return false;
     const bool tail_ = p.pro_res != nullptr;
 #ifdef DEX_LP_WSPLIT
@@ -544,105 +528,156 @@
 #else
     const bool c64 = p.Cin == 64 && p.Cout == 64 && !p.res_w;
 #endif
-    const bool r128 = p.Cin == 64 && p.Cout == 128 && p.res_w && !tail_ && !p.x_bf16;
+    const bool r128 = p.Cin == 64 && p.Cout == 128 && p.res_w && !tail_;
     if (!c64 && !r128) return false;
     const long strips = (long)((p.W + 31) / 32) * p.B;
     const long cur = c64 ? strips * (small ? (p.H + 1) / 2 : (p.H + 3) / 4) : strips * (small ? (p.H + 1) / 2 * 2 : (p.H + 3) / 4);
     const long one = strips * ((p.H + 4) / 5) * (c64 ? 1 : 4);
     const long ncu = device_cus();
     if (cur <= ncu || one > ncu || one * 4 < ncu * 3) return false;
+    bool rw = false;
 #ifndef DEX_LP_WSPLIT
-    if (conv3x3_resident_on()) {
-        if (c64 && !tail_) {
-            p.x_bf16 ? launch_c3<64, 64, 64, 5, false, false, true, 10, true>(p, st) : launch_c3<64, 64, 64, 5, false, false, false, 10, true>(p, st);
-            return true;
-        }
-        if (!c64) { launch_c3<64, 128, 32, 5, false, true, false, 5, true>(p, st); return true; }
-    }
-#endif
-    if (c64) {
-#ifndef DEX_LP_WSPLIT
-        if (tail_) { p.x_bf16 ? launch_c3<64, 64, 64, 5, true, false, true, 10>(p, st) : launch_c3<64, 64, 64, 5, true, false, false, 10>(p, st); return true; }
-#endif
-        p.x_bf16 ? launch_c3<64, 64, 64, 5, false, false, true, 10>(p, st) : launch_c3<64, 64, 64, 5, false, false, false, 10>(p, st);
-    } else {
-        launch_c3<64, 128, 32, 5, false, true, false, 5>(p, st);
-    }
+    rw = conv3x3_resident_on() && !(c64 && tail_);
+#endif
+    f = c64 ? C3Form{64, 64, 5, tail_, false, 10, rw} : C3Form{64, 32, 5, false, true, 5, rw};
     return true;
 }
 
-static bool launch_c3_small_resident(const Conv3P& p, bool small, hipStream_t st) {
+static bool c3_small_resident(const Conv3P& p, bool small) {
 #ifdef DEX_LP_WSPLIT
     return false;
 #else
     if (!small || !conv3x3_resident_on() || p.Cin != 64 || p.Cout != 64 || p.res_w) return false;
-    if ((long)((p.W + 31) / 32) * ((p.H + 1) / 2) * p.B > device_cus()) return false;
-    const bool tail_ = p.pro_res != nullptr;
-    if (tail_) { p.x_bf16 ? launch_c3<64, 64, 64, 2, true, false, true, 4, true>(p, st) : launch_c3<64, 64, 64, 2, true, false, false, 4, true>(p, st); }
-    else { p.x_bf16 ? launch_c3<64, 64, 64, 2, false, false, true, 4, true>(p, st) : launch_c3<64, 64, 64, 2, false, false, false, 4, true>(p, st); }
-    return true;
-#endif
-}
-
-void launch_conv3x3_lp(const Conv3P& p, hipStream_t st) {
-    if (const int tpw = conv3x3_stream_tiles(p)) { launch_conv3x3_stream(p, tpw, st); return; }
-    if (conv3x3_regw_form(p)) { launch_conv3x3_regw(p, st); return; }
+    return (long)((p.W + 31) / 32) * ((p.H + 1) / 2) * p.B <= device_cus();
+#endif
+}
+
+static C3Form c3_tile_form(const Conv3P& p) {
     const bool tail_ = p.pro_res != nullptr;
     const long tiles4 = (long)((p.W + 31) / 32) * ((p.H + 3) / 4) * p.B;
     const long small_max = knob_or("DEX_CONV_SMALL_MAX", 256);
     const bool small = tiles4 < small_max;
     const int w8 = knob_or("DEX_CONV_W8", 1);
     const int th8 = knob_or("DEX_CONV_TH8", 1);
-    if (th8 && w8 && !small && !tail_ && p.Cin == 128 && p.Cout == 128 && !p.res_w && p.H % 8 == 0 && (long)((p.W + 31) / 32) * (p.H / 8) * p.B >= 512) {
-        p.x_bf16 ? launch_c3<128, 128, 128, 8, false, false, true, 8>(p, st) : launch_c3<128, 128, 128, 8, false, false, false, 8>(p, st);
-        return;
-    }
-    if (w8 && !small && p.Cin == 128 && p.Cout == 128 && !p.res_w) {
-        if (p.x_bf16) { tail_ ? launch_c3<128, 128, 128, 4, true, false, true, 8>(p, st) : launch_c3<128, 128, 128, 4, false, false, true, 8>(p, st); }
-        else { tail_ ? launch_c3<128, 128, 128, 4, true, false, false, 8>(p, st) : launch_c3<128, 128, 128, 4, false, false, false, 8>(p, st); }
-        return;
-    }
-    if (w8 && !small && p.res_w && p.Cout == 128 && p.Cin == 64) {
-        p.x_bf16 ? launch_c3<64, 128, 128, 4, false, true, true, 8>(p, st) : launch_c3<64, 128, 128, 4, false, true, false, 8>(p, st);
-        return;
-    }
-    if (th8 && w8 && !small && p.res_w && p.Cout == 64 && p.Cin >= 128 && !p.pro_stats && p.H % 8 == 0 && (long)((p.W + 31) / 32) * (p.H / 8) * p.B >= 512) {
-        p.x_bf16 ? launch_c3<128, 64, 64, 8, false, true, true, 8>(p, st) : launch_c3<128, 64, 64, 8, false, true, false, 8>(p, st);
-        return;
-    }
-    if (w8 && !small && p.res_w && p.Cout == 64 && p.Cin >= 128) {
-        p.x_bf16 ? launch_c3<128, 64, 64, 4, false, true, true, 8>(p, st) : launch_c3<128, 64, 64, 4, false, true, false, 8>(p, st);
-        return;
-    }
-    if (launch_c3_round1(p, small, st)) return;
-    if (launch_c3_small_resident(p, small, st)) return;
-    if (p.x_bf16) {
-        if (tail_) {
-            if (p.Cin == 64) { small ? launch_c3<64, 64, 64, 2, true, false, true>(p, st) : launch_c3<64, 64, 64, 4, true, false, true>(p, st); }
-            else { small ? launch_c3<128, 128, 64, 2, true, false, true>(p, st) : launch_c3<128, 128, 128, 4, true, false, true>(p, st); }
-        } else {
-            if (p.Cin == 64) { small ? launch_c3<64, 64, 64, 2, false, false, true>(p, st) : launch_c3<64, 64, 64, 4, false, false, true>(p, st); }
-            else { small ? launch_c3<128, 128, 64, 2, false, false, true>(p, st) : launch_c3<128, 128, 128, 4, false, false, true>(p, st); }
-        }
-        return;
-    }
-    if (tail_) {
-        if (p.Cin == 64 && p.Cout == 64) { small ? launch_c3<64, 64, 64, 2, true>(p, st) : launch_c3<64, 64, 64, 4, true>(p, st); }
-        else { small ? launch_c3<128, 128, 64, 2, true>(p, st) : launch_c3<128, 128, 128, 4, true>(p, st); }
-        return;
-    }
+    const bool rows8 = p.H % 8 == 0 && (long)((p.W + 31) / 32) * (p.H / 8) * p.B >= 512;
+    if (th8 && w8 && !small && !tail_ && p.Cin == 128 && p.Cout == 128 && !p.res_w && rows8) return C3Form{128, 128, 8, false, false, 8, false};
+    if (w8 && !small && p.Cin == 128 && p.Cout == 128 && !p.res_w) return C3Form{128, 128, 4, tail_, false, 8, false};
+    if (w8 && !small && p.res_w && p.Cout == 128 && p.Cin == 64) return C3Form{64, 128, 4, false, true, 8, false};
+    if (th8 && w8 && !small && p.res_w && p.Cout == 64 && p.Cin >= 128 && !p.pro_stats && rows8) return C3Form{128, 64, 8, false, true, 8, false};
+    if (w8 && !small && p.res_w && p.Cout == 64 && p.Cin >= 128) return C3Form{128, 64, 4, false, true, 8, false};
+    C3Form f{};
+    if (c3_round1_form(p, small, f)) return f;
+    if (c3_small_resident(p, small)) return C3Form{64, 64, 2, tail_, false, 4, true};
+    const int th = small ? 2 : 4, n128 = small ? 64 : 128;
+    if (tail_) return p.Cin == 64 && p.Cout == 64 ? C3Form{64, 64, th, true, false, 4, false} : C3Form{128, n128, th, true, false, 4, false};
     if (p.res_w) {
-        if (p.Cout == 128 && p.Cin == 64) { small ? launch_c3<64, 128, 64, 2, false, true>(p, st) : launch_c3<64, 128, 128, 4, false, true>(p, st); return; }
-        if (p.Cout == 64 && p.Cin >= 128) { small ? launch_c3<128, 64, 64, 2, false, true>(p, st) : launch_c3<128, 64, 64, 4, false, true>(p, st); return; }
-    }
-    if (p.Cout == 64) {
-        if (p.Cin == 64) { small ? launch_c3<64, 64, 64, 2>(p, st) : launch_c3<64, 64, 64, 4>(p, st); }
-        else { small ? launch_c3<128, 64, 64, 2>(p, st) : launch_c3<128, 64, 64, 4>(p, st); }
-    } else {
-        if (p.Cin == 64) { small ? launch_c3<64, 128, 64, 2>(p, st) : launch_c3<64, 128, 128, 4>(p, st); }
-        else { small ? launch_c3<128, 128, 64, 2>(p, st) : launch_c3<128, 128, 128, 4>(p, st); }
-    }
-}
-
-}
-}
+        if (p.Cout == 128 && p.Cin == 64) return C3Form{64, n128, th, false, true, 4, false};
+        if (p.Cout == 64 && p.Cin >= 128) return C3Form{128, 64, th, false, true, 4, false};
+    }
+    if (p.Cout == 64) return C3Form{p.Cin == 64 ? 64 : 128, 64, th, false, false, 4, false};
+    return C3Form{p.Cin == 64 ? 64 : 128, n128, th, false, false, 4, false};
+}
+
+template <int CC, int COUT, int NSL, int TH, bool PRO2, bool RES, int NW, bool RW, bool H32, bool H16>
+static bool c3_row(const C3Form& f, const Conv3P& p, bool query, hipStream_t st, bool& hit) {
+    if (f.cc != CC || p.Cout != COUT || f.nsl != NSL || f.th != TH || f.pro2 != PRO2 || f.res != RES || f.nw != NW || f.rw != RW) return false;
+    hit = true;
+    if (p.x_bf16 ? !H16 : !H32) return false;
+    if (query) return true;
+    if constexpr (H16) { if (p.x_bf16) { launch_c3<CC, COUT, NSL, TH, PRO2, RES, true, NW, RW>(p, st); return true; } }
+    if constexpr (H32) { if (!p.x_bf16) { launch_c3<CC, COUT, NSL, TH, PRO2, RES, false, NW, RW>(p, st); return true; } }
+    return false;
+}
+
+#ifdef DEX_LP_WSPLIT
+#define C3_NEW16 false
+#else
+#define C3_NEW16 true
+#endif
+static bool c3_dispatch(const C3Form& f, const Conv3P& p, bool query, hipStream_t st) {
+    bool hit = false;
+#define C3_ROW(...) { const bool ok = c3_row<__VA_ARGS__>(f, p, query, st, hit); if (hit) return ok; }
+    C3_ROW(128, 128, 128, 8, false, false, 8, false, true, true)
+    C3_ROW(128, 128, 128, 4, false, false, 8, false, true, true)
+    C3_ROW(128, 128, 128, 4, true, false, 8, false, true, true)
+    C3_ROW(64, 128, 128, 4, false, true, 8, false, true, true)
+    C3_ROW(128, 64, 64, 8, false, true, 8, false, true, true)
+    C3_ROW(128, 64, 64, 4, false, true, 8, false, true, true)
+#ifndef DEX_LP_WSPLIT
+    C3_ROW(64, 64, 64, 5, false, false, 10, true, true, true)
+    C3_ROW(64, 128, 32, 5, false, true, 5, true, true, true)
+    C3_ROW(64, 64, 64, 5, true, false, 10, false, true, true)
+    C3_ROW(64, 64, 64, 2, true, false, 4, true, true, true)
+    C3_ROW(64, 64, 64, 2, false, false, 4, true, true, true)
+#endif
+    C3_ROW(64, 64, 64, 5, false, false, 10, false, true, true)
+    C3_ROW(64, 128, 32, 5, false, true, 5, false, true, C3_NEW16)
+    C3_ROW(64, 64, 64, 2, true, false, 4, false, true, true)
+    C3_ROW(64, 64, 64, 4, true, false, 4, false, true, true)
+    C3_ROW(128, 128, 64, 2, true, false, 4, false, true, true)
+    C3_ROW(128, 128, 128, 4, true, false, 4, false, true, true)
+    C3_ROW(64, 64, 64, 2, false, false, 4, false, true, true)
+    C3_ROW(64, 64, 64, 4, false, false, 4, false, true, true)
+    C3_ROW(128, 128, 64, 2, false, false, 4, false, true, true)
+    C3_ROW(128, 128, 128, 4, false, false, 4, false, true, true)
+    C3_ROW(64, 128, 64, 2, false, true, 4, false, true, C3_NEW16)
+    C3_ROW(64, 128, 128, 4, false, true, 4, false, true, false)
+    C3_ROW(128, 64, 64, 2, false, true, 4, false, true, C3_NEW16)
+    C3_ROW(128, 64, 64, 4, false, true, 4, false, true, false)
+    C3_ROW(128, 64, 64, 2, false, false, 4, false, true, false)
+    C3_ROW(128, 64, 64, 4, false, false, 4, false, true, false)
+    C3_ROW(64, 128, 64, 2, false, false, 4, false, true, false)
+    C3_ROW(64, 128, 128, 4, false, false, 4, false, true, false)
+#undef C3_ROW
+    return false;
+}
+
+static bool c3_lp_in_query(int H, int W, int B, int Cin, int Cout, bool res, bool* small) {
+    Conv3P q{};
+    q.H = H; q.W = W; q.B = B; q.Cin = Cin; q.Cout = Cout; q.ldx = Cin; q.x_bf16 = 1;
+    if (res) q.res_w = &q;
+    Conv3P q32 = q; q32.x_bf16 = 0;
+    if (small) *small = false;
+    if (conv3x3_stream_tiles(q)) return true;
+    if (conv3x3_stream_tiles(q32)) return false;
+    const C3Form f = c3_tile_form(q);
+    if (small) *small = f.nw != 8;
+    return c3_dispatch(f, q, true, nullptr);
+}
+
+bool conv3x3_plain_lp_in_supported(int H, int W, int B, int Cin, int Cout) {
+#if defined(DEX_LP_WSPLIT) && !defined(DEX_WS_HAVE_CONV3)
+    return false;
+#endif
+
+    if (Cin != 64 || (Cout != 64 && Cout != 128)) return false;
+    return c3_lp_in_query(H, W, B, Cin, Cout, Cout != Cin, nullptr);
+}
+
+bool conv3x3_cat_lp_in_supported(int H, int W, int B, int Cin, int Cout) {
+#if defined(DEX_LP_WSPLIT) && !defined(DEX_WS_HAVE_CONV3_RES)
+    return false;
+#endif
+
+    if (Cout != 64 || Cin < 128 || Cin % 128 != 0) return false;
+    return c3_lp_in_query(H, W, B, Cin, Cout, true, nullptr);
+}
+
+bool conv3x3_lp_in_small_form(int H, int W, int B, int Cin, int Cout) {
+    bool small = false;
+    return c3_lp_in_query(H, W, B, Cin, Cout, Cin != Cout, &small) && small;
+}
+
+void launch_conv3x3_lp(const Conv3P& p, hipStream_t st) {
+    if (const int tpw = conv3x3_stream_tiles(p)) { launch_conv3x3_stream(p, tpw, st); return; }
+    if (conv3x3_regw_form(p)) { launch_conv3x3_regw(p, st); return; }
+    const C3Form f = c3_tile_form(p);
+    if (!c3_dispatch(f, p, false, st)) {
+        fprintf(stderr, "libdexamd: no conv3x3 patch form <%d,%d,%d,%d,%d,%d,%d,%d%s> is built for this launch (%dx%d, B = %d)\n", f.cc, p.Cout, f.nsl,
+                f.th, (int)f.pro2, (int)f.res, p.x_bf16, f.nw, f.rw ? ",resident" : "", p.H, p.W, p.B);
+        abort();
+    }
+}
+
+}
+}
diff --git a/dex_tts_amd/csrc/dex_api.hip b/dex_tts_amd/csrc/dex_api.hip
--- a/dex_tts_amd/csrc/dex_api.hip
+++ b/dex_tts_amd/csrc/dex_api.hip
@@ -28,7 +28,8 @@
     "DEX_ATTN_SHARED_W8", "DEX_CONVT_MT", "DEX_CONVT_WGS", "DEX_CONV_DOWN_WGS", "DEX_CONV_REGW", "DEX_CONV_REGW_RES", "DEX_CONV_SMALL_MAX", "DEX_CONV_TH8",
     "DEX_CONV_W8", "DEX_DWCONV_CAP", "DEX_FINAL_CAP", "DEX_FIRST_CAP", "DEX_FIRST_MFMA", "DEX_GEMM_NWALK", "DEX_NWALK_SPLIT", "DEX_NWALK_BM", "DEX_POS_COL", "DEX_POS_COL_MIN",
     "DEX_POS_CT", "DEX_REGW_MIN_TILES", "DEX_REGW_WGS", "DEX_ROWCHAIN64", "DEX_ROWCHAIN64A", "DEX_TIV_CAP", "DEX_TV_CHAIN", "DEX_TIV_FOLD", "DEX_LINATTN_NSUB", "DEX_TV_FOLD", "DEX_OUT2_MIN", "DEX_NWALK_DMA",
-    "DEX_LINATTN_HEADWAVES", "DEX_LINATTN_OUT2_HW", "DEX_CONV_ROUND1", "DEX_CONV_RESIDENT", "DEX_KVCTX_ROWS", "DEX_OUT2_ROWS", "DEX_PE_TOK", "DEX_NWALK_SMALL"};
+    "DEX_LINATTN_HEADWAVES", "DEX_LINATTN_OUT2_HW", "DEX_CONV_ROUND1", "DEX_CONV_RESIDENT", "DEX_KVCTX_ROWS", "DEX_OUT2_ROWS", "DEX_PE_TOK", "DEX_NWALK_SMALL",
+    "DEX_LP_SMALL", "DEX_LP_SMALL_ATTN_DOWN", "DEX_LP_SMALL_DOWN", "DEX_LP_SMALL_CAT", "DEX_LP_SMALL_ATTN_UP", "DEX_LP_SMALL_UP"};
 constexpr int N_KNOBS = (int)(sizeof(KNOB_NAMES) / sizeof(KNOB_NAMES[0]));
 int knob_parse(const char* e) {
     if (!e) return KNOB_UNSET;
@@ -998,6 +999,17 @@
         return fl;
     }
     bool linattn_fused(int C) const { return x->lp() && (C == 64 || C == 128) && linattn_fused_supported(C); }
+    bool lp_small(const char* handoff, int dflt) const { return knob_or("DEX_LP_SMALL", 1) != 0 && knob_or(handoff, dflt) != 0; }
+    bool tail_lp_out(long npix, bool small_on) const {
+        const int B = P.d.B;
+        if (linattn_out2_lp_out_supported((int)npix, B)) return true;
+        return small_on && linattn_out2_hw_lp_out_supported((int)npix, B, knob_or("DEX_LINATTN_OUT2_HW", 1) != 0, knob_or("DEX_OUT2_ROWS", 1) != 0);
+    }
+    bool conv_lp_in(bool cat, int H, int W, int Cin, int Cout, bool small_on) const {
+        const int B = P.d.B;
+        if (!(cat ? conv3x3_cat_lp_in_supported(H, W, B, Cin, Cout) : conv3x3_plain_lp_in_supported(H, W, B, Cin, Cout))) return false;
+        return small_on || !conv3x3_lp_in_small_form(H, W, B, Cin, Cout);
+    }
     void linattn(const LinW& w, const StageBuf& s, const TD& X, float* out, int ldo, int ocoff, const LinKvCtxP* tail = nullptr, bool out_lp = false,
                  void* out2_lp = nullptr, int ldo2 = 0, int ocoff2 = 0) {
         const long npix = s.npix; const int B = P.d.B;
@@ -1036,6 +1048,7 @@
             o.wq_lo_off = w.wq_frag[x->lpi()].lo_off;
             o.hw = knob_or("DEX_LINATTN_OUT2_HW", linattn_out2_lp_out_supported((int)npix, B) ? 0 : 1) != 0 ? 1 : 0;
             o.rows = knob_or("DEX_OUT2_ROWS", 1) != 0 ? 1 : 0;
+            if (o.hw && (out_lp || out2_lp) && !linattn_out2_hw_lp_out_supported((int)npix, B, o.hw, o.rows)) o.hw = 0;
             run("linattn_out", 4.0 * npix * B * 128.0 * X.C, ((out_lp ? 6.0 : 8.0) - (xlp ? 2.0 : 0.0) + (out2_lp ? 2.0 : 0.0)) * npix * X.C * B, [&] { launch_linattn_out2(o, x->precision, st); });
             return;
         }
@@ -1315,9 +1328,10 @@
         if (lp_inter && ns == 2 && P.cat16) {
             const StageBuf& sm_ = P.down[ns - 1];
             const ResW& uw = x->up_res[0][0];
-            const bool tail_ok = linattn_fused(sm_.C) && linattn_out2_lp_out_supported((int)sm_.npix, B);
+            const bool cat_small = lp_small("DEX_LP_SMALL_CAT", 1);
+            const bool tail_ok = linattn_fused(sm_.C) && tail_lp_out(sm_.npix, cat_small);
             const bool conv_ok = uw.wr && fast_conv(2 * sm_.C, uw.cout) && conv3x3_bf16_res_supported(2 * sm_.C, uw.cout) &&
-                                 conv3x3_cat_lp_in_supported(P.up[0].H, P.up[0].W, B, 2 * sm_.C, uw.cout);
+                                 conv_lp_in(true, P.up[0].H, P.up[0].W, 2 * sm_.C, uw.cout, cat_small);
             IGemmP fl = final_gemm(sm_.mask_ws, P.cat[0], 2 * sm_.C, 0);
             fl.c_lp = x->lp_kind();
             cat_lp = !knob_off("DEX_CAT_LP") && tail_ok && conv_ok && fl.Wbf && igemm_nwalk_form(fl);
@@ -1338,7 +1352,10 @@
                 char n0[24], n1[24]; snprintf(n0, sizeof n0, "downs.%d.0", i); snprintf(n1, sizeof n1, "downs.%d.1", i);
                 tap(n0, s.r0out, B * s.npix, s.C, s.C); tap(n1, s.r1out, B * s.npix, s.C, s.C);
             }
-            const bool t1_lp = lp_inter && i == 0 && i < ns - 1 && linattn_fused(s.C) && linattn_out2_lp_out_supported((int)s.npix, B);
+            const bool down_strip = i < ns - 1 && x->lp() && !knob_off("DEX_CONV_DOWN") && x->down_ds_w[i].frag[x->lpi()].p &&
+                                    conv_down_supported(s.C, s.H, s.W, s.attn_ld, s.C, s.attn_coff);
+            const bool t1_lp = lp_inter && i == 0 && i < ns - 1 && linattn_fused(s.C) &&
+                               tail_lp_out(s.npix, down_strip && lp_small("DEX_LP_SMALL_ATTN_DOWN", 1));
             const bool skip16 = cat_lp && i == ns - 1;
             linattn(x->down_lin[i], s, r1, s.attn_out, s.attn_ld, s.attn_coff, defer ? &tail : nullptr, t1_lp,
                     skip16 ? P.cat16 : nullptr, s.attn_ld, s.attn_coff);
@@ -1352,7 +1369,7 @@
                 g.inmask = mask; g.inmask_ws = s.mask_ws;
                 const ResW& nw = x->down_res[i + 1][0];
                 const bool t2_lp = lp_inter && nw.wr && fast_conv(s.C, nw.cout) && conv3x3_bf16_res_supported(s.C, nw.cout) &&
-                                   conv3x3_plain_lp_in_supported(g.Ho, g.Wo, B, s.C, nw.cout);
+                                   conv_lp_in(false, g.Ho, g.Wo, s.C, nw.cout, down_strip && lp_small("DEX_LP_SMALL_DOWN", 1));
                 g.a_lp = t1_lp ? lpk : 0; g.c_lp = t2_lp ? lpk : 0;
                 const bool strip_off = knob_off("DEX_CONV_DOWN");
                 if (x->lp() && !strip_off && x->down_ds_w[i].frag[x->lpi()].p && conv_down_supported(s.C, s.H, s.W, a.ld, s.C, a.coff)) {
@@ -1400,7 +1417,9 @@
                 char n0[24], n1[24]; snprintf(n0, sizeof n0, "ups.%d.0", j); snprintf(n1, sizeof n1, "ups.%d.1", j);
                 tap(n0, s.r0out, B * s.npix, s.C, s.C); tap(n1, s.r1out, B * s.npix, s.C, s.C);
             }
-            const bool t5_lp = lp_inter && linattn_fused(s.C) && linattn_out2_lp_out_supported((int)s.npix, B);
+            const int up_ld = j < ns - 2 ? 2 * stage_dim(c, i - 1) : s.C;
+            const bool up_strip = x->lp() && x->up_us_w[j][0].frag[x->lpi()].p && !knob_off("DEX_CONVT_UP") && convt_up_supported(s.C, s.H, s.W, s.C, up_ld);
+            const bool t5_lp = lp_inter && linattn_fused(s.C) && tail_lp_out(s.npix, up_strip && lp_small("DEX_LP_SMALL_ATTN_UP", 1));
             linattn(x->up_lin[j], s, r1, s.attn_out, s.C, 0, defer ? &tail : nullptr, t5_lp);
             char nm[16]; snprintf(nm, sizeof nm, "up%d", j);
             tap(nm, s.attn_out, B * s.npix, s.C, s.C);
@@ -1413,7 +1432,7 @@
                 g.c_bstride = 4L * s.H * s.W * ldd;
                 g.inmask = mask; g.inmask_ws = s.mask_ws;
                 g.a_lp = t5_lp ? lpk : 0;
-                up_out_lp = lp_inter && j == ns - 2 && conv3x3_res2_form(80, P.d.T, B);
+                up_out_lp = lp_inter && j == ns - 2 && conv_lp_in(false, 80, P.d.T, c.dim, c.dim, up_strip && lp_small("DEX_LP_SMALL_UP", 1));
                 g.c_lp = up_out_lp ? lpk : 0;
                 const bool strip_off = knob_off("DEX_CONVT_UP");
                 if (x->lp() && x->up_us_w[j][0].frag[x->lpi()].p && !strip_off && convt_up_supported(s.C, s.H, s.W, s.C, ldd)) {
diff --git a/dex_tts_amd/csrc/kernels.h b/dex_tts_amd/csrc/kernels.h
--- a/dex_tts_amd/csrc/kernels.h
+++ b/dex_tts_amd/csrc/kernels.h
@@ -94,6 +94,7 @@
 bool conv3x3_bf16_res_supported(int Cin, int Cout);
 bool conv3x3_bf16_xb_supported(int Cin, int Cout);
 bool conv3x3_plain_lp_in_supported(int H, int W, int B, int Cin, int Cout);
+bool conv3x3_lp_in_small_form(int H, int W, int B, int Cin, int Cout);
 bool igemm_nwalk_form(const IGemmP& p);
 bool conv3x3_cat_lp_in_supported(int H, int W, int B, int Cin, int Cout);
 bool conv3x3_strip_form(const Conv3P& p);
@@ -196,6 +197,7 @@
                   };
 void launch_linattn_out2(const LinOut2P& p, int precision, hipStream_t st);
 bool linattn_out2_lp_out_supported(int npix, int B);
+bool linattn_out2_hw_lp_out_supported(int npix, int B, int hw, int rows);
 bool linattn_fused_supported(int C);
 
 struct DwConvP { const float* X; int ldx; long xb; int Hi, Wi, C; int k, s, pad; const float* Wd; const float* bd;
diff --git a/dex_tts_amd/csrc/kernels_lp.h b/dex_tts_amd/csrc/kernels_lp.h
--- a/dex_tts_amd/csrc/kernels_lp.h
+++ b/dex_tts_amd/csrc/kernels_lp.h
@@ -14,6 +14,8 @@
 bool conv3x3_regw_form(const Conv3P& p);
 void launch_conv3x3_regw(const Conv3P& p, hipStream_t st);
 bool linattn_out2_lp_out_supported(int npix, int B);
+bool linattn_out2_hw_lp_out_supported(int npix, int B, int hw, int rows);
+bool conv3x3_lp_in_small_form(int H, int W, int B, int Cin, int Cout);
 bool linattn_fused_supported(int C);
 bool conv3x3_plain_lp_in_supported(int H, int W, int B, int Cin, int Cout);
 bool conv3x3_res2_form(int H, int W, int B);
diff --git a/dex_tts_amd/csrc/linattn_fused.hip b/dex_tts_amd/csrc/linattn_fused.hip
--- a/dex_tts_amd/csrc/linattn_fused.hip
+++ b/dex_tts_amd/csrc/linattn_fused.hip
@@ -991,9 +991,18 @@
                 float4 oa, oc;
                 oa.x = ya.x + xa[k].x + bia[0].x; oa.y = ya.y + xa[k].y + bia[0].y; oa.z = ya.z + xa[k].z + bia[0].z; oa.w = ya.w + xa[k].w + bia[0].w;
                 oc.x = yc.x + xc[k].x + bia[1].x; oc.y = yc.y + xc[k].y + bia[1].y; oc.z = yc.z + xc[k].z + bia[1].z; oc.w = yc.w + xc[k].w + bia[1].w;
-                float* yr = Y + (long)(px0 + rp) * p.ldy + rch;
-                *reinterpret_cast<float4*>(yr) = oa;
-                *reinterpret_cast<float4*>(yr + 4) = oc;
+                if (p.y_lp) {
+                    u16* yh = reinterpret_cast<u16*>(p.Y) + (long)b * p.yb + p.y_coff + (long)(px0 + rp) * p.ldy + rch;
+                    *reinterpret_cast<uint4*>(yh) = make_uint4(pack2_lp(oa.x, oa.y), pack2_lp(oa.z, oa.w), pack2_lp(oc.x, oc.y), pack2_lp(oc.z, oc.w));
+                } else {
+                    float* yr = Y + (long)(px0 + rp) * p.ldy + rch;
+                    *reinterpret_cast<float4*>(yr) = oa;
+                    *reinterpret_cast<float4*>(yr + 4) = oc;
+                }
+                if (p.Y2) {
+                    u16* y2 = reinterpret_cast<u16*>(p.Y2) + (long)b * p.y2b + p.y2_coff + (long)(px0 + rp) * p.ldy2 + rch;
+                    *reinterpret_cast<uint4*>(y2) = make_uint4(pack2_lp(oa.x, oa.y), pack2_lp(oa.z, oa.w), pack2_lp(oc.x, oc.y), pack2_lp(oc.z, oc.w));
+                }
             }
         }
     } else if (px0 + i < p.npix) {
@@ -1138,6 +1147,9 @@
 }
 static long out2_min_wgs() { return knob_or("DEX_OUT2_MIN", 256); }
 bool linattn_out2_lp_out_supported(int npix, int B) { return (long)((npix + 127) / 128) * B >= out2_min_wgs(); }
+bool linattn_out2_hw_lp_out_supported(int npix, int B, int hw, int rows) {
+    return hw && rows && !linattn_out2_lp_out_supported(npix, B);
+}
 void launch_linattn_out2(const LinOut2P& p, hipStream_t st) {
     dim3 grid((p.npix + 127) / 128, p.B);
     const size_t lds = (size_t)4 * 32 * (p.C + 4) * sizeof(float);
@@ -1146,8 +1158,8 @@
         hipFuncSetAttribute(reinterpret_cast<const void*>(&linattn_out2_kernel<128>), hipFuncAttributeMaxDynamicSharedMemorySize, (int)((size_t)4 * 32 * 132 * sizeof(float)));
         attr = true;
     }
-    const bool lp_io = p.x_lp || p.y_lp || p.Y2;
-    if (p.hw && !lp_io) {
+    const bool lp_out = p.y_lp || p.Y2;
+    if (p.hw && !p.x_lp && (!lp_out || p.rows)) {
         g_last_symbol = "linattn_out2_hw_kernel";
         const dim3 g1((p.npix + 31) / 32, p.B);
         if (p.rows) {
@@ -1160,6 +1172,7 @@
         return;
     }
     if ((long)grid.x * p.B < out2_min_wgs()) {
+        if (p.x_lp || lp_out) { fprintf(stderr, "libdexamd: the direct linear-attention tail has no 16-bit x / y form (%d pixels, B = %d)\n", p.npix, p.B); abort(); }
         if (p.C == 64) hipLaunchKernelGGL(linattn_out2_direct_kernel<64>, grid, dim3(256), 0, st, p);
         else hipLaunchKernelGGL(linattn_out2_direct_kernel<128>, grid, dim3(256), 0, st, p);
         return;
diff --git a/dex_tts_amd/csrc/lp_dispatch.hip b/dex_tts_amd/csrc/lp_dispatch.hip
--- a/dex_tts_amd/csrc/lp_dispatch.hip
+++ b/dex_tts_amd/csrc/lp_dispatch.hip
@@ -20,6 +20,8 @@
 bool conv3x3_bf16_xb_supported(int Cin, int Cout) { return (g_lp_wsplit ? f16w::conv3x3_bf16_xb_supported(Cin, Cout) : bf16::conv3x3_bf16_xb_supported(Cin, Cout)); }
 bool conv3x3_plain_lp_in_supported(int H, int W, int B, int Cin, int Cout) { return (g_lp_wsplit ? f16w::conv3x3_plain_lp_in_supported(H, W, B, Cin, Cout) : bf16::conv3x3_plain_lp_in_supported(H, W, B, Cin, Cout)); }
 bool linattn_out2_lp_out_supported(int npix, int B) { return (g_lp_wsplit ? f16w::linattn_out2_lp_out_supported(npix, B) : bf16::linattn_out2_lp_out_supported(npix, B)); }
+bool linattn_out2_hw_lp_out_supported(int npix, int B, int hw, int rows) { return (g_lp_wsplit ? f16w::linattn_out2_hw_lp_out_supported(npix, B, hw, rows) : bf16::linattn_out2_hw_lp_out_supported(npix, B, hw, rows)); }
+bool conv3x3_lp_in_small_form(int H, int W, int B, int Cin, int Cout) { return (g_lp_wsplit ? f16w::conv3x3_lp_in_small_form(H, W, B, Cin, Cout) : bf16::conv3x3_lp_in_small_form(H, W, B, Cin, Cout)); }
 bool linattn_fused_supported(int C) { return (g_lp_wsplit ? f16w::linattn_fused_supported(C) : bf16::linattn_fused_supported(C)); }
 bool conv3x3_res2_form(int H, int W, int B) { return (g_lp_wsplit ? f16w::conv3x3_res2_form(H, W, B) : bf16::conv3x3_res2_form(H, W, B)); }
 bool attention_lp_shared_form(int Nq, int heads, int B, int ksplit) { return (g_lp_wsplit ? f16w::attention_lp_shared_form(Nq, heads, B, ksplit) : bf16::attention_lp_shared_form(Nq, heads, B, ksplit)); }
```
